# albfre/ipm-zoo

Measured on AMD Instinct MI355X. Metric: Newton steps/sec + factor TFLOP/s, dense QP n=8192, 1/2/4/8 MI355X, higher is better.
Workload: dtype f64; 1 GPU; c3; n=8192, m=2048, p=1024, kkt_N=11264, formulation=SlackedSlacks ineq + Regularization eq (delta=1e-4), augmented LDL^T, parallelism=replicas x1 (independent QPs, one per GPU)

## Files before the change

### include/ipmz.h

```cpp
#ifndef IPMZ_H
#define IPMZ_H

#include <stddef.h>
#include <stdint.h>

#ifdef __cplusplus
extern "C" {
#endif

#define IPMZ_OK 0
#define IPMZ_ERR_INVALID (-1)
#define IPMZ_ERR_HIP (-2)
#define IPMZ_ERR_NOMEM (-3)
#define IPMZ_ERR_NO_DEVICE (-4)
#define IPMZ_ERR_STATE (-5)

enum ipmz_slot {
  IPMZ_SLOT_X = 0, IPMZ_SLOT_LAMBDA_A, IPMZ_SLOT_LAMBDA_C, IPMZ_SLOT_S, IPMZ_SLOT_P,
  IPMZ_SLOT_LAMBDA_G, IPMZ_SLOT_LAMBDA_H, IPMZ_SLOT_LAMBDA_Y, IPMZ_SLOT_LAMBDA_Z,
  IPMZ_SLOT_G, IPMZ_SLOT_H, IPMZ_SLOT_Y, IPMZ_SLOT_Z, IPMZ_NSLOT
};

enum ipmz_scalar {
  IPMZ_SC_F = 0,
// ... 46 lines not shown

int64_t ipmz_normal_workspace_bytes(ipmz_ctx* ctx, int n, int mp);
int ipmz_normal_factor(ipmz_ctx* ctx, int n, int mp, double* K, int64_t ld, double* D, void* ws, int64_t ws_bytes);
int ipmz_normal_solve(ipmz_ctx* ctx, int n, int mp, const double* K, int64_t ld, const double* D, void* ws, double* b);
int ipmz_normal_solve_multi(ipmz_ctx* ctx, int n, int mp, const double* K, int64_t ld, const double* D, void* ws,
                            double* B, int64_t ldb, int nrhs);

int ipmz_bk_factor(ipmz_ctx* ctx, int N, double* A, int64_t ld, int* ipiv, int fix_kp);
#define IPMZ_BK_AUTO 0
#define IPMZ_BK_WORKGROUP 1
#define IPMZ_BK_GRID 2
int ipmz_bk_factor_ex(ipmz_ctx* ctx, int N, double* A, int64_t ld, int* ipiv, int fix_kp, int algo);
int ipmz_bk_solve(ipmz_ctx* ctx, int N, const double* F, int64_t ld, const int* ipiv, double* b);
int64_t ipmz_bk_solve_workspace_bytes(ipmz_ctx* ctx, int N);
int ipmz_bk_prepare_solve(ipmz_ctx* ctx, int N, const double* F, int64_t ld, const int* ipiv,
                          void* ws, int64_t ws_bytes);
int ipmz_bk_solve_multi(ipmz_ctx* ctx, int N, const double* F, int64_t ld, const int* ipiv,
                        const void* ws, double* B, int64_t ldb, int nrhs);
#define IPMZ_BK_NMAX 4096
int ipmz_bk_factor_batch(ipmz_ctx* ctx, int N, int batch, double* A, int64_t ld, int64_t sA,
                         int* ipiv, int64_t sP, int fix_kp, int* info);
int64_t ipmz_bk_batch_solve_workspace_bytes(ipmz_ctx* ctx, int N, int batch);
int ipmz_bk_prepare_solve_batch(ipmz_ctx* ctx, int N, int batch, const double* F, int64_t ld, int64_t sA,
                                const int* ipiv, int64_t sP, void* ws, int64_t ws_bytes);
int ipmz_bk_solve_multi_batch(ipmz_ctx* ctx, int N, int batch, const double* F, int64_t ld, int64_t sA,
                              const int* ipiv, int64_t sP, const void* ws,
                              double* B, int64_t ldb, int64_t sB, int nrhs);

int ipmz_symmetric_indefinite_factorization(ipmz_ctx* ctx, int N, const double* A, double* F, int* ipiv);
int ipmz_overwriting_solve_bunch_kaufman(ipmz_ctx* ctx, int N, const double* F, const int* ipiv, double* b);
int ipmz_overwriting_solve_bunch_kaufman_multi(ipmz_ctx* ctx, int N, const double* F, const int* ipiv,
                                               double* B, int nrhs);

int ipmz_ldlt_decomposition(ipmz_ctx* ctx, int N, const double* A, double* L, double* D);
int ipmz_overwriting_solve_ldlt(ipmz_ctx* ctx, int N, const double* L, const double* D, double* b);
int ipmz_overwriting_solve_ldlt_multi(ipmz_ctx* ctx, int N, const double* L, const double* D, double* B, int nrhs);

#define IPMZ_EQ_REGULARIZATION 0
#define IPMZ_EQ_NONE 1
#define IPMZ_EQ_PENALTY 2
#define IPMZ_EQ_PENALTY_EXTRA_DUAL 3
#define IPMZ_EQ_SLACKED_SLACKS 4
#define IPMZ_EQ_NAIVE_SLACKS 5
#define IPMZ_INEQ_SLACKED_SLACKS 0
#define IPMZ_INEQ_SLACKS 1
#define IPMZ_INEQ_NAIVE_SLACKS 2
#define IPMZ_BOUNDS_BOTH 0
#define IPMZ_BOUNDS_LOWER 1
#define IPMZ_BOUNDS_UPPER 2
#define IPMZ_BOUNDS_NONE 3
typedef struct ipmz_qp_config {
  int n;
  int m;
  int p;
  double delta;
  int equality_handling;
  int inequality_handling;
  int inequality_bounds;
  int variable_bounds;
} ipmz_qp_config;

int ipmz_qp_create(ipmz_ctx* ctx, const ipmz_qp_config* cfg, ipmz_qp** out);
int ipmz_qp_destroy(ipmz_qp* qp);
int ipmz_qp_load_host(ipmz_qp* qp, const double* Q, const double* c, const double* A, const double* l_A,
                      const double* u_A, const double* C, const double* d, const double* l_x, const double* u_x);
int ipmz_qp_generate(ipmz_qp* qp, uint64_t seed);
#define IPMZ_STEP_RESTART_IF_CONVERGED 1
#define IPMZ_STEP_GRAPH 2
int ipmz_qp_step(ipmz_qp* qp, int flags);
int ipmz_qp_last_step_graph(ipmz_qp* qp);
int ipmz_qp_scalars(ipmz_qp* qp, double* out);
int ipmz_qp_device_scalars(ipmz_qp* qp, double** out);
int ipmz_qp_copy_scalars(ipmz_qp* qp, double* dst_device);
int ipmz_qp_solve(ipmz_qp* qp, int max_iter, double* trace, int* iterations);
#define IPMZ_STATE_VARS 0
#define IPMZ_STATE_DAFF 1
#define IPMZ_STATE_DIR 2
#define IPMZ_STATE_RES 3
int64_t ipmz_qp_state_len(ipmz_qp* qp);
int ipmz_qp_get_state(ipmz_qp* qp, int which, double* host_out);
int ipmz_qp_set_state(ipmz_qp* qp, const double* host_vars);
int ipmz_qp_get_kkt(ipmz_qp* qp, double* host_K);
int ipmz_qp_kkt_dim(ipmz_qp* qp);
int ipmz_qp_kkt_solve(ipmz_qp* qp, int nrhs, double* B, int64_t ldb);
int ipmz_qp_kkt_solve_bk(ipmz_qp* qp, int nrhs, double* B, int64_t ldb);
int ipmz_qp_kkt_solve_mixed(ipmz_qp* qp, int nrhs, double* B, int64_t ldb, double tol, int max_refine, double* stat);
int ipmz_qp_set_mixed_precision(ipmz_qp* qp, int enable, double tol, int max_refine);
#define IPMZ_REDUCTION_AUGMENTED 0
#define IPMZ_REDUCTION_NORMAL 1
int ipmz_qp_set_reduction(ipmz_qp* qp, int reduction);

int ipmz_batch_create(ipmz_ctx* ctx, const ipmz_qp_config* cfg, int batch, ipmz_qp** out);
int ipmz_batch_size(ipmz_qp* qp);
int ipmz_batch_load_host(ipmz_qp* qp, int index, const double* Q, const double* c, const double* A,
                         const double* l_A, const double* u_A, const double* C, const double* d, const double* l_x,
                         const double* u_x);
int ipmz_batch_initialize(ipmz_qp* qp);
int ipmz_batch_scalars(ipmz_qp* qp, double* out);
int ipmz_batch_get_state(ipmz_qp* qp, int index, int which, double* host_out);
int ipmz_batch_set_state(ipmz_qp* qp, int index, const double* host_vars);
typedef struct ipmz_qp_device_data {
  const double* Q;
  int64_t ldq, sQ;
  const double* A;
  int64_t lda, sA;
  const double* C;
  int64_t ldc, sC;
  const double *c, *l_x, *u_x;
  int64_t sc, slx, sux;
  const double *l_A, *u_A;
  int64_t slA, suA;
  const double* d;
  int64_t sd;
} ipmz_qp_device_data;
int ipmz_batch_load_device(ipmz_qp* qp, const ipmz_qp_device_data* data);
int ipmz_batch_copy_state(ipmz_qp* qp, int which, double* dst_device, int64_t ld);
#define IPMZ_SET_STATE_UNCHECKED 1
int ipmz_batch_set_state_device(ipmz_qp* qp, const double* src, int64_t ld, const int32_t* take, double floor,
                                int flags);
int ipmz_batch_copy_scalars(ipmz_qp* qp, double* dst_device);
int ipmz_batch_summary(ipmz_qp* qp, double* dst_device);
int ipmz_batch_solve(ipmz_qp* qp, int max_iter, int* iterations, int* converged_count);
#define IPMZ_BATCH_FACTOR_AUTO 0
#define IPMZ_BATCH_FACTOR_ONE 1
#define IPMZ_BATCH_FACTOR_PAIR 2
#define IPMZ_BATCH_FACTOR_LEFT 3
int ipmz_batch_set_factor_kernel(ipmz_qp* qp, int kernel);
int ipmz_batch_get_kkt(ipmz_qp* qp, int index, double* host_K);
int ipmz_batch_kkt_solve(ipmz_qp* qp, int nrhs, double* B, int64_t ldb, int64_t sB);
int ipmz_batch_kkt_solve_bk(ipmz_qp* qp, int nrhs, double* B, int64_t ldb, int64_t sB, int* info);

int ipmz_qp_newton_solve_multi(ipmz_qp* qp, int nrhs, const double* R, int64_t ldr, double* Dir, int64_t ldd,
                               double* alpha );
int ipmz_batch_newton_solve_multi(ipmz_qp* qp, int nrhs, const double* R, int64_t ldr, int64_t sR, double* Dir,
                                  int64_t ldd, int64_t sD, double* alpha ,
                                  int* info );

int ipmz_qp_newton_adjoint_multi(ipmz_qp* qp, int nrhs, const double* G, int64_t ldg, double* Out, int64_t ldo);
int ipmz_batch_newton_adjoint_multi(ipmz_qp* qp, int nrhs, const double* G, int64_t ldg, int64_t sG, double* Out,
                                    int64_t ldo, int64_t sO, int* info );

typedef struct ipmz_qp_device_grad {
  double* Q;
  int64_t ldq, sQ;
  double* A;
  int64_t lda, sA;
  double* C;
  int64_t ldc, sC;
  double *c, *l_x, *u_x;
  int64_t sc, slx, sux;
  double *l_A, *u_A;
  int64_t slA, suA;
  double* d;
  int64_t sd;
} ipmz_qp_device_grad;
int ipmz_batch_data_vjp(ipmz_qp* qp, const double* W, int64_t sW, const ipmz_qp_device_grad* grad);

typedef struct ipmz_qp_device_grad_multi {
  ipmz_qp_device_grad g;
  int64_t tQ, tA, tC, tc, tlx, tux, tlA, tuA, td;
} ipmz_qp_device_grad_multi;
int ipmz_batch_data_vjp_multi(ipmz_qp* qp, int ncot, const double* W, int64_t ldw, int64_t sW,
                              const ipmz_qp_device_grad_multi* grad);

typedef struct ipmz_qp_device_tangent {
  ipmz_qp_device_data d;
// ... 16 lines not shown
```

### ipm-zoo_amd/csrc/capi.cpp

```cpp
#include "capi.h"

#include <cstring>

namespace {
thread_local std::string g_last_error;
}

int fail(int code, const std::string& msg) {
  g_last_error = msg;
  return code;
}
int hip_fail(hipError_t e, const char* expr, const char* file, int line) {
  return fail(IPMZ_ERR_HIP, std::string(expr) + ": " + hipGetErrorString(e) + " @" + file + ":" + std::to_string(line));
}

std::mutex g_ctx_mutex;

static int ensure_events(ipmz_ctx* ctx, size_t n) {
  while (ctx->evpool.size() < n) {
    hipEvent_t e;
    if (hipEventCreateWithFlags(&e, hipEventDisableTiming | hipEventDisableSystemFence) != hipSuccess &&
        hipEventCreateWithFlags(&e, hipEventDisableTiming) != hipSuccess)
      return fail(IPMZ_ERR_HIP, "hipEventCreate failed");
    ctx->evpool.push_back(e);
  }
  return IPMZ_OK;
}

static int check_device(int device) {
  int count = 0;
  if (hipGetDeviceCount(&count) != hipSuccess || count <= 0)
    return fail(IPMZ_ERR_NO_DEVICE, "no HIP device visible: libipmz has no CPU fallback");
  if (device < 0 || device >= count) return fail(IPMZ_ERR_INVALID, "device index out of range");
  hipDeviceProp_t prop;
  if (hipGetDeviceProperties(&prop, device) != hipSuccess) return fail(IPMZ_ERR_NO_DEVICE, "device query failed");
  if (std::strncmp(prop.gcnArchName, "gfx950", 6) != 0)
    return fail(IPMZ_ERR_NO_DEVICE, std::string("libipmz is built for gfx950, device is ") + prop.gcnArchName);
  return IPMZ_OK;
}

void ctx_free(ipmz_ctx* ctx) {
  hipSetDevice(ctx->device);
  if (ctx->stream) hipStreamSynchronize(ctx->stream);
  for (hipStream_t s : {ctx->own, ctx->sB, ctx->sC, ctx->sD})
    if (s) {
      hipStreamSynchronize(s);
      hipStreamDestroy(s);
    }
  for (auto e : ctx->evpool) hipEventDestroy(e);
  delete ctx;
}

const char PANEL_TIMEOUT[] = ": a hand-off inside the outer-panel factor kernel timed out (spin limit 0.5 s); the "
                             "factor is invalid";
const char SOLVE_TIMEOUT[] = ": a hand-off inside the persistent triangular solve timed out (spin limit 0.5 s); the "
                             "solution is invalid";
int ws_result(hipStream_t st, const int* info, const unsigned* pe_word, const unsigned* se_word, const char* what,
              const char* pe_text, const char* se_text) {
  int i = 0x7f7f7f7f;
  unsigned pe = 0, se = 0;
  if (pe_word) HIP_OK(hipMemcpyAsync(&pe, pe_word, 4, hipMemcpyDeviceToHost, st));
  if (se_word) HIP_OK(hipMemcpyAsync(&se, se_word, 4, hipMemcpyDeviceToHost, st));
  if (info) HIP_OK(hipMemcpyAsync(&i, info, sizeof(int), hipMemcpyDeviceToHost, st));
  HIP_OK(hipStreamSynchronize(st));
  if (pe) return fail(IPMZ_ERR_HIP, std::string(what) + pe_text);
  if (se) return fail(IPMZ_ERR_HIP, std::string(what) + se_text);
  return i == 0x7f7f7f7f ? IPMZ_OK : i;
}

int read_info(ipmz_ctx* ctx, const LdltWs& w) {
  return ws_result(ctx->stream, w.info, w.pctrl + PANEL_ERR_WORD, w.ctrl + SOLVE_ERR_WORD, "ipmz_ldlt_factor");
}

hipError_t solve_ws(const double* K, int64_t ld, int N, const double* D, const LdltWs& w, int nbi, double* b,
                    hipStream_t st) {
  if (nbi == 64) return ldlt_solve_persistent(K, ld, N, D, w.P, b, w.y, w.z, w.ctrl, st);
  return ldlt_solve(K, ld, N, D, w.Linv, nbi, b, w.side, st);
}

int factor_impl(ipmz_ctx* ctx, int N, double* K, int64_t ld, double* D, const LdltWs& w, int nbo, TrailTimer* timer,
                int* info2) {
  HIP_OK(solve_reset(w.y, w.z, sizeof(double), N, w.ctrl, ctx->stream, w.info, w.pctrl, panel_ctrl_words(N, nbo),
                     info2));
  const int npan = (N + nbo - 1) / nbo;
  auto prep = [&]() -> hipError_t {
    return ctx->nbi == 64 ? solve_prep(K, ld, N, w.Linv, w.P, ctx->stream) : hipSuccess;
  };
  if (npan < 3 || (debug_inject_mask() & IPMZ_DEBUG_ONE_STREAM)) {
    HIP_OK(ldlt_factor(K, ld, N, D, w.Linv, w.W, nbo, ctx->nbi, w.info, ctx->stream, timer, nullptr, nullptr, nullptr,
                       0, w.pctrl));
    HIP_OK(prep());
    return IPMZ_OK;
  }
  const int nev = 5 * npan + 5;
  int rc = ensure_events(ctx, (size_t)nev + 4);
  if (rc) return rc;
  hipEvent_t* ev = ctx->evpool.data();
  const bool fourth = false;
  HIP_OK(ldlt_factor(K, ld, N, D, w.Linv, w.W, nbo, ctx->nbi, w.info, ctx->stream, timer, ctx->sB, ctx->sC, ev,
                     nev - 2, w.pctrl, fourth ? ctx->sD : nullptr));
  HIP_OK(prep());
  return IPMZ_OK;
}

hipError_t bk_setup(const double* F, int64_t ld, int N, const int* ipiv, const int* info, double* LT, double* Lp,
                    int64_t ldp, const BkWs& w, hipStream_t st) {
  hipError_t e = bk_fast_prepare(F, ld, N, ipiv, info, LT, Lp, ldp, w.meta, st);
  if (e == hipSuccess) e = linv_from_l(Lp, ldp, N, 64, w.Linv, st);
  if (e == hipSuccess) e = solve_prep(Lp, ldp, N, w.Linv, w.P, st);
  if (e == hipSuccess) e = solve_reset(w.y, w.x, sizeof(double), N, w.ctrl, st);
  return e;
}
hipError_t bk_run(const double* Lp, int64_t ldp, int N, const double* LT, const int* ipiv, const BkWs& w, double* b,
                  hipStream_t st) {
  const unsigned* flag = bk_fast_flag(w.meta);
  double* t = bk_fast_tmp(w.meta, N);
  const double* ones = bk_fast_ones(w.meta, N);
  hipError_t e = bk_fast_gather(b, N, w.meta, st);
  if (e == hipSuccess) e = ldlt_solve_persistent_sweep(Lp, ldp, N, ones, w.P, t, w.y, w.x, w.ctrl, false, st, flag);
  if (e == hipSuccess) e = bk_fast_dsolve(w.y, N, w.meta, st);
  if (e == hipSuccess) e = ldlt_solve_persistent_sweep(Lp, ldp, N, ones, w.P, t, w.y, w.x, w.ctrl, true, st, flag);
  if (e == hipSuccess) e = bk_fast_scatter(b, N, w.meta, st);
  if (e == hipSuccess) e = bk_fast_fallback(LT, N, ipiv, b, w.meta, st);
  return e;
}

int mixed_factor_impl(ipmz_ctx* ctx, const double* K, int64_t ld, MixedWs& w, TrailTimer* timer) {
  const int npan = (w.N + w.nbo - 1) / w.nbo;
  if (npan < 3 || (debug_inject_mask() & IPMZ_DEBUG_ONE_STREAM)) {
    HIP_OK(mixed_factor(K, ld, w, ctx->stream, nullptr, nullptr, nullptr, 0, timer));
    HIP_OK(solve_prep(w.K32, w.ld32, w.N, w.Linv32, w.P32, ctx->stream));
    return IPMZ_OK;
  }
  const int nev = 5 * npan + 5;
  int rc = ensure_events(ctx, (size_t)nev + 4);
  if (rc) return rc;
  hipEvent_t* ev = ctx->evpool.data();
  const bool fourth = !(debug_inject_mask() & IPMZ_DEBUG_NO_FOURTH);
  HIP_OK(mixed_factor(K, ld, w, ctx->stream, ctx->sB, ctx->sC, ev, nev - 2, timer, fourth ? ctx->sD : nullptr));
  HIP_OK(solve_prep(w.K32, w.ld32, w.N, w.Linv32, w.P32, ctx->stream));
  return IPMZ_OK;
}

static constexpr int SOLVE_MULTI_PANEL = IPMZ_SOLVE_MULTI_PANEL;
static constexpr int SOLVE_MULTI_CROSSOVER = 10;
static_assert(SOLVE_MULTI_PANEL % 128 == 0 && SOLVE_MULTI_PANEL <= IPMZ_TRSM_PANEL_MAX, "panel width");

static int ldlt_multi_impl(ipmz_ctx* ctx, int N, const double* K, int64_t ld, const double* D, const LdltWs& w,
                           double* B, int64_t ldb, int nrhs) {
  const MultiPlan plan =
      multi_plan(nrhs, SOLVE_MULTI_CROSSOVER, SOLVE_MULTI_PANEL, debug_inject_mask(), MultiKind::Ldlt);
  if (!plan.blocked) {
    for (int r = 0; r < nrhs; ++r) HIP_OK(solve_ws(K, ld, N, D, w, ctx->nbi, B + (int64_t)r * ldb, ctx->stream));
  } else {
    HIP_OK(ldlt_solve_multi<double>(K, ld, N, D, w.Linv, ctx->nbi, B, ldb, nrhs, plan.width, ctx->stream));
  }
  watch(ctx, w);
  return IPMZ_OK;
}

static constexpr int BK_MULTI_CROSSOVER = 12;

int bk_multi_impl(ipmz_ctx* ctx, int N, const double* F, int64_t ld, const int* ipiv, const double* LT,
                  const double* Lp, int64_t ldp, const BkWs& w, double* B, int64_t ldb, int nrhs) {
  const MultiPlan plan = multi_plan(nrhs, BK_MULTI_CROSSOVER, SOLVE_MULTI_PANEL, debug_inject_mask(), MultiKind::Bk);
  hipStream_t st = ctx->stream;
  if (!plan.blocked) {
    for (int r = 0; r < nrhs; ++r) {
      double* b = B + (int64_t)r * ldb;
      if (N < IPMZ_BK_GRID_MIN) HIP_OK(bk_solve(F, ld, N, ipiv, b, 1, 0, 0, 0, st));
      else HIP_OK(bk_run(Lp, ldp, N, LT, ipiv, w, b, st));
    }
  } else {
    const unsigned* flag = bk_fast_flag(w.meta);
    HIP_OK(bk_multi_gather(B, ldb, nrhs, N, w.meta, st));
    HIP_OK(trsm_sweep<double>(Lp, ldp, N, w.Linv, 64, B, ldb, nrhs, plan.width, false, st, flag));
    HIP_OK(bk_multi_dsolve(B, ldb, nrhs, N, w.meta, st));
    HIP_OK(trsm_sweep<double>(Lp, ldp, N, w.Linv, 64, B, ldb, nrhs, plan.width, true, st, flag));
    HIP_OK(bk_multi_scatter(B, ldb, nrhs, N, w.meta, st));
    HIP_OK(bk_multi_fallback(LT, N, ipiv, B, ldb, nrhs, w.meta, st));
  }
  watch(ctx, w);
  return IPMZ_OK;
// ... 679 lines not shown
```

### ipm-zoo_amd/csrc/capi.h

```cpp
#pragma once
#include <hip/hip_runtime.h>

#include <cstdint>
#include <mutex>
#include <string>
#include <vector>

#include "ipmz.h"
#include "kernels.h"

using namespace ipmz;

#pragma GCC visibility push(hidden)

int fail(int code, const std::string& msg);
int hip_fail(hipError_t e, const char* expr, const char* file, int line);
#define HIP_OK(expr)                                                           \
  do {                                                                         \
    hipError_t _e = (expr);                                                    \
    if (_e != hipSuccess) return hip_fail(_e, #expr, __FILE__, __LINE__);      \
  } while (0)

inline int64_t round_up(int64_t x, int64_t a) { return (x + a - 1) / a * a; }

// ... 95 lines not shown
  int64_t total = 0;
};
inline BkBatchWs bk_batch_ws(char* base, int N, int batch) {
  BkBatchWs w;
  Carver c{base};
  w.ldp = round_up(N, 64);
  w.sLT = round_up((int64_t)N * N, 32);
  w.sLp = (int64_t)N * w.ldp;
  w.sLinv = (int64_t)((N + 63) / 64) * 64 * 64;
  w.sM = (int64_t)bk_fast_meta_bytes(N);
  w.LT = c.take<double>(w.sLT * batch);
  w.Lp = c.take<double>(w.sLp * batch);
  w.Linv = c.take<double>(w.sLinv * batch);
  w.meta = c.take<char>(w.sM * batch);
  w.total = c.off;
  return w;
}

struct VjpWs {
  double* part = nullptr;
  int64_t total = 0;
};
inline VjpWs vjp_ws(char* base, int64_t elems) {
  VjpWs w;
  Carver c{base};
  w.part = c.take<double>(elems);
  w.total = c.off;
  return w;
}

struct JvpWs {
  double* prod = nullptr;
  int64_t total = 0;
};
inline JvpWs jvp_ws(char* base, int64_t elems) {
  JvpWs w;
  Carver c{base};
  w.prod = c.take<double>(elems);
  w.total = c.off;
  return w;
}

inline void watch(ipmz_ctx* ctx, const unsigned* pe, const unsigned* se) {
  ctx->check_pe = pe;
  ctx->check_se = se;
}
inline void watch(ipmz_ctx* ctx, const LdltWs& w) { watch(ctx, w.pctrl + PANEL_ERR_WORD, w.ctrl + SOLVE_ERR_WORD); }
inline void watch(ipmz_ctx* ctx, const BkWs& w) { watch(ctx, nullptr, w.ctrl + SOLVE_ERR_WORD); }
inline void unwatch(ipmz_ctx* ctx) { ctx->check_pe = ctx->check_se = nullptr; }

enum class MultiKind { Ldlt, Bk, Batch };
struct MultiPlan {
  bool blocked;
  int width;
  bool fused;
};
constexpr MultiPlan multi_plan(int nrhs, int crossover, int panel, int dbg, MultiKind kind) {
  const bool w512 = dbg & IPMZ_DEBUG_MULTI_W512, w128 = dbg & IPMZ_DEBUG_MULTI_W128;
  const bool batch = kind == MultiKind::Batch;
  const bool blocked =
      nrhs >= crossover || ((dbg & IPMZ_DEBUG_MULTI_BLOCKED) && (kind == MultiKind::Ldlt || nrhs >= 2));
  return {blocked, batch && w512 && w128 ? panel : w512 ? 512 : w128 ? 128 : panel, blocked && batch && !w512 && !w128};
}
constexpr bool multi_plan_pins(MultiKind kind, int forced, int w0, int w512, int w128, int wboth, bool fused) {
  const int rows[4] = {1, 2, 9, 10}, width[4] = {w0, w512, w128, wboth};
  for (int m = 0; m < 8; ++m)
    for (int i = 0; i < 4; ++i) {
      const int dbg = (m & 1 ? IPMZ_DEBUG_MULTI_W512 : 0) | (m & 2 ? IPMZ_DEBUG_MULTI_W128 : 0) |
                      (m & 4 ? IPMZ_DEBUG_MULTI_BLOCKED : 0);
      const bool blocked = i == 3 || ((m & 4) && (forced >> i & 1));
      const MultiPlan p = multi_plan(rows[i], 10, 256, dbg, kind);
      if (p.blocked != blocked || p.width != width[m & 3] || p.fused != (blocked && fused && !(m & 3))) return false;
    }
  return true;
}
static_assert(multi_plan_pins(MultiKind::Ldlt, 0b1111, 256, 512, 128, 512, false), "Ldlt: blocked at any count, 512 wins");
static_assert(multi_plan_pins(MultiKind::Bk, 0b1110, 256, 512, 128, 512, false), "Bk: blocked from 2 rows, 512 wins");
static_assert(multi_plan_pins(MultiKind::Batch, 0b1110, 256, 512, 128, 256, true), "Batch: from 2 rows, both = default");

extern const char PANEL_TIMEOUT[], SOLVE_TIMEOUT[];
int ws_result(hipStream_t st, const int* info, const unsigned* pe, const unsigned* se, const char* what,
              const char* pe_text = PANEL_TIMEOUT, const char* se_text = SOLVE_TIMEOUT);
int read_info(ipmz_ctx* ctx, const LdltWs& w);
int factor_impl(ipmz_ctx* ctx, int N, double* K, int64_t ld, double* D, const LdltWs& w, int nbo, TrailTimer* timer,
                int* info2 = nullptr);
hipError_t solve_ws(const double* K, int64_t ld, int N, const double* D, const LdltWs& w, int nbi, double* b,
                    hipStream_t st);
int mixed_factor_impl(ipmz_ctx* ctx, const double* K, int64_t ld, MixedWs& w, TrailTimer* timer);
int mixed_multi_impl(ipmz_ctx* ctx, const double* K, int64_t ld, MixedWs& w, const MixedMultiWs& m, double* B,
                     int64_t ldb, int nrhs, double tol, int max_refine, double* stat);
int not_capturing(ipmz_ctx* ctx, const char* who);
int normal_factor_impl(ipmz_ctx* ctx, int n, int mp, double* K, int64_t ld, double* D, const NormalWs& w, int nbo,
                       TrailTimer* timer);
int normal_solve_impl(ipmz_ctx* ctx, int n, int mp, const double* K, int64_t ld, const double* D, const NormalWs& w,
                      double* b);
hipError_t bk_setup(const double* F, int64_t ld, int N, const int* ipiv, const int* info, double* LT, double* Lp,
                    int64_t ldp, const BkWs& w, hipStream_t st);
hipError_t bk_run(const double* Lp, int64_t ldp, int N, const double* LT, const int* ipiv, const BkWs& w, double* b,
                  hipStream_t st);
int bk_multi_impl(ipmz_ctx* ctx, int N, const double* F, int64_t ld, const int* ipiv, const double* LT,
                  const double* Lp, int64_t ldp, const BkWs& w, double* B, int64_t ldb, int nrhs);
int bk_batch_prepare(ipmz_ctx* ctx, int N, int batch, const double* F, int64_t ld, int64_t sA, const int* ipiv,
                     int64_t sP, const int* info, const BkBatchWs& w);
int bk_batch_multi_impl(ipmz_ctx* ctx, int N, int batch, const double* F, int64_t ld, int64_t sA, const int* ipiv,
                        int64_t sP, const BkBatchWs& w, double* B, int64_t ldb, int64_t sB, int nrhs);
int bk_batch_info(hipStream_t st, const int* dinfo, int batch, int* info);

#pragma GCC visibility pop
```

### ipm-zoo_amd/csrc/kernels.h

```cpp
#pragma once
#include <hip/hip_runtime.h>
#include <stdint.h>
#include <stdio.h>

#define IPMZ_NBO_MAX 512
#define IPMZ_PANEL_CTRL_WORDS 320
#define IPMZ_EARLY_CHAIN_MAX_N 4096
#define IPMZ_TCHUNK 32
#define IPMZ_CHAIN_STAMP_BLOCKS 512
#define IPMZ_SOLVE_BLOCK 128
#define IPMZ_SOLVE_CTRL_WORDS 8

namespace ipmz {

enum { IPMZ_INJECT_SOLVE = 1, IPMZ_INJECT_PANEL = 2, IPMZ_INJECT_GRAPH_FORKS = 4, IPMZ_DEBUG_CONVERT_ONLY = 16,
       IPMZ_DEBUG_ONE_STREAM = 32, IPMZ_DEBUG_TRACE = 64, IPMZ_DEBUG_F32_ENGINE = 128,
       IPMZ_DEBUG_NO_FOURTH = 256, IPMZ_DEBUG_IR_FULL = 512,
       IPMZ_DEBUG_F64_ENGINE = 1024, IPMZ_DEBUG_GIVEBACK = 2048, IPMZ_DEBUG_ROWS_CHAIN = 4096,
       IPMZ_DEBUG_NO_K0 = 8192, IPMZ_DEBUG_NO_FUSED_SOLVES = 16384, IPMZ_DEBUG_READY_LATE = 32768,
       IPMZ_DEBUG_MULTI_BLOCKED = 65536, IPMZ_DEBUG_MULTI_W512 = 131072,
       IPMZ_DEBUG_MULTI_W128 = 262144, IPMZ_DEBUG_SOLVE_H2 = 524288, IPMZ_DEBUG_SOLVE_H4 = 1048576,
       IPMZ_DEBUG_NEWTON_RPG1 = 2097152, IPMZ_DEBUG_NEWTON_RPG8 = 4194304 };
#define IPMZ_TRACE(...)                                                  \
  do {                                                                   \
    if (::ipmz::debug_inject_mask() & ::ipmz::IPMZ_DEBUG_TRACE) {        \
      fprintf(stderr, "[ipmz] " __VA_ARGS__);                            \
      fputc('\n', stderr);                                              \
      fflush(stderr);                                                    \
    }                                                                    \
  } while (0)
int debug_inject_mask();
hipError_t stream_record(hipEvent_t e, hipStream_t s);
hipError_t stream_wait(hipStream_t s, hipEvent_t e);
void set_capture_origin(hipStream_t s);
void set_debug_inject_mask(int mask);
constexpr int PANEL_ERR_WORD = 2;
constexpr int SOLVE_ERR_WORD = 1;

struct Carver {
  char* base;
  int64_t off = 0;
  template <typename T>
  T* take(int64_t count) {
    char* p = base ? base + off : nullptr;
    off += (count * (int64_t)sizeof(T) + 255) / 256 * 256;
    return reinterpret_cast<T*>(p);
  }
};

struct BatchStrides {
  int B = 1;
  int64_t sK = 0, sD = 0, sL = 0, sW = 0;
  unsigned* pflags = nullptr;
  const double* K0 = nullptr;
  int small_kernel = 0;
};
#define IPMZ_PAIR_FLAGS 32
bool small_pair_eligible(int B, int N);
bool small_pair_used(int kern, bool have_flags, int B, int N);
#define IPMZ_SMALL_NMAX 1024
hipError_t ldlt_factor_small_batched(double* K, int64_t ld, int N, double* D, double* Linv, double* W, int* info,
                                     hipStream_t st, const BatchStrides& bs);
hipError_t ldlt_factor_small_variant(int snw, double* K, int64_t ld, int N, double* D, double* Linv, double* W,
                                     int* info, hipStream_t st, const BatchStrides& bs);
hipError_t ldlt_factor_batched(double* K, int64_t ld, int N, double* D, double* Linv, double* W, int nbo, int nbi,
                               int* info, hipStream_t st, const BatchStrides& bs);
#define IPMZ_TRAIL_SMALL_M 3072
struct TrailTimer {
  hipEvent_t (*pairs)[2] = nullptr;
  int cap = 0, used = 0;
  double flops = 0.0;
  hipEvent_t* next() { return used < cap ? pairs[used++] : nullptr; }
};
hipError_t ldlt_factor(double* K, int64_t ld, int N, double* D, double* Linv, double* W, int nbo, int nbi,
                       int* info, hipStream_t st, TrailTimer* timer = nullptr, hipStream_t st2 = nullptr,
                       hipStream_t st3 = nullptr, hipEvent_t* ev = nullptr, int nev = 0, unsigned* pctrl = nullptr, hipStream_t st4 = nullptr);
hipError_t ldlt_factor(float* K, int64_t ld, int N, float* D, float* Linv, float* W, int nbo, int nbi, int* info,
                       hipStream_t st, TrailTimer* timer, hipStream_t st2, hipStream_t st3, hipEvent_t* ev, int nev,
                       unsigned* pctrl = nullptr, hipStream_t st4 = nullptr);
#define IPMZ_PANEL_PRE00_WORDS (3 * 64 * 64 * 2)
inline int64_t panel_ctrl_words(int N, int nbo) {
  return (int64_t)IPMZ_PANEL_CTRL_WORDS * (1 + (N + nbo - 1) / nbo) + IPMZ_PANEL_PRE00_WORDS;
}
hipError_t panel_factor(double* K, int64_t ld, int N, int k0, int bo, double* D, double* Lb0, double* Wp, int ldw,
                        const double* pre00_in, double* pre00_out,
                        int* info, unsigned* area, unsigned* err, const double* Wprev, int kprev, int boprev,
                        bool rows_prev, hipStream_t st_chain, hipStream_t st_rows,
                        const unsigned* parea = nullptr, bool wait_ready = false);
hipError_t panel_factor(float* K, int64_t ld, int N, int k0, int bo, float* D, float* Lb0, float* Wp, int ldw,
                        const float* pre00_in, float* pre00_out,
                        int* info, unsigned* area, unsigned* err, const float* Wprev, int kprev, int boprev,
                        bool rows_prev, hipStream_t st_chain, hipStream_t st_rows,
                        const unsigned* parea = nullptr, bool wait_ready = false);
hipError_t panel_ready(unsigned* area, hipStream_t st);
hipError_t linv_from_l(const double* L, int64_t ld, int N, int nbi, double* Linv, hipStream_t st, int batch = 1,
                       int64_t sL = 0, int64_t sLinv = 0);
hipError_t gemm_nt_sub(int M, int N, int Kd, const double* A, int64_t lda, const double* B, int64_t ldb,
                       double* C, int64_t ldc, int64_t row0, int64_t col0, bool square_lower, hipStream_t st,
                       const BatchStrides* bs = nullptr);

hipError_t ldlt_solve(const double* K, int64_t ld, int N, const double* D, const double* Linv, int nbi, double* b,
                      double* side, hipStream_t st);

#define IPMZ_TRSM_PANEL_MAX 512
struct TrsmBatch {
  int B = 1;
  int64_t sK = 0, sD = 0, sL = 0, sB = 0;
  int64_t sG = 0;
};
template <typename T>
hipError_t ldlt_solve_multi(const T* K, int64_t ld, int N, const T* D, const T* Linv, int nbi, T* B, int64_t ldb,
                            int nrhs, int w, hipStream_t st, const TrsmBatch& tb = TrsmBatch());

template <typename T>
hipError_t trsm_sweep(const T* K, int64_t ld, int N, const T* Linv, int nbi, T* B, int64_t ldb, int nrhs, int w,
                      bool backward, hipStream_t st, const unsigned* gate, const TrsmBatch& tb = TrsmBatch());

bool ldlt_solve_fused_eligible(int N, int nbi);
hipError_t ldlt_solve_fused(const double* K, int64_t ld, int N, const double* D, const double* Linv, int nbi,
                            double* B, int64_t ldb, int nrhs, hipStream_t st, const TrsmBatch& tb = TrsmBatch());

hipError_t ldlt_solve_batched(const double* K, int64_t ld, int N, const double* D, const double* Linv, int nbi,
                              double* b, int B, int64_t sK, int64_t sD, int64_t sL, int64_t sb, hipStream_t st);

int64_t solve_prep_elems(int N);
int64_t solve_vec_elems(int N);
hipError_t solve_reset(void* ybuf, void* xbuf, size_t elem, int N, unsigned* ctrl, hipStream_t st,
                       int* info = nullptr, unsigned* words = nullptr, int64_t nwords = 0, int* info2 = nullptr);
hipError_t solve_stamps(unsigned long long* out);
hipError_t chain_stamps(unsigned long long* c, unsigned long long* h);
hipError_t solve_prep(const double* K, int64_t ld, int N, const double* Linv, double* P, hipStream_t st);
hipError_t solve_prep(const float* K, int64_t ld, int N, const float* Linv, float* P, hipStream_t st);
hipError_t ldlt_solve_persistent(const double* K, int64_t ld, int N, const double* D, const double* P, double* b,
                                 double* ybuf, double* xbuf, unsigned* ctrl, hipStream_t st);
hipError_t ldlt_solve_persistent_sweep(const double* K, int64_t ld, int N, const double* D, const double* P,
                                       double* b, double* ybuf, double* xbuf, unsigned* ctrl, bool backward,
                                       hipStream_t st, const unsigned* skip);
hipError_t ldlt_solve_persistent(const float* K, int64_t ld, int N, const float* D, const float* P, float* b,
                                 float* ybuf, float* xbuf, unsigned* ctrl, hipStream_t st,
                                 const unsigned* skip = nullptr);

struct MixedWs {
  int N = 0, nbo = 256;
  int64_t ld32 = 0;
  float *K32 = nullptr, *D32 = nullptr, *Linv32 = nullptr, *W32 = nullptr, *P32 = nullptr;
  float *y32 = nullptr, *z32 = nullptr, *r32 = nullptr;
  unsigned *ctrl = nullptr, *state = nullptr, *pctrl = nullptr;
  int* info = nullptr;
  double *s = nullptr, *x = nullptr, *colp = nullptr, *rowp = nullptr, *part = nullptr;
  double* stat = nullptr;
  unsigned *hst = nullptr, *hst_dev = nullptr;
  hipEvent_t hev = nullptr;
  int last_iters = 2;
};
int64_t mixed_ws_bytes(int N, int nbo);
int64_t mixed_ws_carve(char* base, int N, int nbo, MixedWs& w);
hipError_t mixed_factor(const double* K, int64_t ld, MixedWs& w, hipStream_t st, hipStream_t st2, hipStream_t st3,
                        hipEvent_t* ev, int nev, TrailTimer* timer = nullptr, hipStream_t st4 = nullptr);
hipError_t mixed_solve(const double* K, int64_t ld, MixedWs& w, double* b, double tol, int max_refine,
                       hipStream_t st);

struct MixedMultiWs {
  int64_t ldx = 0, ld32 = 0;
  int ntiles = 0;
  double* x = nullptr;
  float* r32 = nullptr;
  double* part = nullptr;
  double* stat = nullptr;
  unsigned* done = nullptr;
  unsigned* word = nullptr;
};
int64_t mixed_multi_ws_carve(char* base, int N, int nrhs, MixedMultiWs& m);
hipError_t mixed_solve_multi(const double* K, int64_t ld, const MixedWs& w, const MixedMultiWs& m, double* B,
                             int64_t ldb, int nrhs, double tol, int max_refine, int pw, hipStream_t st);
hipError_t sym_residual_multi(const double* K, int64_t ld, int N, const double* X, int64_t ldx, const double* B,
                              int64_t ldb, double* R, int64_t ldr, int nrhs, hipStream_t st);

hipError_t ne_check_sign(const double* D, int N, int offset, double sign, int* info, hipStream_t st);


#ifndef IPMZ_BK_NMAX
#define IPMZ_BK_NMAX 4096
#endif
hipError_t bk_factor(double* A, int64_t ld, int n, int* ipiv, int* info, int fix_kp, int batch, int64_t sA,
                     int64_t sP, hipStream_t st);
hipError_t bk_solve(const double* F, int64_t ld, int n, const int* ipiv, double* b, int batch, int64_t sA, int64_t sP,
                    int64_t sb, hipStream_t st);
#define IPMZ_BK_GRID_MIN 512
size_t bk_grid_ws_bytes(int n);
hipError_t bk_factor_grid(double* A, int64_t ld, int n, int* ipiv, int* info, int fix_kp, void* ws, hipStream_t st);
const unsigned* bk_grid_err_word(const void* ws, int n);
struct BkBatch {
  int B = 1;
  int64_t sA = 0, sP = 0, sLT = 0, sLp = 0, sB = 0;
};
hipError_t bk_transpose(const double* F, int64_t ld, int n, double* LT, hipStream_t st,
                        const BkBatch& bb = BkBatch());
size_t bk_fast_meta_bytes(int n);
const unsigned* bk_fast_flag(const void* meta);
const double* bk_fast_ones(const void* meta, int n);
double* bk_fast_tmp(void* meta, int n);
hipError_t bk_fast_prepare(const double* F, int64_t ld, int n, const int* ipiv, const int* info, double* LT,
                           double* Lp, int64_t ldp, void* meta, hipStream_t st, const BkBatch& bb = BkBatch());
hipError_t bk_fast_gather(const double* b, int n, void* meta, hipStream_t st);
hipError_t bk_fast_dsolve(double* y, int n, void* meta, hipStream_t st);
hipError_t bk_fast_scatter(double* b, int n, void* meta, hipStream_t st);
hipError_t bk_fast_fallback(const double* LT, int n, const int* ipiv, double* b, const void* meta, hipStream_t st);
hipError_t bk_multi_gather(double* B, int64_t ldb, int nrhs, int n, void* meta, hipStream_t st,
                           const BkBatch& bb = BkBatch());
hipError_t bk_multi_dsolve(double* B, int64_t ldb, int nrhs, int n, void* meta, hipStream_t st,
                           const BkBatch& bb = BkBatch());
hipError_t bk_multi_scatter(double* B, int64_t ldb, int nrhs, int n, void* meta, hipStream_t st,
                            const BkBatch& bb = BkBatch());
hipError_t bk_multi_fallback(const double* LT, int n, const int* ipiv, double* B, int64_t ldb, int nrhs,
                             const void* meta, hipStream_t st);
struct BkFusedMeta {
  const unsigned* flag;
// ... 24 lines not shown
  SC_SIGMA,
  SC_ALPHA,
  SC_CONVERGED,
  SC_MU_NEW,
  SC_RESTARTS,
  SC_COUNT = 16
};

struct QPDev {
  int n, m, p;
  int N;
  int64_t ldn;
  int64_t ldk;
  int64_t state_len;
  double delta;
  int eqnone;
  int eqpen;
  int slacks, vlo, vup, alo, aup;
  int naive;
  int eqss, m_usr, p_usr;
  int mk;
  const double *Q, *c, *A, *lA, *uA, *C, *d, *lx, *ux;
  double* v[NSLOT];
  double* r[NSLOT];
  double* daff[NSLOT];
  double* dir[NSLOT];
  double *Qx, *ATl, *CTl, *Ax, *Cx;
  double* b;
  double* scal;
  double* part;
  double* tpart;
  double* K;
  double* K0;
  double *v0, *r0, *scal0;
  double* Cx0;
  unsigned* done;
};

__host__ __device__ __forceinline__ int residual_rows(const QPDev& q) { return q.n + q.m + q.p; }
__host__ __device__ __forceinline__ int comp_rows(const QPDev& q) { return q.n + q.m; }
__host__ __device__ __forceinline__ int corrector_rows(const QPDev& q) {
  return comp_rows(q) + (q.eqpen ? q.p : 0);
}
__host__ __device__ __forceinline__ int update_rows(const QPDev& q) {
  const int mp = q.m > q.p ? q.m : q.p;
  return q.n > mp ? q.n : mp;
}

__host__ __device__ __forceinline__ int64_t eqss_block(int64_t k, int64_t m, int64_t p) {
  const int64_t mp = m + p;
  if (k < m) return k;
  if (k < 2 * m) return mp + (k - m);
  if (k < 2 * m + p) return m + (k - 2 * m);
  return mp + m + (k - 2 * m - p);
}
__host__ __device__ __forceinline__ int64_t eqss_source(int64_t k, const QPDev& q) {
  const int64_t n = q.n, m = q.m_usr, p = q.p_usr, mp = m + p;
  const int64_t duals = q.naive ? n : n + 2 * mp;
  if (k < duals) return k;
  if (k < duals + 2 * mp) return duals + eqss_block(k - duals, m, p);
  const int64_t slacks = duals + 2 * mp + (q.vlo ? n : 0) + (q.vup ? n : 0);
  if (k < slacks) return k;
  if (k < slacks + 2 * mp) return slacks + eqss_block(k - slacks, m, p);
  return k;
}

__host__ __device__ __forceinline__ int slot_in_order(bool naive, int k) {
  constexpr int naive_order[NSLOT] = {X, LG, LH, LC, P, LY, LZ, G, H, Y, Z, LA, S};
  return naive ? naive_order[k] : k;
}
__host__ __device__ __forceinline__ bool nonneg_slot(int slot) { return slot >= LG; }
__host__ __device__ __forceinline__ bool explicit_bounds(const QPDev& q) { return q.slacks || q.m == 0; }

struct QPBatch {
  const QPDev* d;
  QPDev h;
  int B;
};

hipError_t qp_generate(const QPBatch& qb, uint64_t seed0, hipStream_t st);
hipError_t qp_init_iterate(const QPBatch& qb, hipStream_t st);
hipError_t qp_evaluate(const QPBatch& qb, hipStream_t st);
hipError_t qp_assemble(const QPBatch& qb, hipStream_t st);
hipError_t qp_rhs(const QPBatch& qb, hipStream_t st);
hipError_t qp_backsub(const QPBatch& qb, int which, hipStream_t st);
hipError_t qp_ratio(const QPBatch& qb, int which, int out_index, hipStream_t st);
#define IPMZ_NEWTON_MULTI_RPG 4
hipError_t qp_rhs_multi(const QPBatch& qb, const double* R, int64_t ldr, int64_t sR, double* W, int64_t ldw, int64_t sW,
                        int nrhs, hipStream_t st);
hipError_t qp_backsub_multi(const QPBatch& qb, const double* R, int64_t ldr, int64_t sR, const double* W, int64_t ldw,
                            int64_t sW, double* D, int64_t ldd, int64_t sD, int nrhs, hipStream_t st);
hipError_t qp_ratio_multi(const QPBatch& qb, const double* D, int64_t ldd, int64_t sD, double* alpha, int nrhs,
                          hipStream_t st);
hipError_t qp_adj_reduce_multi(const QPBatch& qb, const double* Cot, int64_t ldg, int64_t sG, double* W, int64_t ldw,
                               int64_t sW, int nrhs, hipStream_t st);
hipError_t qp_adj_expand_multi(const QPBatch& qb, const double* Cot, int64_t ldg, int64_t sG, const double* W,
                               int64_t ldw, int64_t sW, double* Out, int64_t ldo, int64_t sO, int nrhs, hipStream_t st);
hipError_t qp_mu_aff(const QPBatch& qb, hipStream_t st);
hipError_t qp_corrector_residuals(const QPBatch& qb, hipStream_t st);
hipError_t qp_update(const QPBatch& qb, int freeze, hipStream_t st);
hipError_t qp_restart_if_converged(const QPBatch& qb, hipStream_t st);
hipError_t qp_save_initial(const QPBatch& qb, hipStream_t st);
hipError_t qp_batch_summary(const QPBatch& qb, double* out, hipStream_t st);
#define IPMZ_FUSED_NMAX 1024
enum { KMODE_K = 0, KMODE_K0_DIAG = 1, KMODE_K0_OFFDIAG = 2 };
hipError_t qp_fused_pre(const QPBatch& qb, int restart, int* info, hipStream_t st, int kmode = KMODE_K);
hipError_t qp_fused_mid(const QPBatch& qb, hipStream_t st);
hipError_t qp_fused_post(const QPBatch& qb, int freeze, hipStream_t st);
inline bool fused_solves_ok(int N, int64_t ld) { return N <= 4096 && !(ld & 1); }
hipError_t qp_fused_solves(const QPBatch& qb, const double* K, int64_t ld, int N, const double* D, const double* Linv,
                           double* b, int64_t sK, int64_t sD, int64_t sL, int64_t sb, int freeze, hipStream_t st);
hipError_t qp_fused_eval(const QPBatch& qb, hipStream_t st);

enum DataBlock { DB_Q = 0, DB_A, DB_CEQ, DB_C, DB_LX, DB_UX, DB_LA, DB_UA, DB_D, DB_COUNT, DB_MATS = DB_C };
enum : unsigned {
  HELD_Q = 1, HELD_C = 2, HELD_A = 4, HELD_LA = 8, HELD_UA = 16, HELD_CEQ = 32, HELD_D = 64, HELD_LX = 128,
  HELD_UX = 256, HELD_ALL = 511
};
struct DataBlockInfo {
  const char* name;
  bool matrix;
  int dim;
  unsigned held;
};
constexpr DataBlockInfo DATA_BLOCKS[DB_COUNT] = {
    {"Q", true, 0, HELD_Q},      {"A", true, 1, HELD_A},      {"C", true, 2, HELD_CEQ},
    {"c", false, 0, HELD_C},     {"l_x", false, 0, HELD_LX},  {"u_x", false, 0, HELD_UX},
    {"l_A", false, 1, HELD_LA},  {"u_A", false, 1, HELD_UA},  {"d", false, 2, HELD_D}};
template <class T>
struct QpBlocks {
  T* p[DB_COUNT];
  int64_t sq[DB_COUNT], tq[DB_COUNT], ld[DB_MATS];
};
typedef QpBlocks<const double> QpBlocksIn;
typedef QpBlocks<double> QpBlocksOut;
constexpr unsigned long long IPMZ_IO_VALID = ~0ull;
constexpr unsigned long long io_key(int qp, int kind, int k) {
  return ((unsigned long long)(unsigned)qp << 33) | ((unsigned long long)kind << 32) | (unsigned)k;
}
hipError_t qp_io_validate(const QPBatch& qb, const QpBlocksIn& in, unsigned long long* verdict, hipStream_t st);
hipError_t qp_io_pack(const QPBatch& qb, const QpBlocksIn& in, hipStream_t st);
hipError_t qp_gather_state(const QPBatch& qb, int which, double* dst, int64_t ld, hipStream_t st);
hipError_t qp_scatter_state(const QPBatch& qb, const double* src, int64_t ld, const int32_t* take, double floor,
                            hipStream_t st);
hipError_t qp_scatter_validate(const QPBatch& qb, const double* src, int64_t ld, const int32_t* take, double floor,
                               unsigned long long* verdict, hipStream_t st);

#define IPMZ_VJP_KCHUNK 64
#define IPMZ_VJP_SLAB 16
int64_t qp_grad_part_elems(const QPBatch& qb, int ncot = 1);
hipError_t qp_data_vjp(const QPBatch& qb, int ncot, const double* W, int64_t ldw, int64_t sW, const QpBlocksOut& o,
                       double* part, hipStream_t st);

#define IPMZ_JVP_ROWS_GY 16384
struct JvpMat {
  int mode, rch, nchunk, nct;
  int64_t off_row, off_col;
};
struct JvpPlan {
  JvpMat mat[3];
  int64_t seg;
};
JvpPlan qp_jvp_plan(const QPBatch& qb, const QpBlocksIn& in);
int jvp_pairs(int n);
hipError_t qp_data_jvp(const QPBatch& qb, int ntan, const QpBlocksIn& in, double* R, int64_t ldr, int64_t sR, double* ws,
                       hipStream_t st);
// ... 3 lines not shown
```

### ipm-zoo_amd/csrc/ldlt.hip

```cpp
#include <cstdlib>
#include <cstring>
#include <map>
#include <mutex>
#include <unordered_map>
#include <vector>

#include "common.h"
#include "diag64.h"
#include "gemm.h"
#include "gemm32.h"
#include "gemm64.h"
#include "kernels.h"

namespace ipmz {

static int g_inject = 0;

int debug_inject_mask() { return g_inject; }
void set_debug_inject_mask(int mask) { g_inject = mask; }

namespace {
struct Noted {
  unsigned long long id;
  std::vector<hipGraphNode_t> nodes;
// ... 264 lines not shown
  if (M <= 4096) return launch_gemm<64, 64, EPI_SUB_STRIP, 2, 2, OPT_NOR2>(g, st, batch);
  if (M <= 8192) return launch_gemm<64, 128, EPI_SUB_STRIP, 2, 4, OPT_NOR2>(g, st, batch);
  return launch_gemm<128, 128, EPI_SUB_STRIP, 2, 4, OPT_NOR2>(g, st, batch);
}
hipError_t gemm_nt_sub(int M, int N, int Kd, const double* A, int64_t lda, const double* B, int64_t ldb,
                       double* C, int64_t ldc, int64_t row0, int64_t col0, bool square_lower, hipStream_t st,
                       const BatchStrides* bs) {
  return gemm_nt_sub_t<double>(M, N, Kd, A, lda, B, ldb, C, ldc, row0, col0, square_lower, st, bs);
}

template <typename T>
static hipError_t factor_panel(T* K, int64_t ld, int N, T* D, T* Linv, T* W, int k0, int bo, int nbo, int nbi,
                               int* info, hipStream_t st, const BatchStrides* bs = nullptr) {
  hipError_t e = hipSuccess;
  const int B = bs ? bs->B : 1;
  const int64_t sK = bs ? bs->sK : 0, sD = bs ? bs->sD : 0, sL = bs ? bs->sL : 0, sW = bs ? bs->sW : 0;
  for (int j0 = k0; j0 < k0 + bo; j0 += nbi) {
    const int bi = k0 + bo - j0 < nbi ? k0 + bo - j0 : nbi;
    T* Lb = Linv + (int64_t)(j0 / nbi) * nbi * nbi;
    if (nbi == 128)
      hipLaunchKernelGGL((ldlt_diag_kernel<T, 128>), dim3(B), dim3(1024), 0, st, K, ld, j0, bi, D, Lb, info, sK, sD, sL);
    else
      launch_diag64(B, st, K, ld, j0, bi, D, Lb, info, sK, sD, sL);
    if ((e = hipGetLastError()) != hipSuccess) return e;
    const int r1 = j0 + bi;
    if (r1 >= N) continue;
    GemmArgsT<T> g{};
    g.M = N - r1;
    g.N = bi;
    g.Kd = bi;
    g.A = K + (int64_t)r1 * ld + j0;
    g.lda = ld;
    g.B = Lb;
    g.ldb = nbi;
    g.C = K + (int64_t)r1 * ld + j0;
    g.ldc = ld;
    g.W = W + (int64_t)r1 * nbo + (j0 - k0);
    g.ldw = nbo;
    g.dvec = D + j0;
    g.lower = 0;
    g.sA = sK;
    g.sB = sL;
    g.sC = sK;
    g.sW = sW;
    g.sD = sD;
    e = nbi == 128 ? launch_gemm<128, 128, EPI_PANEL, 2, 4>(g, st, B) : launch_gemm<128, 64, EPI_PANEL, 4, 2>(g, st, B);
    if (e != hipSuccess) return e;
    const int c1 = k0 + bo;
    if (r1 < c1) {
      e = gemm_nt_sub_t<T>(N - r1, c1 - r1, bi, W + (int64_t)r1 * nbo + (j0 - k0), nbo, K + (int64_t)r1 * ld + j0, ld,
                           K + (int64_t)r1 * ld + r1, ld, r1, r1, false, st, bs);
      if (e != hipSuccess) return e;
    }
  }
  return hipSuccess;
}

template <typename T>
static hipError_t panel_update(T* K, int64_t ld, int N, const T* Wk, int nbo, int k0, int bo, int c0, int c1,
                               bool square, hipStream_t st, const BatchStrides* bs = nullptr) {
  if (c0 >= c1 || c0 >= N) return hipSuccess;
  return gemm_nt_sub_t<T>(N - c0, c1 - c0, bo, Wk + (int64_t)c0 * nbo, nbo, K + (int64_t)c0 * ld + k0, ld,
                     K + (int64_t)c0 * ld + c0, ld, c0, c0, square, st, bs);
}

hipError_t ldlt_factor_batched(double* K, int64_t ld, int N, double* D, double* Linv, double* W, int nbo, int nbi,
                               int* info, hipStream_t st, const BatchStrides& bs) {
  if (N <= 0 || bs.B <= 0) return hipSuccess;
  if (nbi != 64 && nbi != 128) return hipErrorInvalidValue;
  if (nbo % nbi != 0 || nbo > IPMZ_NBO_MAX) return hipErrorInvalidValue;
  if (nbi == 64 && N <= IPMZ_SMALL_NMAX) return ldlt_factor_small_batched(K, ld, N, D, Linv, W, info, st, bs);
  hipError_t e = hipSuccess;
  for (int k0 = 0; k0 < N; k0 += nbo) {
    const int bo = N - k0 < nbo ? N - k0 : nbo, t0 = k0 + bo;
    if ((e = factor_panel(K, ld, N, D, Linv, W, k0, bo, nbo, nbi, info, st, &bs)) != hipSuccess) return e;
    if (t0 < N && (e = panel_update(K, ld, N, W, nbo, k0, bo, t0, N, true, st, &bs)) != hipSuccess) return e;
  }
  return hipSuccess;
}

template <typename T>
static hipError_t ldlt_factor_t(T* K, int64_t ld, int N, T* D, T* Linv, T* W, int nbo, int nbi, int* info,
                                hipStream_t st, TrailTimer* timer, hipStream_t st2, hipStream_t st3, hipEvent_t* ev,
                                int nev, unsigned* pctrl, hipStream_t st4) {
  if (N <= 0) return hipSuccess;
  if (nbi != 64 && nbi != 128) return hipErrorInvalidValue;
  if (nbo % nbi != 0 || nbo > IPMZ_NBO_MAX) return hipErrorInvalidValue;
  const int npan = (N + nbo - 1) / nbo;
  const bool fused = pctrl != nullptr && nbi == 64;
  const bool two = st2 != nullptr && ev != nullptr && nev >= 4 * npan + 2 && (!fused || st3 != nullptr);
  const bool four = two && st4 != nullptr && nev >= 5 * npan + 3 && !(debug_inject_mask() & IPMZ_DEBUG_NO_FOURTH);
  const int64_t wsz = (int64_t)N * nbo;
  auto Wb = [&](int k) { return W + (two ? (k % 3) : 0) * wsz; };
  auto pw = [&](int k) { return N - k * nbo < nbo ? N - k * nbo : nbo; };
  auto area = [&](int k) { return pctrl + (int64_t)IPMZ_PANEL_CTRL_WORDS * (1 + k); };
  unsigned* err = pctrl ? pctrl + PANEL_ERR_WORD : nullptr;
  hipStream_t sC = (two && fused) ? st3 : st;
  hipStreamCaptureStatus cap = hipStreamCaptureStatusNone;
  if (two && fused && hipStreamIsCapturing(st, &cap) != hipSuccess) cap = hipStreamCaptureStatusActive;
  const bool early_ok = two && fused && cap == hipStreamCaptureStatusNone;
  auto early_at = [&](int j) { return early_ok && N - j * nbo <= IPMZ_EARLY_CHAIN_MAX_N; };
  auto tiles_at = [&](int j) { return two && fused && N - j * nbo <= IPMZ_EARLY_CHAIN_MAX_N; };
  auto flag_at = [&](int j) { return j >= 2 && early_at(j - 1) && tiles_at(j); };
  T* pre00 = pctrl ? reinterpret_cast<T*>(pctrl + (int64_t)IPMZ_PANEL_CTRL_WORDS * (1 + npan)) : nullptr;
  auto slot00 = [&](int k) { return pre00 + (int64_t)(k % 3) * 64 * 64; };
  auto factor = [&](int k, bool prev) -> hipError_t {
    const int k0 = k * nbo;
    if (!fused) return factor_panel(K, ld, N, D, Linv, Wb(k), k0, pw(k), nbo, nbi, info, st);
    return panel_factor(K, ld, N, k0, pw(k), D, Linv + (int64_t)(k0 / 64) * 64 * 64, Wb(k), nbo,
                        (two && prev) ? slot00(k) : nullptr, two ? slot00(k + 1) : nullptr, info, area(k), err,
                        prev ? Wb(k - 1) : nullptr, k0 - nbo, nbo, prev && tiles_at(k), st, sC,
                        (early_at(k) && prev) ? area(k - 1) : nullptr, prev && flag_at(k));
  };
  hipError_t e = hipSuccess;
  if (!two) {
    for (int k = 0; k < npan; ++k) {
      const int k0 = k * nbo, bo = pw(k), t0 = k0 + bo;
      if ((e = factor(k, false)) != hipSuccess) return e;
      if (t0 < N) {
        hipEvent_t* te = timer && N - t0 > IPMZ_TRAIL_SMALL_M ? timer->next() : nullptr;
        if (te) hipEventRecord(te[0], st);
        e = panel_update(K, ld, N, Wb(k), nbo, k0, bo, t0, N, true, st);
        if (te) hipEventRecord(te[1], st);
        if (te) timer->flops += (double)(N - t0) * (double)(N - t0 + 1) * (double)bo;
        if (e != hipSuccess) return e;
      }
    }
    return hipSuccess;
  }
  hipEvent_t* evP = ev;
  hipEvent_t* evN = ev + npan;
  hipEvent_t* evC = ev + 2 * npan;
  hipEvent_t* evA = ev + 3 * npan;
  hipEvent_t* evT = ev + 4 * npan + 2;
  hipEvent_t evJoin = ev[4 * npan];
  hipEvent_t evJoin4 = four ? ev[5 * npan + 2] : nullptr;
  hipEvent_t evEntry = ev[4 * npan + 1];
  IPMZ_TRACE("factor: N=%d npan=%d look-ahead", N, npan);
  if ((e = stream_record(evEntry, st)) != hipSuccess) return e;
  if ((e = stream_wait(st2, evEntry)) != hipSuccess) return e;
  if (fused && (e = stream_wait(sC, evEntry)) != hipSuccess) return e;
  if ((e = factor(0, false)) != hipSuccess) return e;
  if (fused) {
    if ((e = stream_record(evA[0], st)) != hipSuccess) return e;
    if ((e = stream_record(evC[0], sC)) != hipSuccess) return e;
    if (!early_at(1) && (e = stream_wait(st, evC[0])) != hipSuccess) return e;
  }
  for (int k = 0; k < npan; ++k) {
    const int k0 = k * nbo, bo = pw(k);
    const int p1 = k0 + bo;
    const int p2 = p1 < N ? p1 + pw(k + 1) : N;
    const int p3 = p2 < N ? p2 + pw(k + 2) : N;
    if (p1 >= N) break;
    IPMZ_TRACE("factor: panel %d", k);
    if ((e = stream_record(evP[k], st)) != hipSuccess) return e;
    if ((e = stream_wait(st2, evP[k])) != hipSuccess) return e;
    if (early_at(k + 1) && (e = stream_wait(st2, evC[k])) != hipSuccess) return e;
    hipStream_t sN = four ? st4 : st2;
    if (four) {
      if ((e = stream_wait(st4, evP[k])) != hipSuccess) return e;
      if (early_at(k + 1) && (e = stream_wait(st4, evC[k])) != hipSuccess) return e;
      if (k >= 1 && (e = stream_wait(st4, evT[k - 1])) != hipSuccess) return e;
    }
    if (p2 < N) {
      if ((e = panel_update(K, ld, N, Wb(k), nbo, k0, bo, p2, p3, false, sN)) != hipSuccess) return e;
      if (k + 2 < npan && flag_at(k + 2) && (e = panel_ready(area(k + 2), sN)) != hipSuccess) return e;
    }
    if ((e = stream_record(evN[k], sN)) != hipSuccess) return e;
    if (p3 < N) {
      hipEvent_t* te = timer && N - p3 > IPMZ_TRAIL_SMALL_M ? timer->next() : nullptr;
      if (te) hipEventRecord(te[0], st2);
      e = panel_update(K, ld, N, Wb(k), nbo, k0, bo, p3, N, true, st2);
      if (te) hipEventRecord(te[1], st2);
      if (te) timer->flops += (double)(N - p3) * (double)(N - p3 + 1) * (double)bo;
      if (e != hipSuccess) return e;
    }
    if (four && (e = stream_record(evT[k], st2)) != hipSuccess) return e;
    if (k >= 1) {
      if (!flag_at(k + 1) && (e = stream_wait(st, evN[k - 1])) != hipSuccess) return e;
      if (fused && (e = stream_wait(sC, evN[k - 1])) != hipSuccess) return e;
    }
    if (k >= 1) {
      if (early_at(k + 1) && !early_at(k) && (e = stream_wait(st, evC[k - 1])) != hipSuccess) return e;
    }
    if (fused) {
      if (!tiles_at(k + 1) && (e = stream_wait(sC, evA[k])) != hipSuccess) return e;
      if (p2 < N && !tiles_at(k + 1)) {
        if ((e = gemm_nt_sub_t<T>(N - p2, p2 - p1, bo, Wb(k) + (int64_t)p2 * nbo, nbo, K + (int64_t)p1 * ld + k0, ld,
                                  K + (int64_t)p2 * ld + p1, ld, p2, p1, false, sC, nullptr)) != hipSuccess)
          return e;
      }
      if ((e = factor(k + 1, true)) != hipSuccess) return e;
      if ((e = stream_record(evA[k + 1], st)) != hipSuccess) return e;
      if ((e = stream_record(evC[k + 1], sC)) != hipSuccess) return e;
      if (!early_at(k + 2) && (e = stream_wait(st, evC[k + 1])) != hipSuccess) return e;
    } else {
      if ((e = panel_update(K, ld, N, Wb(k), nbo, k0, bo, p1, p2, false, st)) != hipSuccess) return e;
      if ((e = factor(k + 1, false)) != hipSuccess) return e;
    }
  }
  if (early_ok && (e = stream_wait(st, evC[npan - 1])) != hipSuccess) return e;
  if ((e = stream_record(evJoin, st2)) != hipSuccess) return e;
  if (four) {
    if ((e = stream_record(evJoin4, st4)) != hipSuccess) return e;
    if ((e = stream_wait(st, evJoin4)) != hipSuccess) return e;
  }
  return stream_wait(st, evJoin);
}

hipError_t ldlt_factor(double* K, int64_t ld, int N, double* D, double* Linv, double* W, int nbo, int nbi,
                       int* info, hipStream_t st, TrailTimer* timer, hipStream_t st2, hipStream_t st3, hipEvent_t* ev,
                       int nev, unsigned* pctrl, hipStream_t st4) {
  return ldlt_factor_t<double>(K, ld, N, D, Linv, W, nbo, nbi, info, st, timer, st2, st3, ev, nev, pctrl, st4);
}
hipError_t ldlt_factor(float* K, int64_t ld, int N, float* D, float* Linv, float* W, int nbo, int nbi, int* info,
                       hipStream_t st, TrailTimer* timer, hipStream_t st2, hipStream_t st3, hipEvent_t* ev, int nev,
                       unsigned* pctrl, hipStream_t st4) {
  return ldlt_factor_t<float>(K, ld, N, D, Linv, W, nbo, nbi, info, st, timer, st2, st3, ev, nev, pctrl, st4);
}

}
```

### ipm-zoo_amd/csrc/newton.hip

```cpp
#include <type_traits>

#include "common.h"
#include "data_terms.h"
#include "kernels.h"
#include "sync.h"
#include "trsv_small.h"

namespace ipmz {

namespace {
constexpr int NT = 256;
constexpr int RED_BLOCKS = 512;
enum : uint64_t { TAG_Q = 1, TAG_C = 2, TAG_A = 3, TAG_C_EQ = 4, TAG_D = 5 };

__device__ __forceinline__ double block_sum(double v, double* sh) {
  const int lane = threadIdx.x & 63, wave = threadIdx.x >> 6;
  v = wave_sum(v);
  __syncthreads();
  if (lane == 0) sh[wave] = v;
  __syncthreads();
  double t = 0.0;
  if (threadIdx.x == 0)
    for (int w = 0; w < NT / 64; ++w) t += sh[w];
  return t;
// ... 340 lines not shown
}

__device__ __forceinline__ void stats_store(const QPDev& q, double res2, double comp, double f) {
  const double res = sqrt(res2);
  const int cnt = comp_count(q);
  const double mu = cnt == 0 ? 0.0 : comp / (double)cnt;
  q.scal[SC_F] = f;
  q.scal[SC_RES] = res;
  q.scal[SC_MU] = mu;
  q.scal[SC_CONVERGED] = (res < 1e-8 && mu < 1e-8) ? 1.0 : 0.0;
}

__global__ void k_stats_final(const QPDev* __restrict__ qs, int nblocks) {
  const QPDev& q = qs[blockIdx.y];
  __shared__ double sh[4][NT];
  double s[4] = {0.0, 0.0, 0.0, 0.0};
  for (int b = threadIdx.x; b < nblocks; b += NT)
    for (int k = 0; k < 4; ++k) s[k] += q.part[4 * b + k];
  for (int k = 0; k < 4; ++k) sh[k][threadIdx.x] = s[k];
  __syncthreads();
  if (threadIdx.x == 0) {
    double t[4] = {0.0, 0.0, 0.0, 0.0};
    for (int i = 0; i < NT; ++i)
      for (int k = 0; k < 4; ++k) t[k] += sh[k][i];
    stats_store(q, t[0], t[1], t[2] + t[3]);
  }
}

static int red_blocks(int total) {
  int b = (total + NT - 1) / NT;
  return b < 1 ? 1 : (b > RED_BLOCKS ? RED_BLOCKS : b);
}

hipError_t qp_evaluate(const QPBatch& qb, hipStream_t st) {
  const QPDev& h = qb.h;
  hipLaunchKernelGGL((k_matvec_rows<MV_Q>), grid2((h.n + 3) / 4, qb.B), dim3(NT), 0, st, qb.d);
  if (h.m) {
    hipLaunchKernelGGL((k_matvec_rows<MV_A>), grid2((h.m + 3) / 4, qb.B), dim3(NT), 0, st, qb.d);
    matvec_t<MV_A>(qb, st);
  }
  if (h.p) {
    hipLaunchKernelGGL((k_matvec_rows<MV_C>), grid2((h.p + 3) / 4, qb.B), dim3(NT), 0, st, qb.d);
    matvec_t<MV_C>(qb, st);
  }
  const int nb = red_blocks(residual_rows(h));
  hipLaunchKernelGGL(k_residuals, grid2(nb, qb.B), dim3(NT), 0, st, qb.d, 0.0, 1);
  hipLaunchKernelGGL(k_stats_final, grid2(1, qb.B), dim3(NT), 0, st, qb.d, nb);
  return hipGetLastError();
}

__device__ __forceinline__ double ds_inv(const QPDev& q, int i) {
  return ipmz_inv(ipmz_inv(q.v[G][i]) * q.v[LG][i] + ipmz_inv(q.v[H][i]) * q.v[LH][i]);
}
__device__ __forceinline__ double ds_inv_sl(const QPDev& q, int i) {
  return ipmz_inv(ipmz_inv(q.uA[i] + (-q.v[S][i])) * q.v[LH][i] + ipmz_inv(q.v[S][i] + (-q.lA[i])) * q.v[LG][i]);
}
__device__ __forceinline__ double kkt_xx(const QPDev& q, int i, double qii) {
  double h = qii;
  if (q.slacks) {
    if (q.vup) h = h + ipmz_inv(q.ux[i] + (-q.v[X][i])) * q.v[LZ][i];
    if (q.vlo) h = h + ipmz_inv(q.v[X][i] + (-q.lx[i])) * q.v[LY][i];
  } else {
    if (q.vlo) h = h + ipmz_inv(q.v[Y][i]) * q.v[LY][i];
    if (q.vup) h = h + ipmz_inv(q.v[Z][i]) * q.v[LZ][i];
  }
  return h;
}
__device__ __forceinline__ double kkt_aa(const QPDev& q, int i) {
  if (q.slacks) return -ds_inv_sl(q, i);
  if (q.alo && q.aup) return -ds_inv(q, i);
  if (q.alo) return -(ipmz_inv(q.v[LG][i]) * q.v[G][i]);
  return -(ipmz_inv(q.v[LH][i]) * q.v[H][i]);
}

__device__ __forceinline__ double kkt_diag(const QPDev& q, int i) {
  const int n = q.n, m = q.m;
  if (i < n) return kkt_xx(q, i, q.Q[(int64_t)i * q.ldn + i]);
  if (q.naive && i < n + m) return -(ipmz_inv(q.v[LG][i - n]) * q.v[G][i - n]);
  if (q.naive && i < n + q.mk) return -(ipmz_inv(q.v[LH][i - n - m]) * q.v[H][i - n - m]);
  if (i < n + q.mk) return kkt_aa(q, i - n);
  return q.eqnone ? 0.0 : q.eqpen ? -q.scal[SC_MU_NEW] : -(q.delta * q.delta);
}

__device__ __forceinline__ void assemble_row(const QPDev& q, int i, int tid, int nth) {
  double* __restrict__ K = q.K;
  const int64_t ld = q.ldk;
  const int n = q.n, m = q.m, mk = q.mk;
  double* Kr = K + (int64_t)i * ld;
  if (i < n) {
    const double* Qr = q.Q + (int64_t)i * q.ldn;
    for (int j = tid; j < i; j += nth) Kr[j] = Qr[j];
    if (tid == 0) Kr[i] = kkt_diag(q, i);
  } else if (i < n + mk && q.naive) {
    const bool hrow = i >= n + m;
    const int r = hrow ? i - n - m : i - n;
    const double* Ar = q.A + (int64_t)r * q.ldn;
    for (int j = tid; j < n; j += nth) Kr[j] = hrow ? Ar[j] : -Ar[j];
    for (int j = n + tid; j < i; j += nth) Kr[j] = 0.0;
    if (tid == 0) Kr[i] = kkt_diag(q, i);
  } else if (i < n + m) {
    const int r = i - n;
    const double* Ar = q.A + (int64_t)r * q.ldn;
    for (int j = tid; j < n; j += nth) Kr[j] = Ar[j];
    for (int j = n + tid; j < i; j += nth) Kr[j] = 0.0;
    if (tid == 0) Kr[i] = kkt_diag(q, i);
  } else {
    const int r = i - n - mk;
    const double* Cr = q.C + (int64_t)r * q.ldn;
    for (int j = tid; j < n; j += nth) Kr[j] = Cr[j];
    for (int j = n + tid; j < i; j += nth) Kr[j] = 0.0;
    if (tid == 0) Kr[i] = kkt_diag(q, i);
  }
}

__global__ __launch_bounds__(NT) void k_assemble(const QPDev* __restrict__ qs) {
  assemble_row(qs[blockIdx.y], blockIdx.x, threadIdx.x, NT);
}

hipError_t qp_assemble(const QPBatch& qb, hipStream_t st) {
  hipLaunchKernelGGL(k_assemble, grid2(qb.h.N, qb.B), dim3(NT), 0, st, qb.d);
  return hipGetLastError();
}

struct DSel {
  typedef double val_t;
  const QPDev& q;
  double* const* dd;
  __device__ __forceinline__ double r(int slot, int i) const { return q.r[slot][i]; }
  __device__ __forceinline__ double& b(int t) const { return q.b[t]; }
  __device__ __forceinline__ double x(int t) const { return q.b[t]; }
  __device__ __forceinline__ double& d(int slot, int i) const { return dd[slot][i]; }
  __device__ __forceinline__ double zero() const { return 0.0; }
};
__device__ __forceinline__ DSel dsel(const QPDev& q, int which) { return DSel{q, which ? q.dir : q.daff}; }

template <int RP>
struct RowVec {
  double v[RP];
};
#define IPMZ_ROWVEC_OP(OP)                                                                                \
  template <int RP>                                                                                       \
  __device__ __forceinline__ RowVec<RP> operator OP(const RowVec<RP>& a, const RowVec<RP>& b) {            \
    RowVec<RP> c;                                                                                         \
    _Pragma("unroll") for (int k = 0; k < RP; ++k) c.v[k] = a.v[k] OP b.v[k];                              \
    return c;                                                                                             \
  }                                                                                                       \
  template <int RP>                                                                                       \
  __device__ __forceinline__ RowVec<RP> operator OP(const RowVec<RP>& a, double b) {                       \
    RowVec<RP> c;                                                                                         \
    _Pragma("unroll") for (int k = 0; k < RP; ++k) c.v[k] = a.v[k] OP b;                                   \
    return c;                                                                                             \
  }                                                                                                       \
  template <int RP>                                                                                       \
  __device__ __forceinline__ RowVec<RP> operator OP(double a, const RowVec<RP>& b) {                       \
    RowVec<RP> c;                                                                                         \
    _Pragma("unroll") for (int k = 0; k < RP; ++k) c.v[k] = a OP b.v[k];                                   \
    return c;                                                                                             \
  }
IPMZ_ROWVEC_OP(+)
IPMZ_ROWVEC_OP(*)
#undef IPMZ_ROWVEC_OP
template <int RP>
__device__ __forceinline__ RowVec<RP> operator-(const RowVec<RP>& a) {
  RowVec<RP> c;
#pragma unroll
  for (int k = 0; k < RP; ++k) c.v[k] = -a.v[k];
  return c;
}
template <int RP>
struct RowRef {
  double* p;
  int64_t ld;
  int cnt;
  __device__ __forceinline__ void operator=(const RowVec<RP>& a) const {
#pragma unroll
    for (int k = 0; k < RP; ++k)
      if (k < cnt) p[k * ld] = a.v[k];
  }
};
template <int RP>
struct RowsIO {
  typedef RowVec<RP> val_t;
  const QPDev& q;
  const double* R;
  int64_t ldr;
  double* W;
  int64_t ldw;
  double* D;
  int64_t ldd;
  int cnt;
  __device__ __forceinline__ val_t load(const double* p, int64_t ld) const {
    val_t a;
#pragma unroll
    for (int k = 0; k < RP; ++k) a.v[k] = p[(k < cnt ? k : cnt - 1) * ld];
    return a;
  }
  __device__ __forceinline__ val_t r(int slot, int i) const { return load(R + (q.r[slot] - q.r[0]) + i, ldr); }
  __device__ __forceinline__ RowRef<RP> b(int t) const { return RowRef<RP>{W + t, ldw, cnt}; }
  __device__ __forceinline__ val_t x(int t) const { return load(W + t, ldw); }
  __device__ __forceinline__ RowRef<RP> d(int slot, int i) const {
    return RowRef<RP>{D + (q.r[slot] - q.r[0]) + i, ldd, cnt};
  }
  __device__ __forceinline__ val_t zero() const {
// ... 992 lines not shown
```

### ipm-zoo_amd/csrc/qp.cpp

```cpp
#include <algorithm>
#include <cmath>

#include "capi.h"

struct GrowBuf {
  char* p = nullptr;
  size_t bytes = 0;
};

struct ipmz_qp {
  ipmz_ctx* ctx = nullptr;
  int n = 0, m = 0, p = 0, N = 0, B = 1;
  int64_t ldn = 0, ldk = 0, state_len = 0;
  double delta = 1e-4;
  std::vector<void*> allocs;
  bool alloc_failed = false;
  std::vector<QPDev> hq;
  QPDev* dq = nullptr;
  QPBatch qb{};
  double *K = nullptr, *D = nullptr;
  int64_t sK = 0, sD = 0, sb = 0;
  double* K0 = nullptr;
  char* ws = nullptr;
  double *bLinv = nullptr, *bW = nullptr;
// ... 151 lines not shown
    const DataBlockInfo& info = DATA_BLOCKS[k];
    const std::string name = who + ": " + info.name;
    facts->supplied |= info.held;
    const int64_t rows = dims[info.dim], ld = info.matrix ? b.ld[k] : rows, sq = b.sq[k], tq = b.tq[k];
    if (info.matrix && ld < n) return fail(IPMZ_ERR_INVALID, name + ": row stride " + std::to_string(ld) + " < n");
    if (ld < 0 || (sq < 0 && !(r.one_qp_ignores_sq && s->B == 1)) || (use_tq && tq < 0))
      return fail(IPMZ_ERR_INVALID, name + ": negative stride");
    const int64_t extent = info.matrix ? (rows - 1) * ld + n : ld;
    if (use_tq && tq < extent)
      return fail(IPMZ_ERR_INVALID, name + ": tangent stride " + std::to_string(tq) +
                                        " is less than the block's extent " + std::to_string(extent));
    const int64_t all = (use_tq ? (int64_t)(r.ntan - 1) * tq : 0) + extent;
    if (s->B > 1 && sq != 0 && sq < all)
      return fail(IPMZ_ERR_INVALID,
                  name + ": QP stride " + std::to_string(sq) + " is neither 0 (" + r.zero_means + ") nor at least " +
                      (tangents ? "the extent of the QP's tangents " : "the block's extent ") + std::to_string(all));
    if (info.matrix && s->B > 1 && sq == 0) facts->shared_matrix = true;
  }
  return IPMZ_OK;
}

void drop_graph(ipmz_qp* s) {
  if (s->gexec) hipGraphExecDestroy(s->gexec);
  if (s->graph) hipGraphDestroy(s->graph);
  s->gexec = nullptr;
  s->graph = nullptr;
}

void carve(const ipmz_qp* s, double* base, double** slots) {
  int64_t off = 0;
  for (int k = 0; k < NSLOT; ++k) {
    const int slot = slot_in_order(s->naive, k);
    slots[slot] = base + off;
    off += slot_len(s, slot);
  }
}

QPDev& q0(ipmz_qp* s) { return s->hq[0]; }

enum class Path { Ldlt, LdltBatch, Normal, Mixed, BkGrid, BkSmall, BkBatch };
Path path_of(const ipmz_qp* s) {
  if (s->eqnone) return s->B > 1 ? Path::BkBatch : s->N >= IPMZ_BK_GRID_MIN ? Path::BkGrid : Path::BkSmall;
  if (s->normal) return Path::Normal;
  if (s->mixed) return Path::Mixed;
  return s->B == 1 ? Path::Ldlt : Path::LdltBatch;
}

LdltWs ldlt_ws_of(const ipmz_qp* s) { return ldlt_ws(s->ws, s->N, nbo_for(s->ctx, s->N), s->ctx->nbi); }
NormalWs normal_ws_of(const ipmz_qp* s) { return normal_ws(s->nws.p, s->N, nbo_for(s->ctx, s->N), s->ctx->nbi); }

BatchStrides batch_strides(const ipmz_qp* s, const double* K0) {
  return BatchStrides{s->B, s->sK, s->sD, s->sL, s->sW, s->pflags, K0, s->small_kernel};
}
TrsmBatch trsm_batch(const ipmz_qp* s, int64_t sB) { return TrsmBatch{s->B, s->sK, s->sD, s->sL, sB}; }

int solve_batch(ipmz_qp* s, hipStream_t st, int which) {
  switch (path_of(s)) {
    case Path::BkGrid:
      HIP_OK(bk_run(s->K, s->ldk, s->N, s->bklt, s->ipiv, bk_ws(s->bkfws, s->N), q0(s).b, st));
      break;
    case Path::BkSmall:
    case Path::BkBatch:
      HIP_OK(bk_solve(s->K, s->ldk, s->N, s->ipiv, q0(s).b, s->B, s->sK, s->sP, s->sb, st));
      break;
    case Path::Normal:
      return normal_solve_impl(s->ctx, s->n, s->m + s->p, s->K, s->ldk, s->D, normal_ws_of(s), q0(s).b);
    case Path::Mixed:
      HIP_OK(mixed_solve(s->K, s->ldk, s->mw, q0(s).b, s->ir_tol, s->ir_max, st));
      HIP_OK(hipMemcpyAsync(q0(s).scal + IPMZ_SC_IR_RATIO_AFF + 2 * which, s->mw.stat, 2 * sizeof(double),
                            hipMemcpyDeviceToDevice, st));
      break;
    case Path::Ldlt:
      HIP_OK(solve_ws(s->K, s->ldk, s->N, s->D, ldlt_ws_of(s), s->ctx->nbi, q0(s).b, st));
      break;
    case Path::LdltBatch:
      HIP_OK(ldlt_solve_batched(s->K, s->ldk, s->N, s->D, s->bLinv, s->ctx->nbi, q0(s).b, s->B, s->sK, s->sD, s->sL,
                                s->sb, st));
      break;
  }
  return IPMZ_OK;
}

bool uses_k0(const ipmz_qp* s);
int factor_batch(ipmz_qp* s, TrailTimer* tt, bool info_reset) {
  hipStream_t st = s->ctx->stream;
  const int nbo = nbo_for(s->ctx, s->N);
  switch (path_of(s)) {
    case Path::BkGrid:
      HIP_OK(bk_factor_grid(s->K, s->ldk, s->N, s->ipiv, s->binfo, 0, s->bkws, st));
      HIP_OK(bk_transpose(s->K, s->ldk, s->N, s->bklt, st));
      HIP_OK(bk_setup(s->K, s->ldk, s->N, s->ipiv, s->binfo, s->bklt, s->K, s->ldk, bk_ws(s->bkfws, s->N), st));
      return IPMZ_OK;
    case Path::BkSmall:
    case Path::BkBatch:
      HIP_OK(bk_factor(s->K, s->ldk, s->N, s->ipiv, s->binfo, 0, s->B, s->sK, s->sP, st));
      return IPMZ_OK;
    case Path::Mixed: return mixed_factor_impl(s->ctx, s->K, s->ldk, s->mw, tt);
    case Path::Normal:
      return normal_factor_impl(s->ctx, s->n, s->m + s->p, s->K, s->ldk, s->D, normal_ws_of(s), nbo, tt);
    case Path::Ldlt: return factor_impl(s->ctx, s->N, s->K, s->ldk, s->D, ldlt_ws_of(s), nbo, tt);
    case Path::LdltBatch: break;
  }
  if (!info_reset) HIP_OK(hipMemsetAsync(s->binfo, 0x7f, sizeof(int), st));
  HIP_OK(ldlt_factor_batched(s->K, s->ldk, s->N, s->D, s->bLinv, s->bW, nbo, s->ctx->nbi, s->binfo, st,
                             batch_strides(s, info_reset && uses_k0(s) ? s->K0 : nullptr)));
  return IPMZ_OK;
}

bool fused_phases(const ipmz_qp* s) { return s->B > 1 && s->N <= IPMZ_FUSED_NMAX; }
bool fused_solves(const ipmz_qp* s) {
  return fused_phases(s) && path_of(s) == Path::LdltBatch && s->ctx->nbi == 64 && fused_solves_ok(s->N, s->ldk) &&
         !(debug_inject_mask() & IPMZ_DEBUG_NO_FUSED_SOLVES);
}
bool uses_k0(const ipmz_qp* s) {
  return s->K0 && s->ctx->nbi == 64 && s->N <= IPMZ_SMALL_NMAX && !(debug_inject_mask() & IPMZ_DEBUG_NO_K0);
}

int run_step(ipmz_qp* s, int flags) {
  hipStream_t st = s->ctx->stream;
  const QPBatch& qb = s->qb;
  const bool t = s->timing;
  auto mark = [&](int i) {
    IPMZ_TRACE("step: phase mark %d", i);
    if (t) hipEventRecord(s->ev[i], st);
  };
  const bool restart = flags & IPMZ_STEP_RESTART_IF_CONVERGED;
  const int freeze = restart ? 0 : 1;
  const bool fused = fused_phases(s);
  TrailTimer tt;
  tt.pairs = s->tr_pairs;
  tt.cap = t ? s->tr_cap : 0;
  int rc;
  if (fused) {
    mark(0);
    HIP_OK(qp_fused_pre(qb, restart ? 1 : 0, s->eqnone ? nullptr : s->binfo, st, uses_k0(s) ? KMODE_K0_DIAG : KMODE_K));
    mark(1);
    if ((rc = factor_batch(s, nullptr, true))) return rc;
    mark(2);
    if (fused_solves(s)) {
      HIP_OK(qp_fused_solves(qb, s->K, s->ldk, s->N, s->D, s->bLinv, q0(s).b, s->sK, s->sD, s->sL, s->sb, freeze, st));
      mark(3);
      mark(4);
      mark(5);
      HIP_OK(qp_fused_eval(qb, st));
    } else {
      if ((rc = solve_batch(s, st, 0))) return rc;
      mark(3);
      HIP_OK(qp_fused_mid(qb, st));
      mark(4);
      if ((rc = solve_batch(s, st, 1))) return rc;
      mark(5);
      HIP_OK(qp_fused_post(qb, freeze, st));
    }
    mark(6);
    mark(7);
  } else {
    if (restart) HIP_OK(qp_restart_if_converged(qb, st));
    mark(0);
    HIP_OK(qp_assemble(qb, st));
    mark(1);
    if ((rc = factor_batch(s, t ? &tt : nullptr, false))) return rc;
    mark(2);
    HIP_OK(qp_rhs(qb, st));
    if ((rc = solve_batch(s, st, 0))) return rc;
    mark(3);
    HIP_OK(qp_backsub(qb, 0, st));
    HIP_OK(qp_ratio(qb, 0, SC_ALPHA_AFF, st));
    HIP_OK(qp_mu_aff(qb, st));
    HIP_OK(qp_corrector_residuals(qb, st));
    HIP_OK(qp_rhs(qb, st));
    mark(4);
    if ((rc = solve_batch(s, st, 1))) return rc;
    mark(5);
    HIP_OK(qp_backsub(qb, 1, st));
    HIP_OK(qp_ratio(qb, 1, SC_ALPHA, st));
    HIP_OK(qp_update(qb, freeze, st));
    mark(6);
    HIP_OK(qp_evaluate(qb, st));
    mark(7);
  }
  if (t) {
    HIP_OK(hipStreamSynchronize(st));
    float ms = 0.f;
    auto el = [&](int a, int b) {
      hipEventElapsedTime(&ms, s->ev[a], s->ev[b]);
      return (double)ms;
    };
    s->ph_ms[IPMZ_PH_STEP] += el(0, 7);
    s->ph_ms[IPMZ_PH_ASSEMBLE] += el(0, 1);
    s->ph_ms[IPMZ_PH_FACTOR] += el(1, 2);
    s->ph_ms[IPMZ_PH_SOLVE] += el(2, 3) + el(4, 5);
    s->ph_ms[IPMZ_PH_EVAL] += fused ? el(3, 4) + el(5, 6) : el(6, 7);
    for (int i = 0; i < tt.used; ++i) {
      hipEventElapsedTime(&ms, s->tr_pairs[i][0], s->tr_pairs[i][1]);
      s->ph_ms[IPMZ_PH_TRAILING] += ms;
    }
    s->tr_launches += tt.used;
    s->tr_flops += tt.flops * s->B;
  }
  return IPMZ_OK;
}

int initialize(ipmz_qp* s) {
  HIP_OK(hipSetDevice(s->ctx->device));
  hipStream_t st = s->ctx->stream;
  HIP_OK(qp_init_iterate(s->qb, st));
  if (s->K0) HIP_OK(qp_fused_pre(s->qb, 0, nullptr, st, KMODE_K0_OFFDIAG));
  HIP_OK(qp_evaluate(s->qb, st));
  HIP_OK(qp_save_initial(s->qb, st));
  s->loaded = true;
  HIP_OK(hipStreamSynchronize(st));
  return IPMZ_OK;
}

int create_solver(ipmz_ctx* ctx, const ipmz_qp_config* cfg, int B, ipmz_qp** out) {
  if (!ctx || !cfg || !out) return fail(IPMZ_ERR_INVALID, "null argument");
  *out = nullptr;
  if (cfg->n <= 0 || cfg->m < 0 || cfg->p < 0 || B <= 0)
    return fail(IPMZ_ERR_INVALID, "dimensions: n > 0, m >= 0, p >= 0, batch > 0");
  if (cfg->equality_handling != IPMZ_EQ_REGULARIZATION && cfg->equality_handling != IPMZ_EQ_NONE &&
      cfg->equality_handling != IPMZ_EQ_PENALTY && cfg->equality_handling != IPMZ_EQ_PENALTY_EXTRA_DUAL &&
      cfg->equality_handling != IPMZ_EQ_SLACKED_SLACKS && cfg->equality_handling != IPMZ_EQ_NAIVE_SLACKS)
    return fail(IPMZ_ERR_INVALID, "unknown equality handling");
  const int mk = cfg->inequality_handling == IPMZ_INEQ_NAIVE_SLACKS ? 2 * cfg->m : cfg->m;
  if (cfg->equality_handling == IPMZ_EQ_NONE && B > 1 && cfg->n + mk + cfg->p > IPMZ_BK_NMAX)
    return fail(IPMZ_ERR_INVALID, "EqualityHandling::None in batches factors with Bunch-Kaufman one workgroup per "
                                  "system: N <= " + std::to_string(IPMZ_BK_NMAX));
  const int ih = cfg->inequality_handling, ib = cfg->inequality_bounds, vb = cfg->variable_bounds;
  if (ih != IPMZ_INEQ_SLACKED_SLACKS && ih != IPMZ_INEQ_SLACKS && ih != IPMZ_INEQ_NAIVE_SLACKS)
    return fail(IPMZ_ERR_INVALID, "unknown inequality handling");
  if (ih == IPMZ_INEQ_NAIVE_SLACKS && cfg->m > 0 && ib != IPMZ_BOUNDS_BOTH)
    return fail(IPMZ_ERR_INVALID, "InequalityHandling::NaiveSlacks: both inequality bounds");
  if (cfg->equality_handling == IPMZ_EQ_NAIVE_SLACKS && (ih != IPMZ_INEQ_NAIVE_SLACKS || ib != IPMZ_BOUNDS_BOTH))
    return fail(IPMZ_ERR_INVALID, "EqualityHandling::NaiveSlacks: with InequalityHandling::NaiveSlacks and both "
                                  "inequality bounds");
  if (cfg->equality_handling == IPMZ_EQ_SLACKED_SLACKS && (ih != IPMZ_INEQ_SLACKED_SLACKS || ib != IPMZ_BOUNDS_BOTH))
    return fail(IPMZ_ERR_INVALID, "EqualityHandling::SlackedSlacks: with InequalityHandling::SlackedSlacks and both "
                                  "inequality bounds");
  if (ib < IPMZ_BOUNDS_BOTH || ib > IPMZ_BOUNDS_NONE || vb < IPMZ_BOUNDS_BOTH || vb > IPMZ_BOUNDS_NONE)
    return fail(IPMZ_ERR_INVALID, "unknown bounds setting");
  if (cfg->m > 0 && ib == IPMZ_BOUNDS_NONE)
    return fail(IPMZ_ERR_INVALID, "inequality rows need a lower or an upper bound (inequality_bounds != NONE)");
  if (ih == IPMZ_INEQ_SLACKS && ((cfg->m > 0 && ib != IPMZ_BOUNDS_BOTH) || vb != IPMZ_BOUNDS_BOTH))
    return fail(IPMZ_ERR_INVALID, "InequalityHandling::Slacks is built on both bounds (the reference's Slacks "
                                  "formulation drops one-sided bounds inconsistently)");
  HIP_OK(hipSetDevice(ctx->device));
  auto* s = new ipmz_qp();
// ... 443 lines not shown
  return initialize(s);
}

int ipmz_qp_generate(ipmz_qp* s, uint64_t seed) {
  if (!s) return fail(IPMZ_ERR_INVALID, "null qp");
  HIP_OK(hipSetDevice(s->ctx->device));
  HIP_OK(qp_generate(s->qb, seed, s->ctx->stream));
  s->held = HELD_ALL;
  return initialize(s);
}

int ipmz_qp_step(ipmz_qp* s, int flags) { return step_impl(s, flags); }

int ipmz_qp_last_step_graph(ipmz_qp* s) { return s ? s->last_step_graph : 0; }

int ipmz_qp_scalars(ipmz_qp* s, double* out) {
  if (!s || !out) return fail(IPMZ_ERR_INVALID, "null argument");
  return scalars_impl(s, out, 1);
}

int ipmz_qp_device_scalars(ipmz_qp* s, double** out) {
  if (!s || !out) return fail(IPMZ_ERR_INVALID, "null argument");
  *out = s->hq[0].scal;
  return IPMZ_OK;
}

int ipmz_qp_copy_scalars(ipmz_qp* s, double* dst) {
  if (!s || !dst) return fail(IPMZ_ERR_INVALID, "null argument");
  return copy_scalars_impl(s, dst, 1);
}

int ipmz_qp_solve(ipmz_qp* s, int max_iter, double* trace, int* iterations) {
  if (!s || !s->loaded) return fail(IPMZ_ERR_STATE, "load or generate the QP first");
  double sc[SC_COUNT];
  int rc = scalars_impl(s, sc, 1);
  if (rc) return rc;
  int it = 0;
  for (; it < max_iter; ++it) {
    double* row = trace ? trace + 8 * (int64_t)it : nullptr;
    if (row) {
      row[0] = sc[SC_F];
      row[1] = sc[SC_RES];
      row[2] = sc[SC_MU];
      row[7] = sc[SC_CONVERGED];
      row[3] = row[4] = row[5] = row[6] = 0.0;
    }
    if (sc[SC_CONVERGED] != 0.0) break;
    rc = step_impl(s, 0);
    if (rc) return rc;
    rc = scalars_impl(s, sc, 1);
    if (rc) return rc;
    if (row) {
      row[3] = sc[SC_ALPHA_AFF];
      row[4] = sc[SC_MU_AFF];
      row[5] = sc[SC_SIGMA];
      row[6] = sc[SC_ALPHA];
    }
  }
  if (iterations) *iterations = it;
  return IPMZ_OK;
}

int64_t ipmz_qp_state_len(ipmz_qp* s) { return s ? s->state_len : 0; }

int ipmz_qp_get_state(ipmz_qp* s, int which, double* out) {
  if (!s) return fail(IPMZ_ERR_INVALID, "null qp");
  return get_state_impl(s, 0, which, out);
}

int ipmz_qp_set_state(ipmz_qp* s, const double* in) {
  if (!s || !in) return fail(IPMZ_ERR_INVALID, "bad arguments");
  const int rc = set_state_impl(s, 0, s->B, in);
  if (!rc) s->loaded = true;
  return rc;
}

int ipmz_qp_kkt_dim(ipmz_qp* s) { return s ? s->N : 0; }

int ipmz_qp_get_kkt(ipmz_qp* s, double* out) {
  if (!s || !out) return fail(IPMZ_ERR_INVALID, "bad arguments");
  return get_kkt_impl(s, 0, out);
}

int ipmz_batch_get_kkt(ipmz_qp* s, int index, double* out) {
  int rc = check_index(s, index);
  if (rc) return rc;
  if (!out) return fail(IPMZ_ERR_INVALID, "bad arguments");
  return get_kkt_impl(s, index, out);
}

static constexpr int BATCH_MULTI_CROSSOVER = 4;

static int batch_multi_impl(ipmz_qp* s, double* B, int64_t ldb, int64_t sB, int nrhs) {
  hipStream_t st = s->ctx->stream;
  const int nbi = s->ctx->nbi;
  const MultiPlan plan =
      multi_plan(nrhs, BATCH_MULTI_CROSSOVER, IPMZ_SOLVE_MULTI_PANEL, debug_inject_mask(), MultiKind::Batch);
  if (!plan.blocked) {
    for (int r = 0; r < nrhs; ++r)
      HIP_OK(ldlt_solve_batched(s->K, s->ldk, s->N, s->D, s->bLinv, nbi, B + (int64_t)r * ldb, s->B, s->sK, s->sD,
                                s->sL, sB, st));
    return IPMZ_OK;
  }
  const TrsmBatch tb = trsm_batch(s, sB);
  if (plan.fused && ldlt_solve_fused_eligible(s->N, nbi)) {
    HIP_OK(ldlt_solve_fused(s->K, s->ldk, s->N, s->D, s->bLinv, nbi, B, ldb, nrhs, st, tb));
    return IPMZ_OK;
  }
  HIP_OK(ldlt_solve_multi<double>(s->K, s->ldk, s->N, s->D, s->bLinv, nbi, B, ldb, nrhs, plan.width, st, tb));
  return IPMZ_OK;
}

static int check_rhs_block(const ipmz_qp* s, const std::string& who, int nrhs, const char* name, const void* p,
                           int64_t ld, int64_t sB, int64_t len, const char* len_name, bool aligned = true) {
  if (!s->loaded) return fail(IPMZ_ERR_STATE, who + ": load (and initialize) the QP first");
  if (nrhs < 0 || ld < len || (ld & 1) || (nrhs > 0 && !p) ||
      (s->B > 1 && (sB < (int64_t)nrhs * ld || (sB & 1))))
    return fail(IPMZ_ERR_INVALID, who + ": bad arguments (nrhs >= 0; " + name + ": not null, row stride >= " + len_name +
                                      " and even" + (s->B > 1 ? ", QP stride >= nrhs * row stride and even)" : ")"));
  if (aligned && nrhs > 0 && ((uintptr_t)p & 15))
    return fail(IPMZ_ERR_INVALID, who + ": " + name + " must be 16-byte aligned");
  if (path_of(s) == Path::BkBatch && (s->N > IPMZ_BK_NMAX || s->B > 65535))
    return fail(IPMZ_ERR_INVALID, who + ": EqualityHandling::None batches: N <= 4096 and batch <= 65535");
  return IPMZ_OK;
}

static int kkt_ws_ensure(ipmz_qp* s) {
  const Path path = path_of(s);
  if (path == Path::BkSmall) return grow(s, s->bkpws, (size_t)bk_solve_ws(nullptr, s->N).total);
  if (path == Path::BkBatch) return grow(s, s->bkpws, (size_t)bk_batch_ws(nullptr, s->N, s->B).total);
  return IPMZ_OK;
}

static int kkt_enqueue(ipmz_qp* s, double* B, int64_t ldb, int64_t sB, int nrhs) {
  hipStream_t st = s->ctx->stream;
  HIP_OK(qp_assemble(s->qb, st));
  int rc = factor_batch(s, nullptr, false);
  if (rc) return rc;
  switch (path_of(s)) {
    case Path::Ldlt:
      rc = ipmz_ldlt_solve_multi(s->ctx, s->N, s->K, s->ldk, s->D, s->ws, B, ldb, nrhs);
      break;
    case Path::LdltBatch: return batch_multi_impl(s, B, ldb, sB, nrhs);
    case Path::BkGrid:
      rc = bk_multi_impl(s->ctx, s->N, s->K, s->ldk, s->ipiv, s->bklt, s->K, s->ldk, bk_ws(s->bkfws, s->N), B, ldb, nrhs);
      break;
    case Path::BkSmall: {
      const BkSolveWs w = bk_solve_ws(s->bkpws.p, s->N);
      HIP_OK(bk_transpose(s->K, s->ldk, s->N, w.LT, st));
      HIP_OK(bk_setup(s->K, s->ldk, s->N, s->ipiv, s->binfo, w.LT, w.Lp, w.ldp, w.k, st));
      rc = bk_multi_impl(s->ctx, s->N, s->K, s->ldk, s->ipiv, w.LT, w.Lp, w.ldp, w.k, B, ldb, nrhs);
      break;
    }
    case Path::BkBatch: {
      if (nrhs == 0) return IPMZ_OK;
      const BkBatchWs w = bk_batch_ws(s->bkpws.p, s->N, s->B);
      if ((rc = bk_batch_prepare(s->ctx, s->N, s->B, s->K, s->ldk, s->sK, s->ipiv, s->sP, s->binfo, w))) return rc;
      return bk_batch_multi_impl(s->ctx, s->N, s->B, s->K, s->ldk, s->sK, s->ipiv, s->sP, w, B, ldb, sB, nrhs);
    }
    default: break;
  }
  unwatch(s->ctx);
  return rc;
}

static int kkt_finish(ipmz_qp* s, const char* what, int* info) {
// ... 500 lines not shown
```

### ipm-zoo_amd/csrc/trsv_persist.hip

```cpp
#include "common.h"
#include "kernels.h"
#include "sync.h"

namespace ipmz {

__device__ unsigned long long g_sstamp[2][256][6];
#ifdef IPMZ_SOLVE_STAMPS
#define SSTAMP(J, i) \
  if (tid == 0 && (J) < 256) g_sstamp[0][J][i] = __builtin_amdgcn_s_memrealtime()
#else
#define SSTAMP(J, i)
#endif
namespace {
constexpr int SB = IPMZ_SOLVE_BLOCK;
constexpr int SNT = 512;
constexpr int RP_ROWS = 4, RP_LANES = 16;
constexpr int CP_ROWS = 8, CP_LANES = 32;
constexpr int XS_LD = SB + 4;
constexpr int TDS = 65;
enum { SC_TICKET = 2, SC_TICKET_B = 3 };

template <typename T>
__device__ __forceinline__ bool is_sentinel(T v);
template <>
__device__ __forceinline__ bool is_sentinel<double>(double v) {
  return __double_as_longlong(v) == (long long)-1;
}
template <>
__device__ __forceinline__ bool is_sentinel<float>(float v) {
  return __float_as_int(v) == -1;
}
template <typename T>
__device__ __forceinline__ T sentinel() {
  if constexpr (sizeof(T) == 8) return __longlong_as_double(-1ll);
  else return __int_as_float(-1);
}

__device__ __forceinline__ void lds_sync() { asm volatile("s_waitcnt lgkmcnt(0)\n\ts_barrier" ::: "memory"); }

template <typename T>
__device__ __forceinline__ T lanes16_sum(T v) {
  v += dpp_t<0xb1>(v);
  v += dpp_t<0x4e>(v);
  v += __shfl_xor(v, 4);
  return v + __shfl_xor(v, 8);
}

template <typename F>
__device__ __forceinline__ void fetch64(double (&v)[16], F f) {
#pragma unroll
  for (int q = 0; q < 16; ++q) {
    const int i = threadIdx.x + 256 * q;
    v[q] = f(i >> 6, i & 63);
  }
}
template <bool TR>
__device__ __forceinline__ void put64(double* dst, const double (&v)[16]) {
#pragma unroll
  for (int q = 0; q < 16; ++q) {
    const int i = threadIdx.x + 256 * q;
    if (TR) dst[(i & 63) * TDS + (i >> 6)] = v[q];
    else dst[(i >> 6) * TDS + (i & 63)] = v[q];
  }
}
template <bool TA>
__device__ __forceinline__ void mm64(double4_t (&acc)[4], const double* A, const double* B) {
  const int lane = threadIdx.x & 63, wave = threadIdx.x >> 6;
  const int arow = 16 * wave + (lane & 15);
#pragma unroll 4
  for (int s = 0; s < 16; ++s) {
    const int k = 4 * s + (lane >> 4);
    const double a = TA ? A[k * TDS + arow] : A[arow * TDS + k];
#pragma unroll
    for (int n = 0; n < 4; ++n) acc[n] = mfma_f64_16x16x4(a, B[k * TDS + 16 * n + (lane & 15)], acc[n]);
  }
}
__device__ __forceinline__ void zero4(double4_t (&acc)[4]) {
#pragma unroll
  for (int n = 0; n < 4; ++n) acc[n] = (double4_t){0.0, 0.0, 0.0, 0.0};
}
__device__ __forceinline__ void put4(double* dst, const double4_t (&acc)[4], double sgn) {
  const int lane = threadIdx.x & 63, wave = threadIdx.x >> 6;
#pragma unroll
  for (int n = 0; n < 4; ++n)
#pragma unroll
    for (int g = 0; g < 4; ++g)
      dst[(16 * wave + Mfma<double>::row(lane, g)) * TDS + 16 * n + (lane & 15)] = sgn * acc[n][g];
}
template <typename T>
__device__ __forceinline__ void out4(T* dst, int r0, int c0, const double4_t (&acc)[4], int rmax) {
  const int lane = threadIdx.x & 63, wave = threadIdx.x >> 6;
#pragma unroll
  for (int n = 0; n < 4; ++n)
#pragma unroll
    for (int g = 0; g < 4; ++g) {
      const int r = r0 + 16 * wave + Mfma<double>::row(lane, g);
      dst[r * SB + c0 + 16 * n + (lane & 15)] = r < rmax ? (T)acc[n][g] : T(0);
    }
}
}

template <typename T>
__global__ __launch_bounds__(256) void solve_prep_kernel(const T* __restrict__ K, int64_t ld, int N,
                                                         const T* __restrict__ Linv, T* __restrict__ X,
                                                         T* __restrict__ XT, T* __restrict__ M, T* __restrict__ Q,
                                                         int nb) {
  __shared__ double S[4][64 * TDS];
  const int J = blockIdx.x, part = blockIdx.y, J0 = J * SB;
  if ((part == 1 || part == 2) && J == 0) return;
  if (part >= 3 && J + 1 >= nb) return;
  const int h = (part - 1) & 1;
  const int R = N - J0 < SB ? N - J0 : SB;
  const bool two = R > 64;
  double* Xa = S[0];
  double* Xb = S[1];
  double* X21 = S[2];
  double* Ls = S[3];
  auto Kat = [&](int r, int c) -> double { return (r < N && c < N) ? (double)K[(int64_t)r * ld + c] : 0.0; };
  const int64_t lb = (int64_t)2 * J * 64 * 64;
  double v0[16], v1[16], v2[16], va[16], vb[16];
  fetch64(v0, [&](int r, int c) { return (double)Linv[lb + r * 64 + c]; });
  fetch64(v1, [&](int r, int c) { return two ? (double)Linv[lb + 4096 + r * 64 + c] : 0.0; });
  fetch64(v2, [&](int r, int c) { return two ? Kat(J0 + 64 + r, J0 + c) : 0.0; });
  if (part == 1 || part == 2) {
    const int C0 = J0 - SB + 64 * h;
    fetch64(va, [&](int r, int c) { return Kat(J0 + r, C0 + c); });
    fetch64(vb, [&](int r, int c) { return Kat(J0 + 64 + r, C0 + c); });
  } else if (part >= 3) {
    const int RR = J0 + SB + 64 * h;
    fetch64(va, [&](int r, int c) { return Kat(RR + r, J0 + c); });
    fetch64(vb, [&](int r, int c) { return Kat(RR + r, J0 + 64 + c); });
  }
  put64<false>(Xa, v0);
  put64<false>(Xb, v1);
  put64<false>(Ls, v2);
  __syncthreads();
  double4_t acc[4], bot[4];
  zero4(acc);
  mm64<false>(acc, Ls, Xa);
  __syncthreads();
  put4(Ls, acc, 1.0);
  __syncthreads();
  zero4(acc);
  mm64<false>(acc, Xb, Ls);
  put4(X21, acc, -1.0);
  __syncthreads();
  if (part == 0) {
    T* Xo = X + (int64_t)J * SB * SB;
    T* XTo = XT + (int64_t)J * SB * SB;
    for (int i = threadIdx.x; i < SB * SB; i += 256) {
      const int r = i >> 7, c = i & 127;
      double v = 0.0;
      if (r < R && c < R) v = r < 64 ? (c < 64 ? Xa[r * TDS + c] : 0.0)
                                     : (c < 64 ? X21[(r - 64) * TDS + c] : Xb[(r - 64) * TDS + c - 64]);
      Xo[r * SB + c] = (T)v;
      XTo[c * SB + r] = (T)v;
    }
    return;
  }
  zero4(acc);
  zero4(bot);
  if (part <= 2) {
    T* Mo = M + (int64_t)J * SB * SB;
    put64<false>(Ls, va);
    __syncthreads();
    mm64<false>(acc, Xa, Ls);
    mm64<false>(bot, X21, Ls);
    __syncthreads();
    put64<false>(Ls, vb);
    __syncthreads();
    mm64<false>(bot, Xb, Ls);
    out4(Mo, 0, 64 * h, acc, R);
    out4(Mo, 64, 64 * h, bot, R);
  } else {
    T* Qo = Q + (int64_t)J * SB * SB;
    put64<true>(Ls, va);
    __syncthreads();
    mm64<true>(acc, Xa, Ls);
    __syncthreads();
    put64<true>(Ls, vb);
    __syncthreads();
    mm64<true>(acc, X21, Ls);
    mm64<true>(bot, Xb, Ls);
    out4(Qo, 0, 64 * h, acc, R);
    out4(Qo, 64, 64 * h, bot, R);
  }
}

template <typename T, bool BWD, int H>
__global__ __launch_bounds__(SNT) void trsv128_kernel(const T* __restrict__ K, int64_t ld, int N,
                                                      const T* __restrict__ D, const T* __restrict__ X,
                                                      const T* __restrict__ XT, const T* __restrict__ M,
                                                      const T* __restrict__ Q, T* b, T* ybuf, T* xbuf,
                                                      unsigned* ctrl, int nb, const unsigned* __restrict__ skip,
                                                      int inject) {
  typedef typename Mfma<T>::vec2_t V2;
  constexpr int RW = SB / H;
  constexpr int RPR = RP_ROWS / H;
  constexpr int CPT = 4 / H;
  constexpr int TE = 8 * RPR;
  static_assert(H == 1 || H == 2 || H == 4, "parts per block");
  typedef T Tile[TE];
  if (skip && *skip) return;
  __shared__ T vs[2][SB];
  __shared__ T red[SB / CP_ROWS][RW];
  __shared__ T vec[SB], bj[RW];
  __shared__ __attribute__((aligned(16))) T xs[RW * XS_LD];
  __shared__ unsigned sh_ticket, sh_stop, sh_nr[2];
  unsigned* err = ctrl + SOLVE_ERR_WORD;
  T* const vbuf = ybuf + (int64_t)nb * SB;
  T* const ubuf = xbuf + (int64_t)nb * SB;
  const int tid = threadIdx.x;
  const int rg = tid / RP_LANES, cg = tid % RP_LANES;
  if (tid == 0) sh_nr[0] = sh_nr[1] = 0u;

  const unsigned long long t_start = __builtin_amdgcn_s_memrealtime();
  auto stage2 = [&](const T* p0, int c0, int f0, T* d0, const T* p1, int c1, int f1, T* d1) -> bool {
    for (unsigned it = 1;; ++it) {
      lds_sync();
      const int bsel = tid / SB, e = tid % SB;
      if (tid == 0) sh_nr[(it + 1) & 1] = 0u;
      const T* const p = bsel ? p1 : p0;
      if (bsel < 2 && p) {
        const int cnt = bsel ? c1 : c0, nfill = bsel ? f1 : f0;
        T* const d = bsel ? d1 : d0;
        const T v = e < cnt ? ld_sc1(&p[e]) : T(0);
        if (e < cnt && is_sentinel(v)) sh_nr[it & 1] = 1u;
        if (e < cnt || e < nfill) d[e] = v;
      }
      if (tid == 0)
        sh_stop = __builtin_amdgcn_s_memrealtime() - t_start > SPIN_TICKS || ((it & 31u) == 0u && ld_sc1(err) != 0u);
      lds_sync();
      if (!sh_nr[it & 1]) return true;
      if (sh_stop) {
        if (tid == 0) st_sc1(err, 1u);
        return false;
      }
      __builtin_amdgcn_s_sleep(1);
    }
  };
  auto stage = [&](const T* buf, int kb0, int nk, int dir) -> bool {
    const int kb1 = kb0 + dir;
    const int n0 = N - kb0 * SB < SB ? N - kb0 * SB : SB;
    const int n1 = N - kb1 * SB < SB ? N - kb1 * SB : SB;
    return stage2(buf + (int64_t)kb0 * SB, n0, SB, vs[0], nk > 1 ? buf + (int64_t)kb1 * SB : nullptr, n1, SB, vs[1]);
  };
  auto load_rows = [&](Tile& t, const T* p) {
    const T* q = p + RPR * rg * SB + 2 * cg;
#pragma unroll
    for (int k = 0; k < RPR; ++k)
#pragma unroll
      for (int j = 0; j < 4; ++j) {
        const V2 v2 = *reinterpret_cast<const V2*>(q + k * SB + 32 * j);
        t[8 * k + 2 * j] = v2.x;
        t[8 * k + 2 * j + 1] = v2.y;
      }
  };
  auto put_xs = [&](const Tile& t) {
#pragma unroll
    for (int k = 0; k < RPR; ++k)
#pragma unroll
      for (int j = 0; j < 4; ++j)
        *reinterpret_cast<V2*>(&xs[(RPR * rg + k) * XS_LD + 2 * cg + 32 * j]) = V2{t[8 * k + 2 * j], t[8 * k + 2 * j + 1]};
  };
  auto dot_xs = [&](T (&acc)[RPR], const T* v) {
    T vv[8];
#pragma unroll
    for (int j = 0; j < 4; ++j) {
      const V2 v2 = *reinterpret_cast<const V2*>(v + 2 * cg + 32 * j);
      vv[2 * j] = v2.x;
      vv[2 * j + 1] = v2.y;
    }
#pragma unroll
    for (int k = 0; k < RPR; ++k)
#pragma unroll
      for (int j = 0; j < 4; ++j) {
        const V2 x2 = *reinterpret_cast<const V2*>(&xs[(RPR * rg + k) * XS_LD + 2 * cg + 32 * j]);
        acc[k] = fma(x2.x, vv[2 * j], acc[k]);
        acc[k] = fma(x2.y, vv[2 * j + 1], acc[k]);
      }
  };
  auto dot_rows = [&](T (&acc)[RPR], const Tile& t, const T* v) {
    T vv[8];
#pragma unroll
    for (int j = 0; j < 4; ++j) {
      const V2 v2 = *reinterpret_cast<const V2*>(v + 2 * cg + 32 * j);
      vv[2 * j] = v2.x;
      vv[2 * j + 1] = v2.y;
    }
#pragma unroll
    for (int k = 0; k < RPR; ++k)
#pragma unroll
      for (int i = 0; i < 8; ++i) acc[k] = fma(t[8 * k + i], vv[i], acc[k]);
  };

  for (;;) {
    lds_sync();
    if (tid == 0) sh_ticket = atomicAdd(&ctrl[BWD ? SC_TICKET_B : SC_TICKET], 1u);
    lds_sync();
    const int ticket = (int)sh_ticket;
    if (ticket >= nb * H) return;
    if (ticket == 0 && tid == 0) st_sc1(&ctrl[BWD ? SC_TICKET : SC_TICKET_B], 0u);

    if constexpr (!BWD) {
      const int J = ticket / H, h = ticket % H, J0 = J * SB, r0 = h * RW;
      const int R = N - J0 < SB ? N - J0 : SB;
      const int Rh = R - r0 < RW ? R - r0 : RW;
      if (Rh <= 0) continue;
#ifdef IPMZ_SOLVE_STAMPS
      const bool stamp = h == H - 1 || Rh < RW || R == r0 + RW;
#define SSTAMPH(J, i) \
  if (stamp) SSTAMP(J, i)
#else
#define SSTAMPH(J, i)
#endif
      SSTAMPH(J, 0);
      if (tid < Rh) {
        st_sc1(&xbuf[J0 + r0 + tid], sentinel<T>());
        if (H > 1) st_sc1(&ubuf[J0 + r0 + tid], sentinel<T>());
      }
      const T* Lrow = K + (int64_t)(J0 + r0) * ld;
      const int64_t ldr = ld;
      auto row_ok = [&](int k) { return RPR * rg + k < Rh; };
      T acc[RPR];
#pragma unroll
      for (int k = 0; k < RPR; ++k) acc[k] = T(0);
      Tile ta, tb;
      load_rows(ta, X + (int64_t)J * SB * SB + r0 * SB);
      if (tid < RW) bj[tid] = tid < Rh ? b[J0 + r0 + tid] : T(0);
      put_xs(ta);
      auto load_tile = [&](Tile& t, int Kb) {
    #pragma unroll
        for (int k = 0; k < RPR; ++k)
#pragma unroll
          for (int j = 0; j < 4; ++j) {
            const int64_t row = row_ok(k) ? RPR * rg + k : 0;
            const V2 v2 = *reinterpret_cast<const V2*>(Lrow + row * ldr + (int64_t)Kb * SB + 2 * cg + 32 * j);
            t[8 * k + 2 * j] = v2.x;
            t[8 * k + 2 * j + 1] = v2.y;
          }
      };
      const int Kp = J - 2;
      const T* Mj = M + (int64_t)J * SB * SB + r0 * SB;
      if (Kp > 0) {
        load_tile(ta, 0);
        if (Kp > 1) load_tile(tb, 1);
        else load_rows(tb, Mj);
      } else if (J >= 1) {
        if (J == 2) load_tile(ta, 0);
        load_rows(tb, Mj);
      }
      for (int Kc = 0; Kc < Kp; Kc += 2) {
        const bool two = Kc + 1 < Kp;
        if (!stage(ybuf, Kc, two ? 2 : 1, 1)) return;
        dot_rows(acc, ta, vs[0]);
        if (two) dot_rows(acc, tb, vs[1]);
        load_tile(ta, Kc + 2 < Kp ? Kc + 2 : J - 2);
        if (two) {
          if (Kc + 3 < Kp) load_tile(tb, Kc + 3);
          else load_rows(tb, Mj);
        }
      }
      if (J >= 2) {
        if (!stage(ybuf, J - 2, 1, 1)) return;
        dot_rows(acc, ta, vs[0]);
      }
      SSTAMPH(J, 1);
#pragma unroll
      for (int k = 0; k < RPR; ++k) acc[k] = lanes16_sum(acc[k]);
      lds_sync();
      if (cg == 0) {
#pragma unroll
        for (int k = 0; k < RPR; ++k) {
          const int rr = RPR * rg + k;
          const T v = bj[rr] - acc[k];
          vec[r0 + rr] = v;
          if (H > 1 && h < H - 1 && rr < Rh) st_sc1(&vbuf[J0 + r0 + rr], v);
        }
      }
      if (H > 1 && tid < SB && tid >= r0 + RW) vec[tid] = T(0);
      const bool both = H > 1 && h > 0 && J > 0;
      if (H > 1 && h > 0) {
        SSTAMPH(J, 2);
        if (!stage2(vbuf + J0, r0, 0, vec, both ? ybuf + (int64_t)(J - 1) * SB : nullptr, SB, SB, vs[0])) return;
        SSTAMPH(J, 5);
// ... 77 lines not shown
#pragma unroll
          for (int i = 0; i < CPT; ++i) acc[i] = fma(t[CPT * k + i], xv[k], acc[i]);
      };
      const int Klo = J + 3;
      const T* Qj = Q + (int64_t)J * SB * SB + c0 * SB;
      if (nb - 1 >= Klo) {
        load_tile(ta, nb - 1);
        if (nb - 2 >= Klo) load_tile(tb, nb - 2);
        else load_rows(tb, Qj);
      } else if (!last) {
        if (J + 2 <= nb - 1) load_tile(ta, J + 2);
        load_rows(tb, Qj);
      }
      for (int Kc = nb - 1; Kc >= Klo; Kc -= 2) {
        const bool two = Kc - 1 >= Klo;
        if (!stage(xbuf, Kc, two ? 2 : 1, -1)) return;
        dot_cols(ta, vs[0]);
        if (two) dot_cols(tb, vs[1]);
        load_tile(ta, Kc - 2 >= Klo ? Kc - 2 : J + 2);
        if (two) {
          if (Kc - 3 >= Klo) load_tile(tb, Kc - 3);
          else load_rows(tb, Qj);
        }
      }
      if (J + 2 <= nb - 1) {
        if (!stage(xbuf, J + 2, 1, 1)) return;
        dot_cols(ta, vs[0]);
      }
      lds_sync();
#pragma unroll
      for (int i = 0; i < CPT; ++i) red[crg][col(i)] = acc[i];
      lds_sync();
      if (tid < RW) {
        T t = T(0);
#pragma unroll
        for (int k = 0; k < SB / CP_ROWS; ++k) t += red[k][tid];
        const T u = bj[tid] - t;
        vec[c0 + tid] = u;
        if (H > 1 && h > 0 && tid < Rh) st_sc1(&ubuf[J0 + c0 + tid], u);
      }
      if (H > 1 && tid < c0) vec[tid] = T(0);
      const bool both = H > 1 && h < H - 1 && !last;
      if (H > 1 && h < H - 1) {
        const int up = c0 + RW;
        const int n1 = N - (J + 1) * SB < SB ? N - (J + 1) * SB : SB;
        if (!stage2(ubuf + J0 + up, R - up, SB - up, vec + up, both ? xbuf + (int64_t)(J + 1) * SB : nullptr, n1, SB,
                    vs[0]))
          return;
      } else {
        lds_sync();
      }
      T x[RPR];
#pragma unroll
      for (int k = 0; k < RPR; ++k) x[k] = T(0);
      dot_xs(x, vec);
      if (!last) {
        if (!both && !stage(xbuf, J + 1, 1, 1)) return;
        T d[RPR];
#pragma unroll
        for (int k = 0; k < RPR; ++k) d[k] = T(0);
        dot_rows(d, tb, vs[0]);
#pragma unroll
        for (int k = 0; k < RPR; ++k) x[k] -= d[k];
      }
#pragma unroll
      for (int k = 0; k < RPR; ++k) {
        const T xk = lanes16_sum(x[k]);
        const int rr = RPR * rg + k;
        if (cg == 0 && rr < Rh) {
          st_sc1(&xbuf[J0 + c0 + rr], xk);
          b[J0 + c0 + rr] = xk;
        }
      }
    }
  }
}

int64_t solve_prep_elems(int N) {
  const int64_t nb = (N + SB - 1) / SB;
  return 4 * nb * SB * SB;
}

template <typename T>
static hipError_t solve_prep_t(const T* K, int64_t ld, int N, const T* Linv, T* P, hipStream_t st) {
  if (N <= 0) return hipSuccess;
  const int nb = (N + SB - 1) / SB;
  const int64_t q = (int64_t)nb * SB * SB;
  hipLaunchKernelGGL(solve_prep_kernel<T>, dim3(nb, 5), dim3(256), 0, st, K, ld, N, Linv, P, P + q, P + 2 * q,
                     P + 3 * q, nb);
  return hipGetLastError();
}
hipError_t solve_stamps(unsigned long long* out) {
  return hipMemcpyFromSymbol(out, HIP_SYMBOL(g_sstamp), sizeof(unsigned long long) * 2 * 256 * 6);
}
hipError_t solve_prep(const double* K, int64_t ld, int N, const double* Linv, double* P, hipStream_t st) {
  return solve_prep_t<double>(K, ld, N, Linv, P, st);
}
hipError_t solve_prep(const float* K, int64_t ld, int N, const float* Linv, float* P, hipStream_t st) {
  return solve_prep_t<float>(K, ld, N, Linv, P, st);
}

int64_t solve_vec_elems(int N) {
  const int64_t nb = (N + SB - 1) / SB;
  return 2 * nb * SB;
}

template <typename T>
static int solve_parts(int N) {
  const int dbg = debug_inject_mask();
  if ((dbg & IPMZ_DEBUG_SOLVE_H2) && (dbg & IPMZ_DEBUG_SOLVE_H4)) return 1;
  if (dbg & IPMZ_DEBUG_SOLVE_H4) return 4;
  if (dbg & IPMZ_DEBUG_SOLVE_H2) return 2;
  if (N <= SB) return 1;
  return N <= 12288 ? 4 : 2;
}

template <typename T, bool BWD, int H>
static hipError_t launch_sweep(const T* K, int64_t ld, int N, const T* D, const T* P, T* b, T* ybuf, T* xbuf,
                               unsigned* ctrl, hipStream_t st, const unsigned* skip) {
  const int nb = (N + SB - 1) / SB;
  const int64_t q = (int64_t)nb * SB * SB;
  constexpr int RW = SB / H;
  constexpr int64_t lds = (int64_t)sizeof(T) * (RW * XS_LD + (SB / CP_ROWS) * RW + 3 * SB + RW) + 64;
  constexpr int by_threads = 2048 / SNT;
  constexpr int per_cu = 160 * 1024 / lds < by_threads ? (int)(160 * 1024 / lds) : by_threads;
  static_assert(per_cu >= 1, "a part's LDS fits a CU");
  const int tickets = nb * H, cap = 256 * per_cu;
  const int grid = tickets < cap ? tickets : cap;
  const int inject = debug_inject_mask() & IPMZ_INJECT_SOLVE;
  hipLaunchKernelGGL((trsv128_kernel<T, BWD, H>), dim3(grid), dim3(SNT), 0, st, K, ld, N, D, P, P + q, P + 2 * q,
                     P + 3 * q, b, ybuf, xbuf, ctrl, nb, skip, inject);
  return hipGetLastError();
}
template <typename T, bool BWD>
static hipError_t sweep_t(const T* K, int64_t ld, int N, const T* D, const T* P, T* b, T* ybuf, T* xbuf,
                          unsigned* ctrl, hipStream_t st, const unsigned* skip) {
  if (N <= 0) return hipSuccess;
  if (ld % 2) return hipErrorInvalidValue;
  switch (solve_parts<T>(N)) {
    case 4: return launch_sweep<T, BWD, 4>(K, ld, N, D, P, b, ybuf, xbuf, ctrl, st, skip);
    case 2: return launch_sweep<T, BWD, 2>(K, ld, N, D, P, b, ybuf, xbuf, ctrl, st, skip);
    default: return launch_sweep<T, BWD, 1>(K, ld, N, D, P, b, ybuf, xbuf, ctrl, st, skip);
  }
}

template <typename T>
static hipError_t solve_persistent_t(const T* K, int64_t ld, int N, const T* D, const T* P, T* b, T* ybuf, T* xbuf,
                                     unsigned* ctrl, hipStream_t st, const unsigned* skip) {
  const hipError_t e = sweep_t<T, false>(K, ld, N, D, P, b, ybuf, xbuf, ctrl, st, skip);
  if (e != hipSuccess) return e;
  return sweep_t<T, true>(K, ld, N, D, P, b, ybuf, xbuf, ctrl, st, skip);
}

hipError_t ldlt_solve_persistent_sweep(const double* K, int64_t ld, int N, const double* D, const double* P,
                                       double* b, double* ybuf, double* xbuf, unsigned* ctrl, bool backward,
                                       hipStream_t st, const unsigned* skip) {
  return backward ? sweep_t<double, true>(K, ld, N, D, P, b, ybuf, xbuf, ctrl, st, skip)
                  : sweep_t<double, false>(K, ld, N, D, P, b, ybuf, xbuf, ctrl, st, skip);
}

namespace {
struct FillJob {
  unsigned* p[6];
  int64_t n[6];
  unsigned v[6];
};
__global__ __launch_bounds__(256) void fill_words_kernel(FillJob f) {
  const int r = blockIdx.y;
  unsigned* const p = f.p[r];
  const unsigned v = f.v[r];
  for (int64_t i = (int64_t)blockIdx.x * 256 + threadIdx.x; i < f.n[r]; i += (int64_t)gridDim.x * 256) p[i] = v;
}
}

hipError_t solve_reset(void* ybuf, void* xbuf, size_t elem, int N, unsigned* ctrl, hipStream_t st, int* info,
                       unsigned* words, int64_t nwords, int* info2) {
  FillJob f{};
  int cnt = 0;
  int64_t most = 0;
  auto add = [&](void* p, int64_t n, unsigned v) {
    if (!p || n <= 0) return;
    f.p[cnt] = static_cast<unsigned*>(p);
    f.n[cnt] = n;
    f.v[cnt++] = v;
    most = n > most ? n : most;
  };
  add(ctrl, IPMZ_SOLVE_CTRL_WORDS, 0u);
  add(ybuf, solve_vec_elems(N) * (int64_t)elem / 4, ~0u);
  add(xbuf, solve_vec_elems(N) * (int64_t)elem / 4, ~0u);
  add(info, 1, 0x7f7f7f7fu);
  add(info2, 1, 0x7f7f7f7fu);
  add(words, nwords, 0u);
  if (!cnt) return hipSuccess;
  const int64_t gx = (most + 255) / 256;
  hipLaunchKernelGGL(fill_words_kernel, dim3((unsigned)(gx < 64 ? gx : 64), cnt), dim3(256), 0, st, f);
  return hipGetLastError();
}

hipError_t ldlt_solve_persistent(const double* K, int64_t ld, int N, const double* D, const double* P, double* b,
                                 double* ybuf, double* xbuf, unsigned* ctrl, hipStream_t st) {
  return solve_persistent_t<double>(K, ld, N, D, P, b, ybuf, xbuf, ctrl, st, nullptr);
}
hipError_t ldlt_solve_persistent(const float* K, int64_t ld, int N, const float* D, const float* P, float* b,
                                 float* ybuf, float* xbuf, unsigned* ctrl, hipStream_t st, const unsigned* skip) {
  return solve_persistent_t<float>(K, ld, N, D, P, b, ybuf, xbuf, ctrl, st, skip);
}

}
```

### ipm-zoo_amd/ipmz_amd/__init__.py

```python
import ctypes
import os

import numpy as np

HERE = os.path.dirname(os.path.abspath(__file__))
LIB_PATH = os.path.join(os.path.dirname(HERE), "lib", "libipmz.so")

IPMZ_OK = 0
ERR = {-1: "invalid argument", -2: "HIP error", -3: "out of device memory", -4: "no gfx950 device",
       -5: "bad state"}
SC = dict(f=0, res=1, mu=2, alpha_aff=3, mu_aff=4, sigma=5, alpha=6, converged=7, mu_new=8, restarts=9,
          ir_ratio_aff=10, ir_iters_aff=11, ir_ratio=12, ir_iters=13)
SC_COUNT = 16
PH = dict(step=0, assemble=1, factor=2, solve=3, trailing=4, eval=5)
STEP_RESTART_IF_CONVERGED = 1
STEP_GRAPH = 2
SET_STATE_UNCHECKED = 1
SLOTS = ["x", "lambda_A", "lambda_C", "s", "p", "lambda_g", "lambda_h", "lambda_y", "lambda_z", "g", "h", "y", "z"]

EXPORTS = [
    "ipmz_ctx_create", "ipmz_ctx_destroy", "ipmz_ctx_set_stream", "ipmz_ctx_reset_stream", "ipmz_ctx_sync", "ipmz_last_error",
    "ipmz_ctx_set_blocking", "ipmz_ctx_get_blocking", "ipmz_ldlt_workspace_bytes", "ipmz_ldlt_factor", "ipmz_ldlt_solve",
    "ipmz_ldlt_prepare_solve", "ipmz_ldlt_decomposition", "ipmz_overwriting_solve_ldlt", "ipmz_qp_create",
    "ipmz_qp_destroy", "ipmz_qp_load_host", "ipmz_qp_generate", "ipmz_qp_step", "ipmz_qp_scalars",
    "ipmz_qp_device_scalars", "ipmz_qp_copy_scalars", "ipmz_qp_solve", "ipmz_qp_state_len", "ipmz_qp_get_state", "ipmz_qp_set_state",
    "ipmz_qp_get_kkt", "ipmz_qp_kkt_dim", "ipmz_qp_set_timing", "ipmz_qp_phase_times",
    "ipmz_batch_create", "ipmz_batch_size", "ipmz_batch_load_host", "ipmz_batch_initialize", "ipmz_batch_scalars",
    "ipmz_batch_get_state", "ipmz_batch_set_state", "ipmz_batch_solve",
    "ipmz_mixed_workspace_bytes", "ipmz_mixed_factor", "ipmz_mixed_solve", "ipmz_qp_set_mixed_precision",
    "ipmz_batch_copy_scalars", "ipmz_normal_workspace_bytes", "ipmz_normal_factor", "ipmz_normal_solve",
    "ipmz_qp_set_reduction", "ipmz_bk_factor", "ipmz_bk_factor_ex", "ipmz_bk_solve", "ipmz_symmetric_indefinite_factorization",
    "ipmz_overwriting_solve_bunch_kaufman", "ipmz_debug_inject", "ipmz_batch_summary", "ipmz_batch_set_factor_kernel",
    "ipmz_qp_last_step_graph", "ipmz_ldlt_solve_multi", "ipmz_overwriting_solve_ldlt_multi", "ipmz_qp_kkt_solve",
    "ipmz_mixed_multi_workspace_bytes", "ipmz_mixed_solve_multi", "ipmz_sym_residual_multi", "ipmz_qp_kkt_solve_mixed",
    "ipmz_bk_solve_workspace_bytes", "ipmz_bk_prepare_solve", "ipmz_bk_solve_multi",
    "ipmz_overwriting_solve_bunch_kaufman_multi", "ipmz_normal_solve_multi", "ipmz_qp_kkt_solve_bk",
    "ipmz_batch_get_kkt", "ipmz_batch_kkt_solve",
    "ipmz_bk_factor_batch", "ipmz_bk_batch_solve_workspace_bytes", "ipmz_bk_prepare_solve_batch",
    "ipmz_bk_solve_multi_batch", "ipmz_batch_kkt_solve_bk",
    "ipmz_qp_newton_solve_multi", "ipmz_batch_newton_solve_multi",
    "ipmz_qp_newton_adjoint_multi", "ipmz_batch_newton_adjoint_multi",
    "ipmz_batch_load_device", "ipmz_batch_copy_state", "ipmz_batch_data_vjp", "ipmz_batch_data_jvp",
    "ipmz_batch_data_vjp_multi", "ipmz_batch_set_state_device",
]
SOLVE_MULTI_PANEL = 256
REDUCTION_AUGMENTED, REDUCTION_NORMAL = 0, 1

_P = ctypes.POINTER(ctypes.c_double)
_VP = ctypes.c_void_p
_I = ctypes.c_int
_I64 = ctypes.c_int64


class IpmzError(AssertionError):
    """A failed libipmz call (the reference throws Utils::AssertionError)."""


EQ_REGULARIZATION = 0
EQ_NONE = 1
EQ_PENALTY = 2
EQ_PENALTY_EXTRA_DUAL = 3
EQ_SLACKED_SLACKS = 4
EQ_NAIVE_SLACKS = 5
INEQ_SLACKED_SLACKS = 0
INEQ_SLACKS = 1
INEQ_NAIVE_SLACKS = 2
BOUNDS_BOTH = 0
BOUNDS_LOWER = 1
BOUNDS_UPPER = 2
BOUNDS_NONE = 3


class _QPConfig(ctypes.Structure):
    _fields_ = [("n", ctypes.c_int), ("m", ctypes.c_int), ("p", ctypes.c_int), ("delta", ctypes.c_double),
                ("equality_handling", ctypes.c_int), ("inequality_handling", ctypes.c_int),
                ("inequality_bounds", ctypes.c_int), ("variable_bounds", ctypes.c_int)]


class _QPDeviceData(ctypes.Structure):
    _fields_ = [("Q", _VP), ("ldq", _I64), ("sQ", _I64), ("A", _VP), ("lda", _I64), ("sA", _I64),
                ("C", _VP), ("ldc", _I64), ("sC", _I64), ("c", _VP), ("l_x", _VP), ("u_x", _VP),
                ("sc", _I64), ("slx", _I64), ("sux", _I64), ("l_A", _VP), ("u_A", _VP), ("slA", _I64), ("suA", _I64),
                ("d", _VP), ("sd", _I64)]


class _QPDeviceGrad(_QPDeviceData):
    """include/ipmz.h ipmz_qp_device_grad: the same layout, the blocks written (ipmz_batch_data_vjp)."""


class _QPDeviceGradMulti(ctypes.Structure):
    _fields_ = [("g", _QPDeviceGrad)] + [(k, _I64) for k in ("tQ", "tA", "tC", "tc", "tlx", "tux", "tlA", "tuA", "td")]


class _QPDeviceTangent(ctypes.Structure):
    _fields_ = [("d", _QPDeviceData)] + [(k, _I64) for k in ("tQ", "tA", "tC", "tc", "tlx", "tux", "tlA", "tuA", "td")]


_BLOCKS = (("Q", "Q", "ldq", "sQ", "n", "n"), ("A_ineq", "A", "lda", "sA", "m", "n"), ("A_eq", "C", "ldc", "sC", "p", "n"),
           ("c", "c", None, "sc", None, "n"), ("l_x", "l_x", None, "slx", None, "n"), ("u_x", "u_x", None, "sux", None, "n"),
           ("l_A_ineq", "l_A", None, "slA", None, "m"), ("u_A_ineq", "u_A", None, "suA", None, "m"),
           ("b_eq", "d", None, "sd", None, "p"))


def _tensor_block(t, batch, rows, cols, tangent=False):
    import torch
    name, what = "matrix" if rows is not None else "vector", "tangent" if tangent else "block"
    if not isinstance(t, torch.Tensor) or t.dtype != torch.float64:
        raise ValueError(f"{name} {what}: a float64 torch tensor is needed, got {getattr(t, 'dtype', type(t))}")
    inner = (cols,) if rows is None else (rows, cols)
    shape = tuple(t.shape)
    lead = len(shape) - len(inner)
    per_qp = lead == tangent + 1
    if not (per_qp or lead == tangent) or shape[lead:] != inner or (per_qp and shape[0] != batch):
        tan = ("ntan",) if tangent else ()
        raise ValueError(f"{name} {what}: shape {shape} is neither {(batch,) + tan + inner} nor {tan + inner}")
    strides = t.stride()
    sq = strides[0] if per_qp and batch > 1 else 0
    if cols > 1 and strides[-1] != 1:
        raise ValueError(f"{name} {what}: inner stride {strides[-1]}, must be 1 (elements of a row adjacent)")
    ld = 0 if rows is None else (strides[lead] if rows > 1 else max(strides[lead], cols))
    if not tangent:
        return t.data_ptr(), ld, sq
    ntan = shape[lead - 1]
    return t.data_ptr(), ld, sq, (strides[lead - 1] if ntan > 1 else 0), ntan


def _set_block(d, fields, blk, tan=None):
    _, ptr, ld, sq, _, _ = fields
    setattr(d, ptr, blk[0])
    if ld:
        setattr(d, ld, blk[1])
    setattr(d, sq, blk[2])
    if tan is not None:
        setattr(tan, "t" + sq[1:], blk[3])


def _load():
    try:
        import torch
    except ImportError:
        pass
    if not os.path.exists(LIB_PATH):
        raise ImportError(f"libipmz not built: {LIB_PATH} missing (run __graft_entry__.build()); "
                          "there is no CPU fallback")
    lib = ctypes.CDLL(LIB_PATH)
    sig = {
        "ipmz_ctx_create": ([ctypes.POINTER(_VP), _I], _I),
        "ipmz_ctx_destroy": ([_VP], _I),
        "ipmz_ctx_set_stream": ([_VP, _VP], _I),
        "ipmz_ctx_reset_stream": ([_VP], _I),
        "ipmz_ctx_sync": ([_VP], _I),
        "ipmz_last_error": ([], ctypes.c_char_p),
        "ipmz_ctx_set_blocking": ([_VP, _I, _I], _I),
        "ipmz_ctx_get_blocking": ([_VP, _I, ctypes.POINTER(_I), ctypes.POINTER(_I)], _I),
        "ipmz_ldlt_workspace_bytes": ([_VP, _I], _I64),
        "ipmz_ldlt_factor": ([_VP, _I, _VP, _I64, _VP, _VP, _I64], _I),
        "ipmz_ldlt_solve": ([_VP, _I, _VP, _I64, _VP, _VP, _VP], _I),
        "ipmz_ldlt_prepare_solve": ([_VP, _I, _VP, _I64, _VP, _I64], _I),
        "ipmz_ldlt_decomposition": ([_VP, _I, _P, _P, _P], _I),
        "ipmz_overwriting_solve_ldlt": ([_VP, _I, _P, _P, _P], _I),
        "ipmz_qp_create": ([_VP, ctypes.POINTER(_QPConfig), ctypes.POINTER(_VP)], _I),
        "ipmz_qp_destroy": ([_VP], _I),
        "ipmz_qp_load_host": ([_VP] + [_P] * 9, _I),
        "ipmz_qp_generate": ([_VP, ctypes.c_uint64], _I),
        "ipmz_qp_step": ([_VP, _I], _I),
        "ipmz_qp_scalars": ([_VP, _P], _I),
        "ipmz_qp_device_scalars": ([_VP, ctypes.POINTER(_VP)], _I),
        "ipmz_qp_copy_scalars": ([_VP, _VP], _I),
        "ipmz_qp_solve": ([_VP, _I, _P, ctypes.POINTER(_I)], _I),
        "ipmz_qp_state_len": ([_VP], _I64),
        "ipmz_qp_get_state": ([_VP, _I, _P], _I),
        "ipmz_qp_set_state": ([_VP, _P], _I),
        "ipmz_qp_get_kkt": ([_VP, _P], _I),
        "ipmz_qp_kkt_dim": ([_VP], _I),
        "ipmz_qp_set_timing": ([_VP, _I], _I),
        "ipmz_qp_phase_times": ([_VP, _P, _P, ctypes.POINTER(_I64)], _I),
        "ipmz_batch_create": ([_VP, ctypes.POINTER(_QPConfig), _I, ctypes.POINTER(_VP)], _I),
        "ipmz_batch_size": ([_VP], _I),
        "ipmz_batch_load_host": ([_VP, _I] + [_P] * 9, _I),
        "ipmz_batch_initialize": ([_VP], _I),
        "ipmz_batch_scalars": ([_VP, _P], _I),
        "ipmz_batch_get_state": ([_VP, _I, _I, _P], _I),
        "ipmz_batch_set_state": ([_VP, _I, _P], _I),
        "ipmz_batch_solve": ([_VP, _I, ctypes.POINTER(_I), ctypes.POINTER(_I)], _I),
        "ipmz_mixed_workspace_bytes": ([_VP, _I], _I64),
        "ipmz_mixed_factor": ([_VP, _I, _VP, _I64, _VP, _I64], _I),
        "ipmz_mixed_solve": ([_VP, _I, _VP, _I64, _VP, _VP, ctypes.c_double, _I, _P], _I),
        "ipmz_qp_set_mixed_precision": ([_VP, _I, ctypes.c_double, _I], _I),
        "ipmz_batch_copy_scalars": ([_VP, _VP], _I),
        "ipmz_normal_workspace_bytes": ([_VP, _I, _I], _I64),
        "ipmz_normal_factor": ([_VP, _I, _I, _VP, _I64, _VP, _VP, _I64], _I),
        "ipmz_normal_solve": ([_VP, _I, _I, _VP, _I64, _VP, _VP, _VP], _I),
        "ipmz_qp_set_reduction": ([_VP, _I], _I),
        "ipmz_bk_factor": ([_VP, _I, _VP, _I64, _VP, _I], _I),
        "ipmz_bk_factor_ex": ([_VP, _I, _VP, _I64, _VP, _I, _I], _I),
        "ipmz_bk_solve": ([_VP, _I, _VP, _I64, _VP, _VP], _I),
        "ipmz_symmetric_indefinite_factorization": ([_VP, _I, _P, _P, ctypes.POINTER(ctypes.c_int)], _I),
        "ipmz_overwriting_solve_bunch_kaufman": ([_VP, _I, _P, ctypes.POINTER(ctypes.c_int), _P], _I),
        "ipmz_debug_inject": ([_I], _I),
        "ipmz_batch_summary": ([_VP, _VP], _I),
        "ipmz_batch_set_factor_kernel": ([_VP, _I], _I),
        "ipmz_qp_last_step_graph": ([_VP], _I),
        "ipmz_ldlt_solve_multi": ([_VP, _I, _VP, _I64, _VP, _VP, _VP, _I64, _I], _I),
        "ipmz_overwriting_solve_ldlt_multi": ([_VP, _I, _P, _P, _P, _I], _I),
        "ipmz_qp_kkt_solve": ([_VP, _I, _VP, _I64], _I),
        "ipmz_mixed_multi_workspace_bytes": ([_VP, _I, _I], _I64),
        "ipmz_mixed_solve_multi": ([_VP, _I, _VP, _I64, _VP, _VP, _I64, _I, ctypes.c_double, _I, _VP, _I64, _P], _I),
        "ipmz_sym_residual_multi": ([_VP, _I, _VP, _I64, _VP, _I64, _VP, _I64, _VP, _I64, _I], _I),
        "ipmz_qp_kkt_solve_mixed": ([_VP, _I, _VP, _I64, ctypes.c_double, _I, _P], _I),
        "ipmz_bk_solve_workspace_bytes": ([_VP, _I], _I64),
        "ipmz_bk_prepare_solve": ([_VP, _I, _VP, _I64, _VP, _VP, _I64], _I),
        "ipmz_bk_solve_multi": ([_VP, _I, _VP, _I64, _VP, _VP, _VP, _I64, _I], _I),
        "ipmz_overwriting_solve_bunch_kaufman_multi": ([_VP, _I, _P, ctypes.POINTER(ctypes.c_int), _P, _I], _I),
        "ipmz_normal_solve_multi": ([_VP, _I, _I, _VP, _I64, _VP, _VP, _VP, _I64, _I], _I),
        "ipmz_qp_kkt_solve_bk": ([_VP, _I, _VP, _I64], _I),
        "ipmz_batch_get_kkt": ([_VP, _I, _P], _I),
        "ipmz_batch_kkt_solve": ([_VP, _I, _VP, _I64, _I64], _I),
        "ipmz_bk_factor_batch": ([_VP, _I, _I, _VP, _I64, _I64, _VP, _I64, _I, ctypes.POINTER(_I)], _I),
        "ipmz_bk_batch_solve_workspace_bytes": ([_VP, _I, _I], _I64),
        "ipmz_bk_prepare_solve_batch": ([_VP, _I, _I, _VP, _I64, _I64, _VP, _I64, _VP, _I64], _I),
        "ipmz_bk_solve_multi_batch": ([_VP, _I, _I, _VP, _I64, _I64, _VP, _I64, _VP, _VP, _I64, _I64, _I], _I),
        "ipmz_batch_kkt_solve_bk": ([_VP, _I, _VP, _I64, _I64, ctypes.POINTER(_I)], _I),
        "ipmz_qp_newton_solve_multi": ([_VP, _I, _VP, _I64, _VP, _I64, _VP], _I),
        "ipmz_batch_newton_solve_multi": ([_VP, _I, _VP, _I64, _I64, _VP, _I64, _I64, _VP, ctypes.POINTER(_I)], _I),
        "ipmz_qp_newton_adjoint_multi": ([_VP, _I, _VP, _I64, _VP, _I64], _I),
        "ipmz_batch_newton_adjoint_multi": ([_VP, _I, _VP, _I64, _I64, _VP, _I64, _I64, ctypes.POINTER(_I)], _I),
        "ipmz_batch_load_device": ([_VP, ctypes.POINTER(_QPDeviceData)], _I),
        "ipmz_batch_copy_state": ([_VP, _I, _VP, _I64], _I),
        "ipmz_batch_data_vjp": ([_VP, _VP, _I64, ctypes.POINTER(_QPDeviceGrad)], _I),
        "ipmz_batch_data_jvp": ([_VP, _I, ctypes.POINTER(_QPDeviceTangent), _VP, _I64, _I64], _I),
        "ipmz_batch_data_vjp_multi": ([_VP, _I, _VP, _I64, _I64, ctypes.POINTER(_QPDeviceGradMulti)], _I),
        "ipmz_batch_set_state_device": ([_VP, _VP, _I64, _VP, ctypes.c_double, _I], _I),
    }
    for name, (args, res) in sig.items():
        fn = getattr(lib, name)
        fn.argtypes = args
        fn.restype = res
    return lib


lib = _load()


def _check(rc, what):
    if rc < 0:
        msg = lib.ipmz_last_error().decode(errors="replace")
        raise IpmzError(f"{what}: {ERR.get(rc, rc)}: {msg}")
    return rc


def _dp(a):
    return a.ctypes.data_as(_P)


class Context:

    def __init__(self, device=0, stream=None, nbo=None, nbi=None):
# ... 58 lines not shown
        return lib.ipmz_mixed_workspace_bytes(self.h, N)

    def mixed_factor(self, N, K_ptr, ld, ws_ptr, ws_bytes):
        return _check(lib.ipmz_mixed_factor(self.h, N, _VP(K_ptr), ld, _VP(ws_ptr), ws_bytes), "ipmz_mixed_factor")

    def mixed_solve(self, N, K_ptr, ld, ws_ptr, b_ptr, tol=1e-12, max_refine=10):
        stat = np.zeros(2)
        _check(lib.ipmz_mixed_solve(self.h, N, _VP(K_ptr), ld, _VP(ws_ptr), _VP(b_ptr), tol, max_refine, _dp(stat)),
               "ipmz_mixed_solve")
        return float(stat[0]), int(stat[1])

    def mixed_multi_workspace_bytes(self, N, nrhs):
        return lib.ipmz_mixed_multi_workspace_bytes(self.h, N, nrhs)

    def mixed_solve_multi(self, N, K_ptr, ld, ws_ptr, B_ptr, ldb, nrhs, mws_ptr, mws_bytes, tol=1e-12, max_refine=10):
        stat = np.zeros((max(nrhs, 0), 2))
        _check(lib.ipmz_mixed_solve_multi(self.h, N, _VP(K_ptr), ld, _VP(ws_ptr), _VP(B_ptr), ldb, nrhs, tol,
                                          max_refine, _VP(mws_ptr), mws_bytes, _dp(stat)), "ipmz_mixed_solve_multi")
        return stat

    def sym_residual_multi(self, N, K_ptr, ld, X_ptr, ldx, B_ptr, ldb, R_ptr, ldr, nrhs):
        return _check(lib.ipmz_sym_residual_multi(self.h, N, _VP(K_ptr), ld, _VP(X_ptr), ldx, _VP(B_ptr), ldb,
                                                  _VP(R_ptr), ldr, nrhs), "ipmz_sym_residual_multi")

    BK_AUTO, BK_WORKGROUP, BK_GRID = 0, 1, 2

    def bk_factor(self, N, A_ptr, ld, ipiv_ptr, fix_kp=False, algo=0):
        return _check(lib.ipmz_bk_factor_ex(self.h, N, _VP(A_ptr), ld, _VP(ipiv_ptr), int(fix_kp), int(algo)),
                      "ipmz_bk_factor")

    def bk_solve(self, N, F_ptr, ld, ipiv_ptr, b_ptr):
        return _check(lib.ipmz_bk_solve(self.h, N, _VP(F_ptr), ld, _VP(ipiv_ptr), _VP(b_ptr)), "ipmz_bk_solve")

    def bk_solve_workspace_bytes(self, N):
        return lib.ipmz_bk_solve_workspace_bytes(self.h, N)

    def bk_prepare_solve(self, N, F_ptr, ld, ipiv_ptr, ws_ptr, ws_bytes):
        return _check(lib.ipmz_bk_prepare_solve(self.h, N, _VP(F_ptr), ld, _VP(ipiv_ptr), _VP(ws_ptr), ws_bytes),
                      "ipmz_bk_prepare_solve")

    def bk_solve_multi(self, N, F_ptr, ld, ipiv_ptr, ws_ptr, B_ptr, ldb, nrhs):
        return _check(lib.ipmz_bk_solve_multi(self.h, N, _VP(F_ptr), ld, _VP(ipiv_ptr), _VP(ws_ptr), _VP(B_ptr), ldb,
                                              nrhs), "ipmz_bk_solve_multi")

    def bk_factor_batch(self, N, batch, A_ptr, ld, sA, ipiv_ptr, sP, fix_kp=False):
        info = np.zeros(max(batch, 0), dtype=np.int32)
        rc = _check(lib.ipmz_bk_factor_batch(self.h, N, batch, _VP(A_ptr), ld, sA, _VP(ipiv_ptr), sP, int(fix_kp),
                                             info.ctypes.data_as(ctypes.POINTER(_I))), "ipmz_bk_factor_batch")
        return rc, info

    def bk_batch_solve_workspace_bytes(self, N, batch):
        return lib.ipmz_bk_batch_solve_workspace_bytes(self.h, N, batch)

    def bk_prepare_solve_batch(self, N, batch, F_ptr, ld, sA, ipiv_ptr, sP, ws_ptr, ws_bytes):
        return _check(lib.ipmz_bk_prepare_solve_batch(self.h, N, batch, _VP(F_ptr), ld, sA, _VP(ipiv_ptr), sP,
                                                      _VP(ws_ptr), ws_bytes), "ipmz_bk_prepare_solve_batch")

    def bk_solve_multi_batch(self, N, batch, F_ptr, ld, sA, ipiv_ptr, sP, ws_ptr, B_ptr, ldb, sB, nrhs):
        return _check(lib.ipmz_bk_solve_multi_batch(self.h, N, batch, _VP(F_ptr), ld, sA, _VP(ipiv_ptr), sP,
                                                    _VP(ws_ptr), _VP(B_ptr), ldb, sB, nrhs),
                      "ipmz_bk_solve_multi_batch")

    def normal_workspace_bytes(self, n, mp):
        return lib.ipmz_normal_workspace_bytes(self.h, n, mp)

    def normal_factor(self, n, mp, K_ptr, ld, D_ptr, ws_ptr, ws_bytes):
        return _check(lib.ipmz_normal_factor(self.h, n, mp, _VP(K_ptr), ld, _VP(D_ptr), _VP(ws_ptr), ws_bytes),
                      "ipmz_normal_factor")

    def normal_solve(self, n, mp, K_ptr, ld, D_ptr, ws_ptr, b_ptr):
        return _check(lib.ipmz_normal_solve(self.h, n, mp, _VP(K_ptr), ld, _VP(D_ptr), _VP(ws_ptr), _VP(b_ptr)),
                      "ipmz_normal_solve")

    def normal_solve_multi(self, n, mp, K_ptr, ld, D_ptr, ws_ptr, B_ptr, ldb, nrhs):
        return _check(lib.ipmz_normal_solve_multi(self.h, n, mp, _VP(K_ptr), ld, _VP(D_ptr), _VP(ws_ptr), _VP(B_ptr),
                                                  ldb, nrhs), "ipmz_normal_solve_multi")


def debug_inject(mask):
    _check(lib.ipmz_debug_inject(int(mask)), "ipmz_debug_inject")


INJECT_SOLVE, INJECT_PANEL, INJECT_GRAPH_FORKS = 1, 2, 4

_default_ctx = None


def default_context():
    global _default_ctx
    if _default_ctx is None:
        _default_ctx = Context(0)
    return _default_ctx


class LinearSolvers:

    @staticmethod
    def ldlt_decomposition(A, ctx=None):
        A = np.ascontiguousarray(A, dtype=np.float64)
        if A.ndim != 2 or A.shape[0] != A.shape[1]:
            raise IpmzError("ldlt_decomposition: matrix must be square")
        N = A.shape[0]
        L = np.zeros((N, N))
        D = np.zeros(N)
        info = _check(lib.ipmz_ldlt_decomposition((ctx or default_context()).h, N, _dp(A), _dp(L), _dp(D)),
                      "ipmz_ldlt_decomposition")
        return L, D, info

    @staticmethod
    def overwriting_solve_ldlt(L, D, b, ctx=None):
        L = np.ascontiguousarray(L, dtype=np.float64)
        D = np.ascontiguousarray(D, dtype=np.float64)
        if not (isinstance(b, np.ndarray) and b.dtype == np.float64 and b.flags.c_contiguous):
            raise IpmzError("overwriting_solve_ldlt: b must be a contiguous float64 array")
        N = b.shape[0]
        if N and (D.shape[0] != N or L.shape != (N, N)):
            raise IpmzError("overwriting_solve_ldlt: size mismatch")
        _check(lib.ipmz_overwriting_solve_ldlt((ctx or default_context()).h, N, _dp(L), _dp(D), _dp(b)),
               "ipmz_overwriting_solve_ldlt")
        return b

    @staticmethod
    def overwriting_solve_ldlt_multi(L, D, B, ctx=None):
        L = np.ascontiguousarray(L, dtype=np.float64)
        D = np.ascontiguousarray(D, dtype=np.float64)
        if not (isinstance(B, np.ndarray) and B.dtype == np.float64 and B.ndim == 2 and B.flags.c_contiguous):
            raise IpmzError("overwriting_solve_ldlt_multi: B must be a C-contiguous float64 (nrhs, N) array")
        nrhs, N = B.shape
        if D.shape != (N,) or L.shape != (N, N):
            raise IpmzError("overwriting_solve_ldlt_multi: size mismatch")
        _check(lib.ipmz_overwriting_solve_ldlt_multi((ctx or default_context()).h, N, _dp(L), _dp(D), _dp(B), nrhs),
               "ipmz_overwriting_solve_ldlt_multi")
        return B


def _ip(a):
    return a.ctypes.data_as(ctypes.POINTER(ctypes.c_int))


def symmetric_indefinite_factorization(A, ctx=None):
    A = np.ascontiguousarray(A, dtype=np.float64)
    if A.ndim != 2 or A.shape[0] != A.shape[1]:
        raise IpmzError("symmetric_indefinite_factorization: matrix must be square")
    N = A.shape[0]
    F = np.zeros((N, N))
    ipiv = np.zeros(N, dtype=np.int32)
    _check(lib.ipmz_symmetric_indefinite_factorization((ctx or default_context()).h, N, _dp(A), _dp(F), _ip(ipiv)),
           "ipmz_symmetric_indefinite_factorization")
    return F, ipiv


def overwriting_solve_bunch_kaufman(F, ipiv, b, ctx=None):
    F = np.ascontiguousarray(F, dtype=np.float64)
    ipiv = np.ascontiguousarray(ipiv, dtype=np.int32)
    if b.dtype != np.float64 or not b.flags.c_contiguous:
        raise IpmzError("overwriting_solve_bunch_kaufman: b must be a contiguous float64 array")
    _check(lib.ipmz_overwriting_solve_bunch_kaufman((ctx or default_context()).h, len(b), _dp(F), _ip(ipiv), _dp(b)),
           "ipmz_overwriting_solve_bunch_kaufman")


def overwriting_solve_bunch_kaufman_multi(F, ipiv, B, ctx=None):
    F = np.ascontiguousarray(F, dtype=np.float64)
    ipiv = np.ascontiguousarray(ipiv, dtype=np.int32)
    if not (isinstance(B, np.ndarray) and B.dtype == np.float64 and B.ndim == 2 and B.flags.c_contiguous):
        raise IpmzError("overwriting_solve_bunch_kaufman_multi: B must be a C-contiguous float64 (nrhs, N) array")
    nrhs, N = B.shape
# ... 225 lines not shown
            raise ValueError("data_jvp_tensors: no tangent given (ntan is taken from the tensors)")
        ldr = L + (L & 1)
        if out is None:
            out = torch.empty((batch, ntan, ldr), dtype=torch.float64, device=f"cuda:{self.ctx.device}")
        else:
            self._on_device(out, "out")
            if out.dtype != torch.float64 or out.dim() != 3 or tuple(out.shape[:2]) != (batch, ntan) or \
                    out.shape[2] < L or (out.shape[2] > 1 and out.stride(2) != 1):
                raise ValueError(f"out: a float64 ({batch}, {ntan}, >= {L}) tensor with inner stride 1 is needed")
        ld_out = out.stride(1) if ntan > 1 else out.shape[2] + (out.shape[2] & 1)
        s_out = out.stride(0) if batch > 1 else ntan * ld_out
        self._order_torch_stream(torch)
        _check(lib.ipmz_batch_data_jvp(self.h, ntan, ctypes.byref(tan), _VP(out.data_ptr()), ld_out, s_out),
               "ipmz_batch_data_jvp")
        if not self.ctx.on_stream(torch.cuda.current_stream(self.ctx.device).cuda_stream):
            self.ctx.sync()
        return out

    def solution_tensor(self):
        return self.state_tensor(0)[:, :self.n]

    def step(self, flags=0):
        self._bump()
        _check(lib.ipmz_qp_step(self.h, flags), "ipmz_qp_step")

    def last_step_graph(self):
        return bool(lib.ipmz_qp_last_step_graph(self.h))

    def set_reduction(self, reduction):
        _check(lib.ipmz_qp_set_reduction(self.h, reduction), "ipmz_qp_set_reduction")

    def set_mixed_precision(self, enable=True, tol=1e-12, max_refine=10):
        _check(lib.ipmz_qp_set_mixed_precision(self.h, int(enable), tol, max_refine), "ipmz_qp_set_mixed_precision")

    def scalars(self):
        out = np.zeros(SC_COUNT)
        _check(lib.ipmz_qp_scalars(self.h, _dp(out)), "ipmz_qp_scalars")
        return {k: out[i] for k, i in SC.items()}

    def device_scalars_ptr(self):
        p = _VP()
        _check(lib.ipmz_qp_device_scalars(self.h, ctypes.byref(p)), "ipmz_qp_device_scalars")
        return p.value

    def copy_scalars(self, dst_ptr):
        _check(lib.ipmz_qp_copy_scalars(self.h, _VP(dst_ptr)), "ipmz_qp_copy_scalars")

    def solve(self, max_iter=100):
        self._bump()
        trace = np.zeros((max_iter + 1, 8))
        it = ctypes.c_int(0)
        _check(lib.ipmz_qp_solve(self.h, max_iter, _dp(trace), ctypes.byref(it)), "ipmz_qp_solve")
        rows = min(it.value + 1, max_iter)
        keys = ("f", "res", "mu", "alpha_aff", "mu_aff", "sigma", "alpha", "converged")
        return it.value, [dict(zip(keys, r)) for r in trace[:rows]]

    def _state(self, which):
        out = np.zeros(self.state_len)
        _check(lib.ipmz_qp_get_state(self.h, which, _dp(out)), "ipmz_qp_get_state")
        return out

    def vars(self):
        return self._state(0)

    def daff(self):
        return self._state(1)

    def dir(self):
        return self._state(2)

    def residuals(self):
        return self._state(3)

    def set_vars(self, v):
        self._bump()
        v = np.ascontiguousarray(v, dtype=np.float64)
        _check(lib.ipmz_qp_set_state(self.h, _dp(v)), "ipmz_qp_set_state")

    def kkt(self):
        K = np.zeros((self.N, self.N))
        _check(lib.ipmz_qp_get_kkt(self.h, _dp(K)), "ipmz_qp_get_kkt")
        return K

    def kkt_solve(self, B_ptr, nrhs, ldb):
        return _check(lib.ipmz_qp_kkt_solve(self.h, nrhs, _VP(B_ptr), ldb), "ipmz_qp_kkt_solve")

    def kkt_solve_bk(self, B_ptr, nrhs, ldb):
        return _check(lib.ipmz_qp_kkt_solve_bk(self.h, nrhs, _VP(B_ptr), ldb), "ipmz_qp_kkt_solve_bk")

    def kkt_solve_mixed(self, B_ptr, nrhs, ldb, tol=1e-12, max_refine=10):
        stat = np.zeros((max(nrhs, 0), 2))
        info = _check(lib.ipmz_qp_kkt_solve_mixed(self.h, nrhs, _VP(B_ptr), ldb, tol, max_refine, _dp(stat)),
                      "ipmz_qp_kkt_solve_mixed")
        return info, stat

    def newton_solve(self, R_ptr, D_ptr, nrhs, ldr, ldd, alpha_ptr=None):
        return _check(lib.ipmz_qp_newton_solve_multi(self.h, nrhs, _VP(R_ptr), ldr, _VP(D_ptr), ldd, _VP(alpha_ptr)),
                      "ipmz_qp_newton_solve_multi")

    def newton_adjoint(self, G_ptr, Out_ptr, nrhs, ldg, ldo):
        return _check(lib.ipmz_qp_newton_adjoint_multi(self.h, nrhs, _VP(G_ptr), ldg, _VP(Out_ptr), ldo),
                      "ipmz_qp_newton_adjoint_multi")

    def set_timing(self, on=True):
        _check(lib.ipmz_qp_set_timing(self.h, 1 if on else 0), "ipmz_qp_set_timing")

    def phase_times(self):
        ms = np.zeros(8)
        fl = ctypes.c_double(0)
        nl = ctypes.c_int64(0)
        _check(lib.ipmz_qp_phase_times(self.h, _dp(ms), ctypes.byref(fl), ctypes.byref(nl)), "ipmz_qp_phase_times")
        out = {k: ms[i] for k, i in PH.items()}
        out["trailing_flops"] = fl.value
        out["trailing_launches"] = nl.value
        return out

    def close(self):
        if getattr(self, "h", None):
            lib.ipmz_qp_destroy(self.h)
            self.h = None

    def __del__(self):
        try:
            self.close()
        except Exception:
            pass


class Batch(Optimizer):

    def __init__(self, n, m=0, p=0, batch=1, ctx=None, delta=1e-4, equality_handling=0, inequality_handling=0,
                 inequality_bounds=0, variable_bounds=0):
        self.ctx = ctx or default_context()
        cfg = _QPConfig(n, m, p, delta, equality_handling, inequality_handling, inequality_bounds, variable_bounds)
        self.equality_handling = equality_handling
        self.form = (inequality_handling, inequality_bounds, variable_bounds)
        h = _VP()
        _check(lib.ipmz_batch_create(self.ctx.h, ctypes.byref(cfg), batch, ctypes.byref(h)), "ipmz_batch_create")
        self.h = h
        self.n, self.m, self.p = n, m, p
        self.N = lib.ipmz_qp_kkt_dim(h)
        self.batch = batch
        self.state_len = lib.ipmz_qp_state_len(h)

    def load_one(self, index, data):
        self._bump()
        keep = [data.Q, data.c, data.A_ineq, data.l_A_ineq, data.u_A_ineq, data.A_eq, data.b_eq, data.l_x, data.u_x]
        keep = [np.ascontiguousarray(a, dtype=np.float64).reshape(-1) if np.size(a) else np.zeros(1) for a in keep]
        _check(lib.ipmz_batch_load_host(self.h, index, *[_dp(a) for a in keep]), "ipmz_batch_load_host")

    def initialize(self):
        self._bump()
        _check(lib.ipmz_batch_initialize(self.h), "ipmz_batch_initialize")

    def copy_batch_scalars(self, dst_ptr):
        _check(lib.ipmz_batch_copy_scalars(self.h, _VP(dst_ptr)), "ipmz_batch_copy_scalars")

    def summary(self, dst_ptr):
        _check(lib.ipmz_batch_summary(self.h, _VP(dst_ptr)), "ipmz_batch_summary")

    def summary_into(self, t):
        self.summary(t.data_ptr())
        import torch
        if not self.ctx.on_stream(torch.cuda.current_stream(t.device).cuda_stream):
            self.ctx.sync()

# ... 55 lines not shown
```

Measured before the change: 79.29 steps/s.

## Overlap KKT assembly and leading forward solve rows with the LDLT factorization

Adds hooks to the multi-stream LDLT factorization so that the caller's work (the remaining KKT assembly columns) runs on the update stream before the first trailing update. Once the panels covering the leading R rows are final, it also launches the solve-prep and the forward triangular sweep for those rows on a fourth stream. The rest of the forward sweep and the backward sweep then resume from block R/SB. The goal is to hide assembly and part of the solve latency behind the factorization's critical path, at the cost of more events, stream dependencies and split-kernel complexity.

After: 80.32 steps/s, median of 6. +1.3%, better.

```diff
diff --git a/include/ipmz.h b/include/ipmz.h
--- a/include/ipmz.h
+++ b/include/ipmz.h
@@ -152,6 +152,7 @@
 int ipmz_qp_set_state(ipmz_qp* qp, const double* host_vars);
 int ipmz_qp_get_kkt(ipmz_qp* qp, double* host_K);
 int ipmz_qp_kkt_dim(ipmz_qp* qp);
+int ipmz_qp_get_factor(ipmz_qp* qp, double* host_L, double* host_D, double* host_P, int64_t* p_len);
 int ipmz_qp_kkt_solve(ipmz_qp* qp, int nrhs, double* B, int64_t ldb);
 int ipmz_qp_kkt_solve_bk(ipmz_qp* qp, int nrhs, double* B, int64_t ldb);
 int ipmz_qp_kkt_solve_mixed(ipmz_qp* qp, int nrhs, double* B, int64_t ldb, double tol, int max_refine, double* stat);
diff --git a/ipm-zoo_amd/csrc/capi.cpp b/ipm-zoo_amd/csrc/capi.cpp
--- a/ipm-zoo_amd/csrc/capi.cpp
+++ b/ipm-zoo_amd/csrc/capi.cpp
@@ -78,27 +78,62 @@
   return ldlt_solve(K, ld, N, D, w.Linv, nbi, b, w.side, st);
 }
 
+hipError_t solve_ws_tail(const double* K, int64_t ld, int N, const double* D, const LdltWs& w, double* b, int rows,
+                         hipStream_t st) {
+  return ldlt_solve_persistent_tail(K, ld, N, D, w.P, b, w.y, w.z, w.ctrl, rows, st);
+}
+
+int chain_bound_rows(int N, int nbo) {
+  int k = 0;
+  while (N - k * nbo > IPMZ_EARLY_CHAIN_MAX_N) ++k;
+  const int r = k * nbo / IPMZ_SOLVE_BLOCK * IPMZ_SOLVE_BLOCK;
+  return r >= N - IPMZ_SOLVE_BLOCK ? 0 : r;
+}
+
 int factor_impl(ipmz_ctx* ctx, int N, double* K, int64_t ld, double* D, const LdltWs& w, int nbo, TrailTimer* timer,
-                int* info2) {
+                int* info2, StepEdges* edges) {
   HIP_OK(solve_reset(w.y, w.z, sizeof(double), N, w.ctrl, ctx->stream, w.info, w.pctrl, panel_ctrl_words(N, nbo),
                      info2));
   const int npan = (N + nbo - 1) / nbo;
   auto prep = [&]() -> hipError_t {
     return ctx->nbi == 64 ? solve_prep(K, ld, N, w.Linv, w.P, ctx->stream) : hipSuccess;
   };
+  FactorHooks hooks;
+  if (edges) {
+    edges->swept = false;
+    hooks.before_b = edges->rest;
+  }
   if (npan < 3 || (debug_inject_mask() & IPMZ_DEBUG_ONE_STREAM)) {
     HIP_OK(ldlt_factor(K, ld, N, D, w.Linv, w.W, nbo, ctx->nbi, w.info, ctx->stream, timer, nullptr, nullptr, nullptr,
-                       0, w.pctrl));
+                       0, w.pctrl, nullptr, edges ? &hooks : nullptr));
     HIP_OK(prep());
     return IPMZ_OK;
   }
-  const int nev = 5 * npan + 5;
+  const int nev = 5 * npan + 7;
   int rc = ensure_events(ctx, (size_t)nev + 4);
   if (rc) return rc;
   hipEvent_t* ev = ctx->evpool.data();
+  hipEvent_t evSwept = ev[5 * npan + 4];
+  const int R = edges && ctx->nbi == 64 && edges->rows % IPMZ_SOLVE_BLOCK == 0 && edges->rows < N ? edges->rows : 0;
+  if (R > 0) {
+    hooks.final_rows = R;
+    hooks.final_st = ctx->sD;
+    hooks.rows_final = [&](hipStream_t s4) -> hipError_t {
+      hipError_t e = solve_prep_split(K, ld, N, w.Linv, w.P, R, true, s4);
+      if (e == hipSuccess) e = ldlt_solve_persistent_head(K, ld, N, D, w.P, edges->b, w.y, w.z, w.ctrl, R, s4);
+      if (e == hipSuccess) e = stream_record(evSwept, s4);
+      return e;
+    };
+  }
   const bool fourth = false;
   HIP_OK(ldlt_factor(K, ld, N, D, w.Linv, w.W, nbo, ctx->nbi, w.info, ctx->stream, timer, ctx->sB, ctx->sC, ev,
-                     nev - 2, w.pctrl, fourth ? ctx->sD : nullptr));
+                     nev - 2, w.pctrl, fourth ? ctx->sD : nullptr, edges ? &hooks : nullptr));
+  if (hooks.fired) {
+    HIP_OK(stream_wait(ctx->stream, evSwept));
+    HIP_OK(solve_prep_split(K, ld, N, w.Linv, w.P, R, false, ctx->stream));
+    edges->swept = true;
+    return IPMZ_OK;
+  }
   HIP_OK(prep());
   return IPMZ_OK;
 }
diff --git a/ipm-zoo_amd/csrc/capi.h b/ipm-zoo_amd/csrc/capi.h
--- a/ipm-zoo_amd/csrc/capi.h
+++ b/ipm-zoo_amd/csrc/capi.h
@@ -201,8 +201,17 @@
 int ws_result(hipStream_t st, const int* info, const unsigned* pe, const unsigned* se, const char* what,
               const char* pe_text = PANEL_TIMEOUT, const char* se_text = SOLVE_TIMEOUT);
 int read_info(ipmz_ctx* ctx, const LdltWs& w);
+struct StepEdges {
+  std::function<hipError_t(hipStream_t)> rest;
+  int rows = 0;
+  const double* b = nullptr;
+  bool swept = false;
+};
+int chain_bound_rows(int N, int nbo);
 int factor_impl(ipmz_ctx* ctx, int N, double* K, int64_t ld, double* D, const LdltWs& w, int nbo, TrailTimer* timer,
-                int* info2 = nullptr);
+                int* info2 = nullptr, StepEdges* edges = nullptr);
+hipError_t solve_ws_tail(const double* K, int64_t ld, int N, const double* D, const LdltWs& w, double* b, int rows,
+                         hipStream_t st);
 hipError_t solve_ws(const double* K, int64_t ld, int N, const double* D, const LdltWs& w, int nbi, double* b,
                     hipStream_t st);
 int mixed_factor_impl(ipmz_ctx* ctx, const double* K, int64_t ld, MixedWs& w, TrailTimer* timer);
diff --git a/ipm-zoo_amd/csrc/kernels.h b/ipm-zoo_amd/csrc/kernels.h
--- a/ipm-zoo_amd/csrc/kernels.h
+++ b/ipm-zoo_amd/csrc/kernels.h
@@ -2,6 +2,8 @@
 #include <hip/hip_runtime.h>
 #include <stdint.h>
 #include <stdio.h>
+
+#include <functional>
 
 #define IPMZ_NBO_MAX 512
 #define IPMZ_PANEL_CTRL_WORDS 320
@@ -20,7 +22,8 @@
        IPMZ_DEBUG_NO_K0 = 8192, IPMZ_DEBUG_NO_FUSED_SOLVES = 16384, IPMZ_DEBUG_READY_LATE = 32768,
        IPMZ_DEBUG_MULTI_BLOCKED = 65536, IPMZ_DEBUG_MULTI_W512 = 131072,
        IPMZ_DEBUG_MULTI_W128 = 262144, IPMZ_DEBUG_SOLVE_H2 = 524288, IPMZ_DEBUG_SOLVE_H4 = 1048576,
-       IPMZ_DEBUG_NEWTON_RPG1 = 2097152, IPMZ_DEBUG_NEWTON_RPG8 = 4194304 };
+       IPMZ_DEBUG_NEWTON_RPG1 = 2097152, IPMZ_DEBUG_NEWTON_RPG8 = 4194304, IPMZ_DEBUG_SERIAL_EDGES = 8388608,
+       IPMZ_DEBUG_EDGE_ROWS_SHIFT = 24, IPMZ_DEBUG_EDGE_ROWS_MASK = 63 << 24 };
 #define IPMZ_TRACE(...)                                                  \
   do {                                                                   \
     if (::ipmz::debug_inject_mask() & ::ipmz::IPMZ_DEBUG_TRACE) {        \
@@ -72,9 +75,17 @@
   double flops = 0.0;
   hipEvent_t* next() { return used < cap ? pairs[used++] : nullptr; }
 };
+struct FactorHooks {
+  std::function<hipError_t(hipStream_t)> before_b;
+  int final_rows = 0;
+  hipStream_t final_st = nullptr;
+  std::function<hipError_t(hipStream_t)> rows_final;
+  bool fired = false;
+};
 hipError_t ldlt_factor(double* K, int64_t ld, int N, double* D, double* Linv, double* W, int nbo, int nbi,
                        int* info, hipStream_t st, TrailTimer* timer = nullptr, hipStream_t st2 = nullptr,
-                       hipStream_t st3 = nullptr, hipEvent_t* ev = nullptr, int nev = 0, unsigned* pctrl = nullptr, hipStream_t st4 = nullptr);
+                       hipStream_t st3 = nullptr, hipEvent_t* ev = nullptr, int nev = 0, unsigned* pctrl = nullptr,
+                       hipStream_t st4 = nullptr, FactorHooks* hooks = nullptr);
 hipError_t ldlt_factor(float* K, int64_t ld, int N, float* D, float* Linv, float* W, int nbo, int nbi, int* info,
                        hipStream_t st, TrailTimer* timer, hipStream_t st2, hipStream_t st3, hipEvent_t* ev, int nev,
                        unsigned* pctrl = nullptr, hipStream_t st4 = nullptr);
@@ -133,6 +144,13 @@
 hipError_t solve_prep(const float* K, int64_t ld, int N, const float* Linv, float* P, hipStream_t st);
 hipError_t ldlt_solve_persistent(const double* K, int64_t ld, int N, const double* D, const double* P, double* b,
                                  double* ybuf, double* xbuf, unsigned* ctrl, hipStream_t st);
+hipError_t solve_prep_split(const double* K, int64_t ld, int N, const double* Linv, double* P, int R, bool head,
+                            hipStream_t st);
+hipError_t ldlt_solve_persistent_head(const double* K, int64_t ld, int N, const double* D, const double* P,
+                                      const double* b, double* ybuf, double* xbuf, unsigned* ctrl, int R,
+                                      hipStream_t st);
+hipError_t ldlt_solve_persistent_tail(const double* K, int64_t ld, int N, const double* D, const double* P, double* b,
+                                      double* ybuf, double* xbuf, unsigned* ctrl, int R, hipStream_t st);
 hipError_t ldlt_solve_persistent_sweep(const double* K, int64_t ld, int N, const double* D, const double* P,
                                        double* b, double* ybuf, double* xbuf, unsigned* ctrl, bool backward,
                                        hipStream_t st, const unsigned* skip);
@@ -323,6 +341,7 @@
 hipError_t qp_init_iterate(const QPBatch& qb, hipStream_t st);
 hipError_t qp_evaluate(const QPBatch& qb, hipStream_t st);
 hipError_t qp_assemble(const QPBatch& qb, hipStream_t st);
+hipError_t qp_assemble_cols(const QPBatch& qb, int c, bool head, hipStream_t st);
 hipError_t qp_rhs(const QPBatch& qb, hipStream_t st);
 hipError_t qp_backsub(const QPBatch& qb, int which, hipStream_t st);
 hipError_t qp_ratio(const QPBatch& qb, int which, int out_index, hipStream_t st);
diff --git a/ipm-zoo_amd/csrc/ldlt.hip b/ipm-zoo_amd/csrc/ldlt.hip
--- a/ipm-zoo_amd/csrc/ldlt.hip
+++ b/ipm-zoo_amd/csrc/ldlt.hip
@@ -370,11 +370,13 @@
 template <typename T>
 static hipError_t ldlt_factor_t(T* K, int64_t ld, int N, T* D, T* Linv, T* W, int nbo, int nbi, int* info,
                                 hipStream_t st, TrailTimer* timer, hipStream_t st2, hipStream_t st3, hipEvent_t* ev,
-                                int nev, unsigned* pctrl, hipStream_t st4) {
+                                int nev, unsigned* pctrl, hipStream_t st4, FactorHooks* hooks = nullptr) {
   if (N <= 0) return hipSuccess;
   if (nbi != 64 && nbi != 128) return hipErrorInvalidValue;
   if (nbo % nbi != 0 || nbo > IPMZ_NBO_MAX) return hipErrorInvalidValue;
   const int npan = (N + nbo - 1) / nbo;
+  const bool hook_b = hooks && hooks->before_b;
+  if (hook_b && ev != nullptr && nev < 5 * npan + 4) return hipErrorInvalidValue;
   const bool fused = pctrl != nullptr && nbi == 64;
   const bool two = st2 != nullptr && ev != nullptr && nev >= 4 * npan + 2 && (!fused || st3 != nullptr);
   const bool four = two && st4 != nullptr && nev >= 5 * npan + 3 && !(debug_inject_mask() & IPMZ_DEBUG_NO_FOURTH);
@@ -402,6 +404,7 @@
   };
   hipError_t e = hipSuccess;
   if (!two) {
+    if (hook_b && (e = hooks->before_b(st)) != hipSuccess) return e;
     for (int k = 0; k < npan; ++k) {
       const int k0 = k * nbo, bo = pw(k), t0 = k0 + bo;
       if ((e = factor(k, false)) != hipSuccess) return e;
@@ -428,6 +431,12 @@
   if ((e = stream_record(evEntry, st)) != hipSuccess) return e;
   if ((e = stream_wait(st2, evEntry)) != hipSuccess) return e;
   if (fused && (e = stream_wait(sC, evEntry)) != hipSuccess) return e;
+  hipEvent_t evHook = hook_b ? ev[5 * npan + 3] : nullptr;
+  if (hook_b) {
+    IPMZ_TRACE("factor: the caller's work on B before its first update");
+    if ((e = hooks->before_b(st2)) != hipSuccess) return e;
+    if ((e = stream_record(evHook, st2)) != hipSuccess) return e;
+  }
   if ((e = factor(0, false)) != hipSuccess) return e;
   if (fused) {
     if ((e = stream_record(evA[0], st)) != hipSuccess) return e;
@@ -442,6 +451,13 @@
     if (p1 >= N) break;
     IPMZ_TRACE("factor: panel %d", k);
     if ((e = stream_record(evP[k], st)) != hipSuccess) return e;
+    if (hooks && hooks->rows_final && !hooks->fired && hooks->final_rows > 0 && p1 >= hooks->final_rows) {
+      if ((e = stream_wait(hooks->final_st, evP[k])) != hipSuccess) return e;
+      if (fused && early_at(k + 1) && (e = stream_wait(hooks->final_st, evC[k])) != hipSuccess) return e;
+      IPMZ_TRACE("factor: rows < %d final with panel %d", p1, k);
+      if ((e = hooks->rows_final(hooks->final_st)) != hipSuccess) return e;
+      hooks->fired = true;
+    }
     if ((e = stream_wait(st2, evP[k])) != hipSuccess) return e;
     if (early_at(k + 1) && (e = stream_wait(st2, evC[k])) != hipSuccess) return e;
     hipStream_t sN = four ? st4 : st2;
@@ -449,6 +465,7 @@
       if ((e = stream_wait(st4, evP[k])) != hipSuccess) return e;
       if (early_at(k + 1) && (e = stream_wait(st4, evC[k])) != hipSuccess) return e;
       if (k >= 1 && (e = stream_wait(st4, evT[k - 1])) != hipSuccess) return e;
+      if (k == 0 && hook_b && (e = stream_wait(st4, evHook)) != hipSuccess) return e;
     }
     if (p2 < N) {
       if ((e = panel_update(K, ld, N, Wb(k), nbo, k0, bo, p2, p3, false, sN)) != hipSuccess) return e;
@@ -464,6 +481,10 @@
       if (e != hipSuccess) return e;
     }
     if (four && (e = stream_record(evT[k], st2)) != hipSuccess) return e;
+    if (k == 0 && hook_b) {
+      if ((e = stream_wait(st, evHook)) != hipSuccess) return e;
+      if (fused && (e = stream_wait(sC, evHook)) != hipSuccess) return e;
+    }
     if (k >= 1) {
       if (!flag_at(k + 1) && (e = stream_wait(st, evN[k - 1])) != hipSuccess) return e;
       if (fused && (e = stream_wait(sC, evN[k - 1])) != hipSuccess) return e;
@@ -498,8 +519,8 @@
 
 hipError_t ldlt_factor(double* K, int64_t ld, int N, double* D, double* Linv, double* W, int nbo, int nbi,
                        int* info, hipStream_t st, TrailTimer* timer, hipStream_t st2, hipStream_t st3, hipEvent_t* ev,
-                       int nev, unsigned* pctrl, hipStream_t st4) {
-  return ldlt_factor_t<double>(K, ld, N, D, Linv, W, nbo, nbi, info, st, timer, st2, st3, ev, nev, pctrl, st4);
+                       int nev, unsigned* pctrl, hipStream_t st4, FactorHooks* hooks) {
+  return ldlt_factor_t<double>(K, ld, N, D, Linv, W, nbo, nbi, info, st, timer, st2, st3, ev, nev, pctrl, st4, hooks);
 }
 hipError_t ldlt_factor(float* K, int64_t ld, int N, float* D, float* Linv, float* W, int nbo, int nbi, int* info,
                        hipStream_t st, TrailTimer* timer, hipStream_t st2, hipStream_t st3, hipEvent_t* ev, int nev,
diff --git a/ipm-zoo_amd/csrc/newton.hip b/ipm-zoo_amd/csrc/newton.hip
--- a/ipm-zoo_amd/csrc/newton.hip
+++ b/ipm-zoo_amd/csrc/newton.hip
@@ -446,43 +446,61 @@
   return q.eqnone ? 0.0 : q.eqpen ? -q.scal[SC_MU_NEW] : -(q.delta * q.delta);
 }
 
-__device__ __forceinline__ void assemble_row(const QPDev& q, int i, int tid, int nth) {
+__device__ __forceinline__ void assemble_row(const QPDev& q, int i, int tid, int nth, int c0, int c1) {
   double* __restrict__ K = q.K;
   const int64_t ld = q.ldk;
   const int n = q.n, m = q.m, mk = q.mk;
   double* Kr = K + (int64_t)i * ld;
+  const int je = i < c1 ? i : c1;
+  const int jn = n < je ? n : je;
+  const int jz = n > c0 ? n : c0;
+  const bool dg = c0 <= i && i < c1;
   if (i < n) {
     const double* Qr = q.Q + (int64_t)i * q.ldn;
-    for (int j = tid; j < i; j += nth) Kr[j] = Qr[j];
+    for (int j = c0 + tid; j < je; j += nth) Kr[j] = Qr[j];
+    if (!dg) return;
     if (tid == 0) Kr[i] = kkt_diag(q, i);
   } else if (i < n + mk && q.naive) {
     const bool hrow = i >= n + m;
     const int r = hrow ? i - n - m : i - n;
     const double* Ar = q.A + (int64_t)r * q.ldn;
-    for (int j = tid; j < n; j += nth) Kr[j] = hrow ? Ar[j] : -Ar[j];
-    for (int j = n + tid; j < i; j += nth) Kr[j] = 0.0;
+    for (int j = c0 + tid; j < jn; j += nth) Kr[j] = hrow ? Ar[j] : -Ar[j];
+    for (int j = jz + tid; j < je; j += nth) Kr[j] = 0.0;
+    if (!dg) return;
     if (tid == 0) Kr[i] = kkt_diag(q, i);
   } else if (i < n + m) {
     const int r = i - n;
     const double* Ar = q.A + (int64_t)r * q.ldn;
-    for (int j = tid; j < n; j += nth) Kr[j] = Ar[j];
-    for (int j = n + tid; j < i; j += nth) Kr[j] = 0.0;
+    for (int j = c0 + tid; j < jn; j += nth) Kr[j] = Ar[j];
+    for (int j = jz + tid; j < je; j += nth) Kr[j] = 0.0;
+    if (!dg) return;
     if (tid == 0) Kr[i] = kkt_diag(q, i);
   } else {
     const int r = i - n - mk;
     const double* Cr = q.C + (int64_t)r * q.ldn;
-    for (int j = tid; j < n; j += nth) Kr[j] = Cr[j];
-    for (int j = n + tid; j < i; j += nth) Kr[j] = 0.0;
+    for (int j = c0 + tid; j < jn; j += nth) Kr[j] = Cr[j];
+    for (int j = jz + tid; j < je; j += nth) Kr[j] = 0.0;
+    if (!dg) return;
     if (tid == 0) Kr[i] = kkt_diag(q, i);
   }
 }
 
-__global__ __launch_bounds__(NT) void k_assemble(const QPDev* __restrict__ qs) {
-  assemble_row(qs[blockIdx.y], blockIdx.x, threadIdx.x, NT);
+__global__ __launch_bounds__(NT) void k_assemble(const QPDev* __restrict__ qs, int row0, int c0, int c1) {
+  assemble_row(qs[blockIdx.y], row0 + blockIdx.x, threadIdx.x, NT, c0, c1);
 }
 
 hipError_t qp_assemble(const QPBatch& qb, hipStream_t st) {
-  hipLaunchKernelGGL(k_assemble, grid2(qb.h.N, qb.B), dim3(NT), 0, st, qb.d);
+  hipLaunchKernelGGL(k_assemble, grid2(qb.h.N, qb.B), dim3(NT), 0, st, qb.d, 0, 0, qb.h.N);
+  return hipGetLastError();
+}
+hipError_t qp_assemble_cols(const QPBatch& qb, int c, bool head, hipStream_t st) {
+  const int N = qb.h.N;
+  if (c > N) c = N;
+  if (head) {
+    if (c > 0) hipLaunchKernelGGL(k_assemble, grid2(N, qb.B), dim3(NT), 0, st, qb.d, 0, 0, c);
+  } else if (c < N) {
+    hipLaunchKernelGGL(k_assemble, grid2(N - c, qb.B), dim3(NT), 0, st, qb.d, c, c, N);
+  }
   return hipGetLastError();
 }
 
diff --git a/ipm-zoo_amd/csrc/qp.cpp b/ipm-zoo_amd/csrc/qp.cpp
--- a/ipm-zoo_amd/csrc/qp.cpp
+++ b/ipm-zoo_amd/csrc/qp.cpp
@@ -257,7 +257,7 @@
 }
 
 bool uses_k0(const ipmz_qp* s);
-int factor_batch(ipmz_qp* s, TrailTimer* tt, bool info_reset) {
+int factor_batch(ipmz_qp* s, TrailTimer* tt, bool info_reset, StepEdges* edges = nullptr) {
   hipStream_t st = s->ctx->stream;
   const int nbo = nbo_for(s->ctx, s->N);
   switch (path_of(s)) {
@@ -273,7 +273,7 @@
     case Path::Mixed: return mixed_factor_impl(s->ctx, s->K, s->ldk, s->mw, tt);
     case Path::Normal:
       return normal_factor_impl(s->ctx, s->n, s->m + s->p, s->K, s->ldk, s->D, normal_ws_of(s), nbo, tt);
-    case Path::Ldlt: return factor_impl(s->ctx, s->N, s->K, s->ldk, s->D, ldlt_ws_of(s), nbo, tt);
+    case Path::Ldlt: return factor_impl(s->ctx, s->N, s->K, s->ldk, s->D, ldlt_ws_of(s), nbo, tt, nullptr, edges);
     case Path::LdltBatch: break;
   }
   if (!info_reset) HIP_OK(hipMemsetAsync(s->binfo, 0x7f, sizeof(int), st));
@@ -289,6 +289,19 @@
 }
 bool uses_k0(const ipmz_qp* s) {
   return s->K0 && s->ctx->nbi == 64 && s->N <= IPMZ_SMALL_NMAX && !(debug_inject_mask() & IPMZ_DEBUG_NO_K0);
+}
+
+bool step_edges(const ipmz_qp* s) {
+  const int dbg = debug_inject_mask();
+  if (path_of(s) != Path::Ldlt || (dbg & (IPMZ_DEBUG_SERIAL_EDGES | IPMZ_DEBUG_ONE_STREAM))) return false;
+  const int nbo = nbo_for(s->ctx, s->N);
+  return (s->N + nbo - 1) / nbo >= 3;
+}
+int step_edge_rows(const ipmz_qp* s) {
+  if (s->ctx->nbi != 64) return 0;
+  const int v = (debug_inject_mask() & IPMZ_DEBUG_EDGE_ROWS_MASK) >> IPMZ_DEBUG_EDGE_ROWS_SHIFT;
+  const int r = v ? (v - 1) * IPMZ_SOLVE_BLOCK : chain_bound_rows(s->N, nbo_for(s->ctx, s->N));
+  return r >= s->N - IPMZ_SOLVE_BLOCK ? 0 : r;
 }
 
 int run_step(ipmz_qp* s, int flags) {
@@ -332,12 +345,30 @@
   } else {
     if (restart) HIP_OK(qp_restart_if_converged(qb, st));
     mark(0);
-    HIP_OK(qp_assemble(qb, st));
-    mark(1);
-    if ((rc = factor_batch(s, t ? &tt : nullptr, false))) return rc;
+    StepEdges edges;
+    const bool overlap = step_edges(s);
+    if (overlap) {
+      const int c_head = nbo_for(s->ctx, s->N);
+      HIP_OK(qp_assemble_cols(qb, c_head, true, st));
+      mark(1);
+      HIP_OK(qp_rhs(qb, st));
+      edges.rest = [&qb, c_head](hipStream_t sb) { return qp_assemble_cols(qb, c_head, false, sb); };
+      edges.rows = step_edge_rows(s);
+      edges.b = q0(s).b;
+      IPMZ_TRACE("step: edges, head columns %d, early sweep rows %d", c_head, edges.rows);
+    } else {
+      HIP_OK(qp_assemble(qb, st));
+      mark(1);
+    }
+    if ((rc = factor_batch(s, t ? &tt : nullptr, false, overlap ? &edges : nullptr))) return rc;
     mark(2);
-    HIP_OK(qp_rhs(qb, st));
-    if ((rc = solve_batch(s, st, 0))) return rc;
+    if (!overlap) HIP_OK(qp_rhs(qb, st));
+    if (edges.swept) {
+      IPMZ_TRACE("step: forward sweep from row %d on", edges.rows);
+      HIP_OK(solve_ws_tail(s->K, s->ldk, s->N, s->D, ldlt_ws_of(s), q0(s).b, edges.rows, st));
+    } else if ((rc = solve_batch(s, st, 0))) {
+      return rc;
+    }
     mark(3);
     HIP_OK(qp_backsub(qb, 0, st));
     HIP_OK(qp_ratio(qb, 0, SC_ALPHA_AFF, st));
@@ -947,6 +978,30 @@
   return get_kkt_impl(s, 0, out);
 }
 
+int ipmz_qp_get_factor(ipmz_qp* s, double* L, double* D, double* P, int64_t* p_len) {
+  if (!s) return fail(IPMZ_ERR_INVALID, "bad arguments");
+  if (path_of(s) != Path::Ldlt || s->ctx->nbi != 64)
+    return fail(IPMZ_ERR_STATE, "ipmz_qp_get_factor: single QPs on the fp64 augmented LDL^T with nbi = 64");
+  HIP_OK(hipSetDevice(s->ctx->device));
+  hipStream_t st = s->ctx->stream;
+  const int N = s->N;
+  const int64_t q = solve_prep_elems(N) / 4;
+  if (p_len) *p_len = 4 * q;
+  const LdltWs w = ldlt_ws_of(s);
+  if (L) HIP_OK(hipMemcpy2DAsync(L, (size_t)N * 8, s->K, s->ldk * 8, (size_t)N * 8, N, hipMemcpyDeviceToHost, st));
+  if (D) HIP_OK(hipMemcpyAsync(D, s->D, (size_t)N * 8, hipMemcpyDeviceToHost, st));
+  if (P) HIP_OK(hipMemcpyAsync(P, w.P, (size_t)(4 * q) * 8, hipMemcpyDeviceToHost, st));
+  HIP_OK(hipStreamSynchronize(st));
+  if (L)
+    for (int r = 0; r < N; ++r)
+      for (int c = r + 1; c < N; ++c) L[(int64_t)r * N + c] = 0.0;
+  if (P) {
+    const int64_t blk = (int64_t)IPMZ_SOLVE_BLOCK * IPMZ_SOLVE_BLOCK;
+    for (int64_t i = 0; i < blk; ++i) P[2 * q + i] = P[4 * q - blk + i] = 0.0;
+  }
+  return IPMZ_OK;
+}
+
 int ipmz_batch_get_kkt(ipmz_qp* s, int index, double* out) {
   int rc = check_index(s, index);
   if (rc) return rc;
diff --git a/ipm-zoo_amd/csrc/trsv_persist.hip b/ipm-zoo_amd/csrc/trsv_persist.hip
--- a/ipm-zoo_amd/csrc/trsv_persist.hip
+++ b/ipm-zoo_amd/csrc/trsv_persist.hip
@@ -18,7 +18,7 @@
 constexpr int CP_ROWS = 8, CP_LANES = 32;
 constexpr int XS_LD = SB + 4;
 constexpr int TDS = 65;
-enum { SC_TICKET = 2, SC_TICKET_B = 3 };
+enum { SC_TICKET = 2, SC_TICKET_B = 3, SC_TICKET_F2 = 4 };
 
 template <typename T>
 __device__ __forceinline__ bool is_sentinel(T v);
@@ -104,9 +104,11 @@
 __global__ __launch_bounds__(256) void solve_prep_kernel(const T* __restrict__ K, int64_t ld, int N,
                                                          const T* __restrict__ Linv, T* __restrict__ X,
                                                          T* __restrict__ XT, T* __restrict__ M, T* __restrict__ Q,
-                                                         int nb) {
+                                                         int nb, int jbase, int jx0, int jx1, int jq0,
+                                                         int jq1) {
   __shared__ double S[4][64 * TDS];
-  const int J = blockIdx.x, part = blockIdx.y, J0 = J * SB;
+  const int J = jbase + blockIdx.x, part = blockIdx.y, J0 = J * SB;
+  if (part <= 2 ? (J < jx0 || J >= jx1) : (J < jq0 || J >= jq1)) return;
   if ((part == 1 || part == 2) && J == 0) return;
   if (part >= 3 && J + 1 >= nb) return;
   const int h = (part - 1) & 1;
@@ -193,7 +195,7 @@
                                                       const T* __restrict__ XT, const T* __restrict__ M,
                                                       const T* __restrict__ Q, T* b, T* ybuf, T* xbuf,
                                                       unsigned* ctrl, int nb, const unsigned* __restrict__ skip,
-                                                      int inject) {
+                                                      int inject, int nbv, int jfirst) {
   typedef typename Mfma<T>::vec2_t V2;
   constexpr int RW = SB / H;
   constexpr int RPR = RP_ROWS / H;
@@ -208,8 +210,8 @@
   __shared__ __attribute__((aligned(16))) T xs[RW * XS_LD];
   __shared__ unsigned sh_ticket, sh_stop, sh_nr[2];
   unsigned* err = ctrl + SOLVE_ERR_WORD;
-  T* const vbuf = ybuf + (int64_t)nb * SB;
-  T* const ubuf = xbuf + (int64_t)nb * SB;
+  T* const vbuf = ybuf + (int64_t)nbv * SB;
+  T* const ubuf = xbuf + (int64_t)nbv * SB;
   const int tid = threadIdx.x;
   const int rg = tid / RP_LANES, cg = tid % RP_LANES;
   if (tid == 0) sh_nr[0] = sh_nr[1] = 0u;
@@ -296,11 +298,14 @@
 
   for (;;) {
     lds_sync();
-    if (tid == 0) sh_ticket = atomicAdd(&ctrl[BWD ? SC_TICKET_B : SC_TICKET], 1u);
+    if (tid == 0) sh_ticket = atomicAdd(&ctrl[BWD ? SC_TICKET_B : jfirst ? SC_TICKET_F2 : SC_TICKET], 1u);
     lds_sync();
-    const int ticket = (int)sh_ticket;
+    const int ticket = (int)sh_ticket + (BWD ? 0 : jfirst * H);
     if (ticket >= nb * H) return;
-    if (ticket == 0 && tid == 0) st_sc1(&ctrl[BWD ? SC_TICKET : SC_TICKET_B], 0u);
+    if (ticket == 0 && tid == 0) {
+      st_sc1(&ctrl[BWD ? SC_TICKET : SC_TICKET_B], 0u);
+      if (BWD) st_sc1(&ctrl[SC_TICKET_F2], 0u);
+    }
 
     if constexpr (!BWD) {
       const int J = ticket / H, h = ticket % H, J0 = J * SB, r0 = h * RW;
@@ -544,13 +549,25 @@
 }
 
 template <typename T>
-static hipError_t solve_prep_t(const T* K, int64_t ld, int N, const T* Linv, T* P, hipStream_t st) {
+static hipError_t solve_prep_t(const T* K, int64_t ld, int N, const T* Linv, T* P, hipStream_t st, int jx0 = 0,
+                               int jx1 = 1 << 30, int jq0 = 0, int jq1 = 1 << 30) {
   if (N <= 0) return hipSuccess;
   const int nb = (N + SB - 1) / SB;
   const int64_t q = (int64_t)nb * SB * SB;
-  hipLaunchKernelGGL(solve_prep_kernel<T>, dim3(nb, 5), dim3(256), 0, st, K, ld, N, Linv, P, P + q, P + 2 * q,
-                     P + 3 * q, nb);
+  jx1 = jx1 < nb ? jx1 : nb;
+  jq1 = jq1 < nb ? jq1 : nb;
+  const int lo = jx0 < jq0 ? jx0 : jq0, hi = jx1 > jq1 ? jx1 : jq1;
+  if (hi <= lo) return hipSuccess;
+  hipLaunchKernelGGL(solve_prep_kernel<T>, dim3(hi - lo, 5), dim3(256), 0, st, K, ld, N, Linv, P, P + q, P + 2 * q,
+                     P + 3 * q, nb, lo, jx0, jx1, jq0, jq1);
   return hipGetLastError();
+}
+hipError_t solve_prep_split(const double* K, int64_t ld, int N, const double* Linv, double* P, int R, bool head,
+                            hipStream_t st) {
+  if (R <= 0 || R >= N || R % SB) return hipErrorInvalidValue;
+  const int j = R / SB;
+  return head ? solve_prep_t<double>(K, ld, N, Linv, P, st, 0, j, 0, j - 1)
+              : solve_prep_t<double>(K, ld, N, Linv, P, st, j, 1 << 30, j - 1, 1 << 30);
 }
 hipError_t solve_stamps(unsigned long long* out) {
   return hipMemcpyFromSymbol(out, HIP_SYMBOL(g_sstamp), sizeof(unsigned long long) * 2 * 256 * 6);
@@ -577,32 +594,38 @@
   return N <= 12288 ? 4 : 2;
 }
 
+struct SweepRange {
+  int lead = 0, first = 0;
+};
 template <typename T, bool BWD, int H>
 static hipError_t launch_sweep(const T* K, int64_t ld, int N, const T* D, const T* P, T* b, T* ybuf, T* xbuf,
-                               unsigned* ctrl, hipStream_t st, const unsigned* skip) {
-  const int nb = (N + SB - 1) / SB;
-  const int64_t q = (int64_t)nb * SB * SB;
+                               unsigned* ctrl, hipStream_t st, const unsigned* skip, const SweepRange& sr) {
+  const int nb = ((sr.lead ? sr.lead : N) + SB - 1) / SB, nbv = (N + SB - 1) / SB;
+  const int64_t q = (int64_t)nbv * SB * SB;
+  if (sr.lead) N = sr.lead;
   constexpr int RW = SB / H;
   constexpr int64_t lds = (int64_t)sizeof(T) * (RW * XS_LD + (SB / CP_ROWS) * RW + 3 * SB + RW) + 64;
   constexpr int by_threads = 2048 / SNT;
   constexpr int per_cu = 160 * 1024 / lds < by_threads ? (int)(160 * 1024 / lds) : by_threads;
   static_assert(per_cu >= 1, "a part's LDS fits a CU");
-  const int tickets = nb * H, cap = 256 * per_cu;
+  const int tickets = (nb - sr.first) * H, cap = 256 * per_cu;
   const int grid = tickets < cap ? tickets : cap;
   const int inject = debug_inject_mask() & IPMZ_INJECT_SOLVE;
   hipLaunchKernelGGL((trsv128_kernel<T, BWD, H>), dim3(grid), dim3(SNT), 0, st, K, ld, N, D, P, P + q, P + 2 * q,
-                     P + 3 * q, b, ybuf, xbuf, ctrl, nb, skip, inject);
+                     P + 3 * q, b, ybuf, xbuf, ctrl, nb, skip, inject, nbv, sr.first);
   return hipGetLastError();
 }
 template <typename T, bool BWD>
 static hipError_t sweep_t(const T* K, int64_t ld, int N, const T* D, const T* P, T* b, T* ybuf, T* xbuf,
-                          unsigned* ctrl, hipStream_t st, const unsigned* skip) {
+                          unsigned* ctrl, hipStream_t st, const unsigned* skip, const SweepRange& sr = SweepRange()) {
   if (N <= 0) return hipSuccess;
   if (ld % 2) return hipErrorInvalidValue;
+  if (BWD && (sr.lead || sr.first)) return hipErrorInvalidValue;
+  if (sr.lead % SB || sr.lead >= N || (sr.lead && sr.first) || sr.first * SB >= N) return hipErrorInvalidValue;
   switch (solve_parts<T>(N)) {
-    case 4: return launch_sweep<T, BWD, 4>(K, ld, N, D, P, b, ybuf, xbuf, ctrl, st, skip);
-    case 2: return launch_sweep<T, BWD, 2>(K, ld, N, D, P, b, ybuf, xbuf, ctrl, st, skip);
-    default: return launch_sweep<T, BWD, 1>(K, ld, N, D, P, b, ybuf, xbuf, ctrl, st, skip);
+    case 4: return launch_sweep<T, BWD, 4>(K, ld, N, D, P, b, ybuf, xbuf, ctrl, st, skip, sr);
+    case 2: return launch_sweep<T, BWD, 2>(K, ld, N, D, P, b, ybuf, xbuf, ctrl, st, skip, sr);
+    default: return launch_sweep<T, BWD, 1>(K, ld, N, D, P, b, ybuf, xbuf, ctrl, st, skip, sr);
   }
 }
 
@@ -612,6 +635,21 @@
   const hipError_t e = sweep_t<T, false>(K, ld, N, D, P, b, ybuf, xbuf, ctrl, st, skip);
   if (e != hipSuccess) return e;
   return sweep_t<T, true>(K, ld, N, D, P, b, ybuf, xbuf, ctrl, st, skip);
+}
+
+hipError_t ldlt_solve_persistent_head(const double* K, int64_t ld, int N, const double* D, const double* P,
+                                      const double* b, double* ybuf, double* xbuf, unsigned* ctrl, int R,
+                                      hipStream_t st) {
+  if (R <= 0) return hipErrorInvalidValue;
+  return sweep_t<double, false>(K, ld, N, D, P, const_cast<double*>(b), ybuf, xbuf, ctrl, st, nullptr,
+                                SweepRange{R, 0});
+}
+hipError_t ldlt_solve_persistent_tail(const double* K, int64_t ld, int N, const double* D, const double* P, double* b,
+                                      double* ybuf, double* xbuf, unsigned* ctrl, int R, hipStream_t st) {
+  if (R <= 0 || R % SB) return hipErrorInvalidValue;
+  const hipError_t e = sweep_t<double, false>(K, ld, N, D, P, b, ybuf, xbuf, ctrl, st, nullptr, SweepRange{0, R / SB});
+  if (e != hipSuccess) return e;
+  return sweep_t<double, true>(K, ld, N, D, P, b, ybuf, xbuf, ctrl, st, nullptr);
 }
 
 hipError_t ldlt_solve_persistent_sweep(const double* K, int64_t ld, int N, const double* D, const double* P,
diff --git a/ipm-zoo_amd/ipmz_amd/__init__.py b/ipm-zoo_amd/ipmz_amd/__init__.py
--- a/ipm-zoo_amd/ipmz_amd/__init__.py
+++ b/ipm-zoo_amd/ipmz_amd/__init__.py
@@ -41,7 +41,7 @@
     "ipmz_qp_newton_solve_multi", "ipmz_batch_newton_solve_multi",
     "ipmz_qp_newton_adjoint_multi", "ipmz_batch_newton_adjoint_multi",
     "ipmz_batch_load_device", "ipmz_batch_copy_state", "ipmz_batch_data_vjp", "ipmz_batch_data_jvp",
-    "ipmz_batch_data_vjp_multi", "ipmz_batch_set_state_device",
+    "ipmz_batch_data_vjp_multi", "ipmz_batch_set_state_device", "ipmz_qp_get_factor",
 ]
 SOLVE_MULTI_PANEL = 256
 REDUCTION_AUGMENTED, REDUCTION_NORMAL = 0, 1
@@ -173,6 +173,7 @@
         "ipmz_qp_set_state": ([_VP, _P], _I),
         "ipmz_qp_get_kkt": ([_VP, _P], _I),
         "ipmz_qp_kkt_dim": ([_VP], _I),
+        "ipmz_qp_get_factor": ([_VP, _P, _P, _P, ctypes.POINTER(_I64)], _I),
         "ipmz_qp_set_timing": ([_VP, _I], _I),
         "ipmz_qp_phase_times": ([_VP, _P, _P, ctypes.POINTER(_I64)], _I),
         "ipmz_batch_create": ([_VP, ctypes.POINTER(_QPConfig), _I, ctypes.POINTER(_VP)], _I),
@@ -397,6 +398,12 @@
 
 
 INJECT_SOLVE, INJECT_PANEL, INJECT_GRAPH_FORKS = 1, 2, 4
+DEBUG_SERIAL_EDGES = 8388608
+
+
+def debug_edge_rows(rows):
+    assert rows % 128 == 0 and 0 <= rows // 128 <= 62
+    return (rows // 128 + 1) << 24
 
 _default_ctx = None
 
@@ -788,6 +795,13 @@
         _check(lib.ipmz_qp_get_kkt(self.h, _dp(K)), "ipmz_qp_get_kkt")
         return K
 
+    def factor(self):
+        n = _I64(0)
+        _check(lib.ipmz_qp_get_factor(self.h, None, None, None, ctypes.byref(n)), "ipmz_qp_get_factor")
+        L, D, P = np.zeros((self.N, self.N)), np.zeros(self.N), np.zeros(n.value)
+        _check(lib.ipmz_qp_get_factor(self.h, _dp(L), _dp(D), _dp(P), ctypes.byref(n)), "ipmz_qp_get_factor")
+        return L, D, P
+
     def kkt_solve(self, B_ptr, nrhs, ldb):
         return _check(lib.ipmz_qp_kkt_solve(self.h, nrhs, _VP(B_ptr), ldb), "ipmz_qp_kkt_solve")
 
```
